# DannielSilva/MM-VQA

Measured on AMD Instinct MI355X. Metric: samples/sec ROCO-MLM pretrain (resnet152+transformer, bs16/GPU, 224^2, seq32), higher is better.
Workload: dtype f32; 1 GPU; pretrain/roco_train.py MLM-only: resnet152 + transformer(4 layers, 12 heads), num_vis 5, hidden 768, vocab 30522, per-GPU batch 16, 224x224, T=32; fwd + log_softmax/NLL + bwd + grad all-reduce + Adam; dropout on, train-mode BN; random-init weights; global_batch=16, seq_len=32, parallelism=dp1

## Files before the change

### include/mmvqa.h

```cpp
#ifndef MMVQA_H
#define MMVQA_H
#include <stddef.h>
#include <stdint.h>

#ifdef __cplusplus
extern "C" {
#endif

typedef void* mmvqa_stream_t;

#define MMVQA_ACT_NONE 0
#define MMVQA_ACT_RELU 1
#define MMVQA_ACT_GELU 2
#define MMVQA_ACT_SERF 3
#define MMVQA_ACT_SILU 4
#define MMVQA_ACT_SIGMOID 5

#define MMVQA_KIND_FWD 0
#define MMVQA_KIND_DGRAD 1
#define MMVQA_KIND_WGRAD 2

#define MMVQA_STAT_SLOTS 16

typedef struct mmvqa_bn_fold {
// ... 75 lines not shown
  float* colsum;
  const float* gate;
  int gate_hw;
  int mk_mode;
  const int* pixmask;
  float* sk_ws;
  long long sk_ws_floats;
  mmvqa_bn_fold a_fold;
  int stat_slots;
  int reserved1;
  unsigned int* sk_cnt;
  int sk_cnt_n;
  int reserved0;
} mmvqa_gemm_desc;

#define MMVQA_PREC_F32 0
#define MMVQA_PREC_F16 1

typedef struct mmvqa_attn_desc {
  const float* q;
  const float* k;
  const float* v;
  int row_stride, head_stride;
  float* out;
  int out_row_stride, out_head_stride;
  const long long* mask;
  int mask_on_query;
  const float* prev_in;
  float* prev_out;
  float* probs;
  int B, T, heads;
  float sqrt_d;
  float drop_p;
  uint32_t seed;
  const float* dout;
  float* dq;
  float* dk;
  float* dv;
  const float* dprev_in;
  float* dprev_out;
} mmvqa_attn_desc;

typedef struct mmvqa_fb_attn_desc {
  const float* q;
  int q_ld;
  const float* mem_k;
  const float* mem_v;
  long long mem_win;
  int mem_ld;
  const float* self_k;
  const float* self_v;
  int self_ld;
  const float* bias;
  float* probs;
  int p_ld;
  float* out;
  int out_ld;
  int B, n, n_mem, T;
  float scale, drop_p;
  uint32_t seed;
  const float* dout;
  int dout_ld;
  float* dq;
  int dq_ld;
  float* dself_k;
  float* dself_v;
  int dself_ld;
  float* dmem_k;
  float* dmem_v;
  float* dbias;
} mmvqa_fb_attn_desc;

#define MMVQA_FB_MAX_HIDDENS 16
#define MMVQA_FB_MAX_T 256

typedef struct mmvqa_model_desc {
  int cnn;
  int resnet_layers[4];
  int resnet_width;
  int effnet_depth_div;
  int encoder;
  int hidden, heads, n_layers;
  int emb_vocab, max_pos, type_vocab;
  int num_vis;
  int head_kind;
  int n_classes;
  int supcon, feat_dim;
  int use_relu;
  float p_drop;
  float p_emb_drop;
  float p_rf_drop;
  float p_fb_drop;
  int fb_tokens;
} mmvqa_model_desc;

typedef struct mmvqa_bert_desc {
  int layers, hidden, heads, inter, vocab, max_pos, type_vocab;
  float eps;
} mmvqa_bert_desc;

typedef struct mmvqa_bert mmvqa_bert;

typedef void (*mmvqa_grad_cb)(void* user, long long lo, long long hi);

typedef struct mmvqa_engine mmvqa_engine;

int mmvqa_version(void);
const char* mmvqa_last_error(void);
size_t mmvqa_sizeof_gemm_desc(void);
size_t mmvqa_sizeof_attn_desc(void);
size_t mmvqa_sizeof_model_desc(void);
size_t mmvqa_sizeof_fb_attn_desc(void);
size_t mmvqa_sizeof_bert_desc(void);

int mmvqa_igemm(const mmvqa_gemm_desc* d, int kind, int nchw, int tile, mmvqa_stream_t s);
int mmvqa_attention(const mmvqa_attn_desc* d, int head_dim, int backward, mmvqa_stream_t s);
int mmvqa_attention_len_fwd(mmvqa_stream_t s, const float* q, const float* k, const float* v, int row_stride,
                            int head_stride, float* out, int out_row_stride, int out_head_stride, const int* len, int B,
                            int T, int heads, float scale);
int mmvqa_qkv_attention_fwd(mmvqa_stream_t s, const float* xn, const float* W, const float* bias, const long long* mask,
                            float* qkv, float* probs, float* ctx, int B, int T, int hidden, int heads, float drop_p,
                            uint32_t seed);

int mmvqa_fb_attention(const mmvqa_fb_attn_desc* d, int backward, mmvqa_stream_t s);
int mmvqa_fb_aggregate_fwd(mmvqa_stream_t s, const float* hid, long long hid_stride, int n_hid, const float* layer_weight,
                           float* agg, long rows, int H);
int mmvqa_fb_aggregate_bwd(mmvqa_stream_t s, const float* dagg, const float* hid, long long hid_stride, int n_hid,
                           const float* layer_weight, float* dh, long long dh_stride, float* dtop, float* d_layer_weight,
                           long rows, int H);
int mmvqa_geglu_fwd(mmvqa_stream_t s, const float* pre, float* y, long M, int F, float drop_p, uint32_t seed, uint32_t idx0);
int mmvqa_geglu_bwd(mmvqa_stream_t s, const float* dy, const float* pre, float* dpre, long M, int F, float drop_p,
                    uint32_t seed, uint32_t idx0);

int mmvqa_bn_coef_fwd(mmvqa_stream_t s, const double* stat, int C, double count, float eps, const float* gamma,
                      const float* beta, float* run_mean, float* run_var, long long* nbt, float momentum, int reps,
                      int training, float* scale, float* shift, float* mean, float* invstd);
int mmvqa_bn_coef_bwd(mmvqa_stream_t s, const double* stat, int C, double count, const float* gamma,
                      const float* mean, const float* invstd, int training, float* P, float* Q, float* R,
                      float* dgamma, float* dbeta);
int mmvqa_bn_add_relu(mmvqa_stream_t s, const float* z, const float* sc, const float* sh, const float* idn,
                      const float* id_sc, const float* id_sh, float* out, long rows, int C);
int mmvqa_bn_add_relu_fold(mmvqa_stream_t s, const float* z, const mmvqa_bn_fold* f3, const float* idn,
                           const mmvqa_bn_fold* fd, float* out, long rows, int C);
int mmvqa_maxpool_fwd(mmvqa_stream_t s, const float* z, const float* sc, const float* sh, float* out,
                      unsigned char* idx, int N, int H, int W, int C, int OH, int OW);
int mmvqa_maxpool_bwd(mmvqa_stream_t s, const float* gp, const unsigned char* idx, const float* extra,
                      const float* z, const float* sc, const float* sh, const float* mean, const float* invstd,
                      float* g0, double* stat, int N, int H, int W, int C, int OH, int OW);
int mmvqa_layernorm_fwd(mmvqa_stream_t s, const float* x, const float* res, const float* gamma, const float* beta,
                        float* y, float* sum_out, float* mean, float* rstd, int rows, int H, float eps);
int mmvqa_layernorm_bwd(mmvqa_stream_t s, const float* dy, const float* x, const float* gamma, const float* mean,
                        const float* rstd, const float* dres, float* dx, float* dgamma, float* dbeta, int rows,
                        int H);
int mmvqa_embed_fwd(mmvqa_stream_t s, const long long* ids, const long long* seg, const float* word,
                    const float* pos, const float* type, const float* gamma, const float* beta, const float* vis,
                    float* out, float* xhat, float* rstd, int B, int T, int H, int num_vis, float eps,
                    float drop_p, uint32_t seed);
int mmvqa_embed_bwd(mmvqa_stream_t s, const float* dout, const long long* ids, const long long* seg,
                    const float* xhat, const float* rstd, const float* gamma, float* dword, float* dpos,
                    float* dtype, float* dgamma, float* dbeta, float* dvis, int B, int T, int H, int num_vis,
                    float drop_p, uint32_t seed, int pad_idx);
int mmvqa_meanpool_fwd(mmvqa_stream_t s, const float* h, const long long* mask, float* out, int B, int T, int H);
int mmvqa_meanpool_bwd(mmvqa_stream_t s, const float* dout, const long long* mask, float* dh, int B, int T, int H,
                       int accumulate);
int mmvqa_mlm_loss(mmvqa_stream_t s, const float* logits, int ld, const long long* target, float* row_loss,
                   float* row_lse, long long* pred, float* dlogits, int dld, const float* gscale_ptr, float gscale_mul,
                   int rows, int V, float* out3);
int mmvqa_mlm_grad(mmvqa_stream_t s, const float* logits, int ld, const long long* target, const float* row_lse,
                   float* dlogits, int dld, const float* gscale_ptr, float gscale_mul, int rows, int V);
int mmvqa_asl_loss(mmvqa_stream_t s, const float* logits, int ld, const long long* target, float* row_loss,
                   float* dlogits, int dld, int rows, int C, float gamma_pos, float gamma_neg, float eps,
                   float gscale);
int mmvqa_l2norm_fwd(mmvqa_stream_t s, const float* x, float* y, float* nrm, int rows, int D);
int mmvqa_l2norm_bwd(mmvqa_stream_t s, const float* dy, const float* y, const float* nrm, float* dx, int rows,
                     int D);
int mmvqa_supcon_loss(mmvqa_stream_t s, const float* f, float* loss, float* df, float* ws, int N, int D, float temp,
                      float base_temp, float gscale);
int mmvqa_supcon_loss_masked(mmvqa_stream_t s, const float* f, const float* mask, float* loss, float* df, float* ws,
                             int N, int D, float temp, float base_temp, float gscale);
int mmvqa_jaccard_mask(mmvqa_stream_t s, const int* offsets, const int* ids, const int* rowsA, const int* colsA,
                       const int* rowsB, const int* colsB, float* mask, int n, int table_rows);
int mmvqa_normalize_rows(mmvqa_stream_t s, float* x, long long rows, int D, float eps);
int mmvqa_cosine_mask(mmvqa_stream_t s, const float* table, const int* rowsA, const int* colsA, const int* rowsB,
                      const int* colsB, float* mask, int n, int D, int table_rows);
int mmvqa_bertscore_mask(mmvqa_stream_t s, const float* xa, const int* lenA, const float* xb, const int* lenB, float* mask,
                         float* prec, float* rec, int n, int T, int D, float baseline);
#define MMVQA_SOFT_CE_HARD 0
#define MMVQA_SOFT_CE_UNIFORM 1
#define MMVQA_SOFT_CE_CATEGORY 2
int mmvqa_soft_ce_loss(mmvqa_stream_t s, const float* logits, int ld, const long long* target, const long long* category,
                       const float* table, int table_ld, int n_cat, int mode, double smoothing, float* row_loss,
                       float* loss, float* dlogits, int dld, int rows, int C, float gscale);
int mmvqa_distill_mse(mmvqa_stream_t s, const float* h, int ld, const void* table, int table_f16, long long table_rows,
                      const long long* start, const int* count, int first, int B, int T, int H, float* row_sq, float* loss,
                      float* dh, int dld, float gscale);
int mmvqa_dwconv_fwd(mmvqa_stream_t s, const float* z1, const float* s1, const float* b1, const float* w, float* z2,
                     double* stat, int N, int H, int W, int C, int OH, int OW, int stride, int pad);
int mmvqa_dwconv_bwd_data(mmvqa_stream_t s, const float* g2, const float* z2, const float* P, const float* Q,
                          const float* R, const float* w, const float* z1, const float* s1, const float* b1,
                          const float* mean1, const float* invstd1, float* g1, double* stat, int N, int H, int W, int C,
                          int OH, int OW, int stride, int pad);
int mmvqa_dwconv_bwd_weight(mmvqa_stream_t s, const float* g2, const float* z2, const float* P, const float* Q,
                            const float* R, const float* z1, const float* s1, const float* b1, float* dw, int N, int H,
                            int W, int C, int OH, int OW, int stride, int pad);
int mmvqa_se_pool(mmvqa_stream_t s, const float* z, const float* sc, const float* sh, float* pool, int N, int HW, int C);
int mmvqa_se_dgate(mmvqa_stream_t s, const float* t, const float* z, const float* sc, const float* sh, float* dgate,
                   int N, int HW, int C);
int mmvqa_dwconv_fwd_fold(mmvqa_stream_t s, const float* z1, const float* s1, const float* b1, const float* w, float* z2,
                          double* stat, int N, int H, int W, int C, int OH, int OW, int stride, int pad,
                          const mmvqa_bn_fold* fold);
int mmvqa_dwconv_bwd_data_fold(mmvqa_stream_t s, const float* g2, const float* z2, const float* P, const float* Q,
                               const float* R, const float* w, const float* z1, const float* s1, const float* b1,
                               const float* mean1, const float* invstd1, float* g1, double* stat, int N, int H, int W,
                               int C, int OH, int OW, int stride, int pad, const mmvqa_bn_fold* fold);
int mmvqa_dwconv_bwd_weight_fold(mmvqa_stream_t s, const float* g2, const float* z2, const float* P, const float* Q,
                                 const float* R, const float* z1, const float* s1, const float* b1, float* dw, int N,
                                 int H, int W, int C, int OH, int OW, int stride, int pad, const mmvqa_bn_fold* fold);
int mmvqa_se_pool_fold(mmvqa_stream_t s, const float* z, const float* sc, const float* sh, float* pool, int N, int HW,
                       int C, const mmvqa_bn_fold* fold);
int mmvqa_tap_thin_ok(long M, int N, int C, int HW);
int mmvqa_tap_thin_fwd(mmvqa_stream_t s, const float* x, const float* sc, const float* sh, const float* W, float* out,
                       long M, int N, int C, int HW, int act);
int mmvqa_tap_thin_bwd(mmvqa_stream_t s, const float* x, const float* sc, const float* sh, const float* W,
                       const float* dv, float* du, long M, int N, int C, int HW, int act);
int mmvqa_se_fc_fwd(mmvqa_stream_t s, const float* pool, const float* Wr, const float* br, const float* We,
                    const float* be, float* rpre, float* r, float* gpre, float* gate, int B, int mid, int rd);
size_t mmvqa_se_fc_bwd_scratch_floats(int B, int mid, int rd);
int mmvqa_se_fc_bwd(mmvqa_stream_t s, const float* dgate, const float* gpre, const float* r, const float* rpre,
                    const float* pool, const float* We, const float* Wr, float* dWe, float* dbe, float* dWr, float* dbr,
                    float* dpool, float* scratch, int B, int mid, int rd);
int mmvqa_act_bwd_stats(mmvqa_stream_t s, const float* t, const float* gate, const float* add, const float* z,
                        const float* sc, const float* sh, const float* mean, const float* invstd, int act, float* out,
                        double* stat, long npix, int HW, int C);
int mmvqa_bn_act_add(mmvqa_stream_t s, const float* z, const float* sc, const float* sh, int pre_act, const float* idn,
                     const float* ids, const float* idb, int idn_act, int post_act, float* out, long rows, int C);
int mmvqa_bn_act_add_fold(mmvqa_stream_t s, const float* z, const mmvqa_bn_fold* f3, int pre_act, const float* idn,
                          const mmvqa_bn_fold* fd, int post_act, float* out, long rows, int C);
int mmvqa_adam(mmvqa_stream_t s, float* p, float* g, float* m, float* v, long n, double lr, double b1, double b2,
               double eps, int step, float gscale, int zero_grad);
int mmvqa_amp_unscale(mmvqa_stream_t s, float* g, long n, const float* inv_scale, float* found_inf, int multiply);
int mmvqa_amp_update_scale(mmvqa_stream_t s, float* scale, int* growth_tracker, const float* found_inf,
                           double growth_factor, double backoff_factor, int growth_interval);
int mmvqa_axpy(mmvqa_stream_t s, float* y, const float* x, float a, long n);
int mmvqa_colsum(mmvqa_stream_t s, const float* x, int ld, int rows, int cols, float* out);
int mmvqa_dropout(mmvqa_stream_t s, float* x, long n, float p, uint32_t seed);
int mmvqa_dropout_copy(mmvqa_stream_t s, const float* x, float* y, long n, float p, uint32_t seed);
int mmvqa_pixmask(mmvqa_stream_t s, int* out, int N, int OH, int OW, int SH, int SW, int KH, int KW, int stride,
                  int pad);

int mmvqa_engine_create(const mmvqa_model_desc* desc, mmvqa_engine** out);
void mmvqa_engine_destroy(mmvqa_engine* e);
int mmvqa_engine_num_tensors(const mmvqa_engine* e);
int mmvqa_engine_tensor_info(const mmvqa_engine* e, int i, char* name, int name_cap, int* kind, int* ndim,
                             long long shape[4], long long* offset, int* channels_last);
long long mmvqa_engine_param_floats(const mmvqa_engine* e);
long long mmvqa_engine_buf_floats(const mmvqa_engine* e);
long long mmvqa_engine_nbt_count(const mmvqa_engine* e);
size_t mmvqa_engine_plan(mmvqa_engine* e, int B, int T, int img_h, int img_w);
int mmvqa_engine_bind(mmvqa_engine* e, float* params, float* grads, float* bufs, long long* nbt, void* workspace,
                      size_t workspace_bytes);
int mmvqa_engine_forward(mmvqa_engine* e, mmvqa_stream_t s, const float* img, const long long* ids,
                         const long long* seg, const long long* mask, float* logits, int logits_ld, float* feat,
                         int training, uint32_t seed);
int mmvqa_engine_backward(mmvqa_engine* e, mmvqa_stream_t s, const float* dlogits, int dlogits_ld,
                          const float* dfeat);
int mmvqa_engine_backward_feature(mmvqa_engine* e, mmvqa_stream_t s, const float* dlogits, int dlogits_ld, float* dA);
int mmvqa_engine_feature_map(mmvqa_engine* e, const float** A, int* H, int* W, int* C);
int mmvqa_gradcam(mmvqa_stream_t s, const float* A, const float* dA, int B, int H, int W, int C, float* cam, int* valid,
                  float* up, int IH, int IW, const unsigned char* image_u8, const unsigned char* jet, float alpha,
                  unsigned char* overlay);
int mmvqa_engine_set_grad_callback(mmvqa_engine* e, mmvqa_grad_cb cb, void* user);
int mmvqa_engine_tune(mmvqa_engine* e, int enable);
int mmvqa_engine_set_precision(mmvqa_engine* e, int mode);
int mmvqa_engine_profile(mmvqa_engine* e, int enable);
int mmvqa_engine_profile_read(mmvqa_engine* e, int cls, long long* launches, double* ms, double* flops);
int mmvqa_engine_profile_read_region(mmvqa_engine* e, int region, int cls, long long* launches, double* ms,
                                     double* flops);
int mmvqa_engine_profile_read_hbm(mmvqa_engine* e, int kernel, long long* launches, double* ms, double* bytes);

int mmvqa_bert_create(const mmvqa_bert_desc* desc, mmvqa_bert** out);
void mmvqa_bert_destroy(mmvqa_bert* e);
int mmvqa_bert_num_tensors(const mmvqa_bert* e);
long long mmvqa_bert_param_floats(const mmvqa_bert* e);
int mmvqa_bert_tensor_info(const mmvqa_bert* e, int i, char* name, int name_cap, int* ndim, long long shape[2],
                           long long* offset);
size_t mmvqa_bert_plan(mmvqa_bert* e, int B, int T);
int mmvqa_bert_bind(mmvqa_bert* e, const float* params, void* workspace, size_t workspace_bytes);
int mmvqa_bert_forward(mmvqa_bert* e, mmvqa_stream_t s, const long long* ids, const int* len, int B, int T, float* out);
int mmvqa_bert_forward_layers(mmvqa_bert* e, mmvqa_stream_t s, const long long* ids, const int* len, int B, int T,
                              int n_layers, float* out);

typedef struct mmvqa_resample_job {
  const unsigned char* src; int sh, sw, spitch;
  int bx, by, bw, bh;
  int rw, rh;
  int ox, oy;
  int ty0, tyn;
  unsigned char* tmp;
  unsigned char* dst; int dpitch;
  const int* hb; const int* hk; int hks;
  const int* vb; const int* vk; int vks;
} mmvqa_resample_job;
size_t mmvqa_sizeof_resample_job(void);
int mmvqa_resample_coeffs(int in_size, double in0, double in1, int out_size, int* bounds, int* kk, int ksize_cap);
int mmvqa_aug_resample(mmvqa_stream_t s, const mmvqa_resample_job* jobs_dev, int njobs, int max_tmp_rows, int out_h,
                       int out_w);
// ... 30 lines not shown
```

### mm-vqa_amd/_lib.py

```python
from __future__ import annotations

import ctypes as C
import os

_HERE = os.path.dirname(os.path.abspath(__file__))
LIB_PATH = os.path.join(_HERE, "libmmvqa_hip.so")

c_f32p = C.c_void_p
c_ptr = C.c_void_p

ACT_NONE, ACT_RELU, ACT_GELU, ACT_SERF, ACT_SILU, ACT_SIGMOID = 0, 1, 2, 3, 4, 5
KIND_FWD, KIND_DGRAD, KIND_WGRAD = 0, 1, 2
PRO_NONE, PRO_AFFINE_RELU, PRO_DZ, PRO_AFFINE, PRO_AFFINE_SILU, PRO_SILU_GATE = 0, 1, 2, 3, 4, 5
EPI_PLAIN, EPI_TAP_FWD, EPI_TAP_BWD = 0, 1, 2
PREC_F32, PREC_F16 = 0, 1
SOFT_CE_HARD, SOFT_CE_UNIFORM, SOFT_CE_CATEGORY = 0, 1, 2
HEAD_MLM, HEAD_VQA, HEAD_NONE = 0, 1, 2
STAT_SLOTS = 16


class BnFold(C.Structure):
    _fields_ = [
        ("stat", c_ptr), ("slots", C.c_int), ("bwd", C.c_int), ("publish", C.c_int), ("reps", C.c_int),
        ("count", C.c_double), ("keep", C.c_double), ("eps", C.c_float), ("reserved", C.c_int),
        ("gamma", c_ptr), ("beta", c_ptr), ("mean", c_ptr), ("invstd", c_ptr),
        ("out0", c_ptr), ("out1", c_ptr), ("out2", c_ptr), ("out3", c_ptr),
        ("run_mean", c_ptr), ("run_var", c_ptr), ("nbt", c_ptr), ("dgamma", c_ptr), ("dbeta", c_ptr),
    ]


class GemmDesc(C.Structure):
    _fields_ = [
        ("M", C.c_int), ("N", C.c_int), ("K", C.c_int), ("splitk", C.c_int), ("ktiles_per_split", C.c_int),
        ("A", c_ptr), ("A2", c_ptr), ("a_c0", c_ptr), ("a_c1", c_ptr), ("a_c2", c_ptr),
        ("a_pro", C.c_int), ("a_ld", C.c_int),
        ("B", c_ptr), ("b_c0", c_ptr), ("b_c1", c_ptr), ("b_pro", C.c_int), ("b_ld", C.c_int),
        ("b_tapstride", C.c_int),
        ("g_SH", C.c_int), ("g_SW", C.c_int), ("g_Cs", C.c_int), ("g_OH", C.c_int), ("g_OW", C.c_int),
        ("g_KH", C.c_int), ("g_KW", C.c_int), ("g_stride", C.c_int), ("g_pad", C.c_int), ("g_nchw", C.c_int),
        ("C", c_ptr), ("c_ld", C.c_int), ("c_atomic", C.c_int), ("Cpre", c_ptr), ("bias", c_ptr),
        ("act", C.c_int), ("dact", C.c_int), ("Pre", c_ptr), ("pre_ld", C.c_int),
        ("drop_p", C.c_float), ("drop_seed", C.c_uint32), ("R", c_ptr), ("r_ld", C.c_int),
        ("epi_mode", C.c_int), ("tap_HW", C.c_int), ("tap_out", c_ptr), ("tap_dv", c_ptr),
        ("Mk", c_ptr), ("mk_ld", C.c_int), ("mk_s", c_ptr), ("mk_b", c_ptr),
        ("stat1", c_ptr), ("stat_bwd", C.c_int), ("Z1", c_ptr), ("z1_ld", C.c_int), ("mean1", c_ptr),
        ("invstd1", c_ptr),
        ("stat2", c_ptr), ("Z2", c_ptr), ("z2_ld", C.c_int), ("mean2", c_ptr), ("invstd2", c_ptr),
        ("colsum", c_ptr), ("gate", c_ptr), ("gate_hw", C.c_int), ("mk_mode", C.c_int), ("pixmask", c_ptr),
        ("sk_ws", c_ptr), ("sk_ws_floats", C.c_longlong),
        ("a_fold", BnFold), ("stat_slots", C.c_int), ("reserved1", C.c_int), ("sk_cnt", c_ptr), ("sk_cnt_n", C.c_int),
        ("reserved0", C.c_int),
    ]


class AttnDesc(C.Structure):
    _fields_ = [
        ("q", c_ptr), ("k", c_ptr), ("v", c_ptr), ("row_stride", C.c_int), ("head_stride", C.c_int),
        ("out", c_ptr), ("out_row_stride", C.c_int), ("out_head_stride", C.c_int),
        ("mask", c_ptr), ("mask_on_query", C.c_int), ("prev_in", c_ptr), ("prev_out", c_ptr), ("probs", c_ptr),
        ("B", C.c_int), ("T", C.c_int), ("heads", C.c_int), ("sqrt_d", C.c_float), ("drop_p", C.c_float),
        ("seed", C.c_uint32),
        ("dout", c_ptr), ("dq", c_ptr), ("dk", c_ptr), ("dv", c_ptr), ("dprev_in", c_ptr), ("dprev_out", c_ptr),
    ]


class FbAttnDesc(C.Structure):
    _fields_ = [
        ("q", c_ptr), ("q_ld", C.c_int), ("mem_k", c_ptr), ("mem_v", c_ptr), ("mem_win", C.c_longlong), ("mem_ld", C.c_int),
        ("self_k", c_ptr), ("self_v", c_ptr), ("self_ld", C.c_int), ("bias", c_ptr), ("probs", c_ptr), ("p_ld", C.c_int),
        ("out", c_ptr), ("out_ld", C.c_int), ("B", C.c_int), ("n", C.c_int), ("n_mem", C.c_int), ("T", C.c_int),
        ("scale", C.c_float), ("drop_p", C.c_float), ("seed", C.c_uint32),
        ("dout", c_ptr), ("dout_ld", C.c_int), ("dq", c_ptr), ("dq_ld", C.c_int),
        ("dself_k", c_ptr), ("dself_v", c_ptr), ("dself_ld", C.c_int), ("dmem_k", c_ptr), ("dmem_v", c_ptr), ("dbias", c_ptr),
    ]


FB_MAX_HIDDENS, FB_MAX_T = 16, 256
ENC_TRANSFORMER, ENC_REALFORMER, ENC_FEEDBACK = 0, 1, 2


class ResampleJob(C.Structure):
    _fields_ = [
        ("src", c_ptr), ("sh", C.c_int), ("sw", C.c_int), ("spitch", C.c_int),
        ("bx", C.c_int), ("by", C.c_int), ("bw", C.c_int), ("bh", C.c_int),
        ("rw", C.c_int), ("rh", C.c_int), ("ox", C.c_int), ("oy", C.c_int), ("ty0", C.c_int), ("tyn", C.c_int),
        ("tmp", c_ptr), ("dst", c_ptr), ("dpitch", C.c_int),
        ("hb", c_ptr), ("hk", c_ptr), ("hks", C.c_int), ("vb", c_ptr), ("vk", c_ptr), ("vks", C.c_int),
    ]


class AugRecord(C.Structure):
    _fields_ = [
        ("bx", C.c_int), ("by", C.c_int), ("bw", C.c_int), ("bh", C.c_int), ("ty0", C.c_int), ("tyn", C.c_int),
        ("hb", C.c_int), ("hk", C.c_int), ("hks", C.c_int), ("vb", C.c_int), ("vk", C.c_int), ("vks", C.c_int),
        ("fix", C.c_int * 6), ("op", C.c_int * 4), ("factor", C.c_float * 4),
    ]


class ModelDesc(C.Structure):
    _fields_ = [
        ("cnn", C.c_int), ("resnet_layers", C.c_int * 4), ("resnet_width", C.c_int), ("effnet_depth_div", C.c_int),
        ("encoder", C.c_int), ("hidden", C.c_int), ("heads", C.c_int), ("n_layers", C.c_int),
        ("emb_vocab", C.c_int), ("max_pos", C.c_int), ("type_vocab", C.c_int), ("num_vis", C.c_int),
        ("head_kind", C.c_int), ("n_classes", C.c_int), ("supcon", C.c_int), ("feat_dim", C.c_int),
        ("use_relu", C.c_int), ("p_drop", C.c_float), ("p_emb_drop", C.c_float), ("p_rf_drop", C.c_float),
        ("p_fb_drop", C.c_float), ("fb_tokens", C.c_int),
    ]


class BertDesc(C.Structure):
    _fields_ = [
        ("layers", C.c_int), ("hidden", C.c_int), ("heads", C.c_int), ("inter", C.c_int), ("vocab", C.c_int),
        ("max_pos", C.c_int), ("type_vocab", C.c_int), ("eps", C.c_float),
    ]


_i, _f, _d, _l, _ll, _u32, _sz = C.c_int, C.c_float, C.c_double, C.c_long, C.c_longlong, C.c_uint32, C.c_size_t
_P = c_ptr
SIGNATURES = {
    "mmvqa_version": (_i, []),
    "mmvqa_last_error": (C.c_char_p, []),
    "mmvqa_sizeof_gemm_desc": (_sz, []),
    "mmvqa_sizeof_attn_desc": (_sz, []),
    "mmvqa_sizeof_model_desc": (_sz, []),
    "mmvqa_sizeof_fb_attn_desc": (_sz, []),
    "mmvqa_sizeof_bert_desc": (_sz, []),
    "mmvqa_igemm": (_i, [C.POINTER(GemmDesc), _i, _i, _i, _P]),
    "mmvqa_attention": (_i, [C.POINTER(AttnDesc), _i, _i, _P]),
    "mmvqa_attention_len_fwd": (_i, [_P, _P, _P, _P, _i, _i, _P, _i, _i, _P, _i, _i, _i, _f]),
    "mmvqa_qkv_attention_fwd": (_i, [_P, _P, _P, _P, _P, _P, _P, _P, _i, _i, _i, _i, _f, _u32]),
    "mmvqa_fb_attention": (_i, [C.POINTER(FbAttnDesc), _i, _P]),
    "mmvqa_fb_aggregate_fwd": (_i, [_P, _P, _ll, _i, _P, _P, _l, _i]),
    "mmvqa_fb_aggregate_bwd": (_i, [_P, _P, _P, _ll, _i, _P, _P, _ll, _P, _P, _l, _i]),
    "mmvqa_geglu_fwd": (_i, [_P, _P, _P, _l, _i, _f, _u32, _u32]),
    "mmvqa_geglu_bwd": (_i, [_P, _P, _P, _P, _l, _i, _f, _u32, _u32]),
    "mmvqa_bn_coef_fwd": (_i, [_P, _P, _i, _d, _f, _P, _P, _P, _P, _P, _f, _i, _i, _P, _P, _P, _P]),
    "mmvqa_bn_coef_bwd": (_i, [_P, _P, _i, _d, _P, _P, _P, _i, _P, _P, _P, _P, _P]),
    "mmvqa_bn_add_relu": (_i, [_P, _P, _P, _P, _P, _P, _P, _P, _l, _i]),
    "mmvqa_bn_add_relu_fold": (_i, [_P, _P, C.POINTER(BnFold), _P, C.POINTER(BnFold), _P, _l, _i]),
    "mmvqa_maxpool_fwd": (_i, [_P, _P, _P, _P, _P, _P, _i, _i, _i, _i, _i, _i]),
    "mmvqa_maxpool_bwd": (_i, [_P, _P, _P, _P, _P, _P, _P, _P, _P, _P, _P, _i, _i, _i, _i, _i, _i]),
    "mmvqa_layernorm_fwd": (_i, [_P, _P, _P, _P, _P, _P, _P, _P, _P, _i, _i, _f]),
    "mmvqa_layernorm_bwd": (_i, [_P, _P, _P, _P, _P, _P, _P, _P, _P, _P, _i, _i]),
    "mmvqa_embed_fwd": (_i, [_P, _P, _P, _P, _P, _P, _P, _P, _P, _P, _P, _P, _i, _i, _i, _i, _f, _f, _u32]),
    "mmvqa_embed_bwd": (_i, [_P, _P, _P, _P, _P, _P, _P, _P, _P, _P, _P, _P, _P, _i, _i, _i, _i, _f, _u32, _i]),
    "mmvqa_meanpool_fwd": (_i, [_P, _P, _P, _P, _i, _i, _i]),
    "mmvqa_meanpool_bwd": (_i, [_P, _P, _P, _P, _i, _i, _i, _i]),
    "mmvqa_mlm_loss": (_i, [_P, _P, _i, _P, _P, _P, _P, _P, _i, _P, _f, _i, _i, _P]),
    "mmvqa_mlm_grad": (_i, [_P, _P, _i, _P, _P, _P, _i, _P, _f, _i, _i]),
    "mmvqa_asl_loss": (_i, [_P, _P, _i, _P, _P, _P, _i, _i, _i, _f, _f, _f, _f]),
    "mmvqa_l2norm_fwd": (_i, [_P, _P, _P, _P, _i, _i]),
    "mmvqa_l2norm_bwd": (_i, [_P, _P, _P, _P, _P, _i, _i]),
    "mmvqa_supcon_loss": (_i, [_P, _P, _P, _P, _P, _i, _i, _f, _f, _f]),
    "mmvqa_supcon_loss_masked": (_i, [_P, _P, _P, _P, _P, _P, _i, _i, _f, _f, _f]),
    "mmvqa_jaccard_mask": (_i, [_P] * 8 + [_i, _i]),
    "mmvqa_normalize_rows": (_i, [_P, _P, _ll, _i, _f]),
    "mmvqa_cosine_mask": (_i, [_P] * 7 + [_i, _i, _i]),
    "mmvqa_bertscore_mask": (_i, [_P] * 8 + [_i, _i, _i, _f]),
    "mmvqa_soft_ce_loss": (_i, [_P, _P, _i, _P, _P, _P, _i, _i, _i, _d, _P, _P, _P, _i, _i, _i, _f]),
    "mmvqa_distill_mse": (_i, [_P, _P, _i, _P, _i, _ll, _P, _P, _i, _i, _i, _i, _P, _P, _P, _i, _f]),
    "mmvqa_dwconv_fwd": (_i, [_P, _P, _P, _P, _P, _P, _P] + [_i] * 8),
    "mmvqa_dwconv_bwd_data": (_i, [_P] * 14 + [_i] * 8),
    "mmvqa_dwconv_bwd_weight": (_i, [_P] * 10 + [_i] * 8),
    "mmvqa_se_pool": (_i, [_P, _P, _P, _P, _P, _i, _i, _i]),
    "mmvqa_dwconv_fwd_fold": (_i, [_P, _P, _P, _P, _P, _P, _P] + [_i] * 8 + [C.POINTER(BnFold)]),
    "mmvqa_dwconv_bwd_data_fold": (_i, [_P] * 14 + [_i] * 8 + [C.POINTER(BnFold)]),
    "mmvqa_dwconv_bwd_weight_fold": (_i, [_P] * 10 + [_i] * 8 + [C.POINTER(BnFold)]),
    "mmvqa_se_pool_fold": (_i, [_P, _P, _P, _P, _P, _i, _i, _i, C.POINTER(BnFold)]),
    "mmvqa_bn_act_add_fold": (_i, [_P, _P, C.POINTER(BnFold), _i, _P, C.POINTER(BnFold), _i, _P, _l, _i]),
    "mmvqa_se_dgate": (_i, [_P, _P, _P, _P, _P, _P, _i, _i, _i]),
    "mmvqa_tap_thin_ok": (_i, [_l, _i, _i, _i]),
    "mmvqa_tap_thin_fwd": (_i, [_P] * 6 + [_l, _i, _i, _i, _i]),
    "mmvqa_tap_thin_bwd": (_i, [_P] * 7 + [_l, _i, _i, _i, _i]),
    "mmvqa_se_fc_fwd": (_i, [_P] * 10 + [_i, _i, _i]),
    "mmvqa_se_fc_bwd_scratch_floats": (_sz, [_i, _i, _i]),
    "mmvqa_se_fc_bwd": (_i, [_P] * 14 + [_i, _i, _i]),
    "mmvqa_act_bwd_stats": (_i, [_P] * 9 + [_i, _P, _P, _l, _i, _i]),
    "mmvqa_bn_act_add": (_i, [_P, _P, _P, _P, _i, _P, _P, _P, _i, _i, _P, _l, _i]),
    "mmvqa_adam": (_i, [_P, _P, _P, _P, _P, _l, _d, _d, _d, _d, _i, _f, _i]),
    "mmvqa_axpy": (_i, [_P, _P, _P, _f, _l]),
    "mmvqa_colsum": (_i, [_P, _P, _i, _i, _i, _P]),
    "mmvqa_dropout": (_i, [_P, _P, _l, _f, _u32]),
    "mmvqa_dropout_copy": (_i, [_P, _P, _P, _l, _f, _u32]),
    "mmvqa_pixmask": (_i, [_P, _P] + [_i] * 9),
    "mmvqa_sizeof_resample_job": (_sz, []),
    "mmvqa_resample_coeffs": (_i, [_i, _d, _d, _i, _P, _P, _i]),
    "mmvqa_aug_resample": (_i, [_P, _P, _i, _i, _i, _i]),
    "mmvqa_aug_rotate": (_i, [_P, _P, _P, _P, _i, _i, _i]),
    "mmvqa_aug_jitter_round": (_i, [_P, _P, _P, _P, _P, _i, _i]),
    "mmvqa_aug_to_tensor": (_i, [_P, _P, _P, _i, _i, _P, _P]),
    "mmvqa_sizeof_aug_record": (_sz, []),
    "mmvqa_aug_train_fused": (_i, [_P, _P, _P, _P, _P, _i, _i, _P, _P]),
    "mmvqa_aug_train_fused_views": (_i, [_P, _P, _P, _P, _P, _P, _i, _i, _i, _P, _P]),
    "mmvqa_aug_train_fused_fits": (_i, [_i]),
    "mmvqa_low_priority_stream": (_i, [C.POINTER(_P), C.POINTER(_i)]),
    "mmvqa_stream_priority": (_i, [_P, C.POINTER(_i)]),
    "mmvqa_bert_create": (_i, [C.POINTER(BertDesc), C.POINTER(_P)]),
    "mmvqa_bert_destroy": (None, [_P]),
    "mmvqa_bert_num_tensors": (_i, [_P]),
    "mmvqa_bert_param_floats": (_ll, [_P]),
    "mmvqa_bert_tensor_info": (_i, [_P, _i, C.c_char_p, _i, C.POINTER(_i), C.POINTER(_ll * 2), C.POINTER(_ll)]),
    "mmvqa_bert_plan": (_sz, [_P, _i, _i]),
    "mmvqa_bert_bind": (_i, [_P, _P, _P, _sz]),
    "mmvqa_bert_forward": (_i, [_P, _P, _P, _P, _i, _i, _P]),
    "mmvqa_bert_forward_layers": (_i, [_P, _P, _P, _P, _i, _i, _i, _P]),
    "mmvqa_engine_create": (_i, [C.POINTER(ModelDesc), C.POINTER(_P)]),
    "mmvqa_engine_destroy": (None, [_P]),
    "mmvqa_engine_num_tensors": (_i, [_P]),
    "mmvqa_engine_tensor_info": (_i, [_P, _i, C.c_char_p, _i, C.POINTER(_i), C.POINTER(_i), C.POINTER(_ll * 4),
                                      C.POINTER(_ll), C.POINTER(_i)]),
    "mmvqa_engine_param_floats": (_ll, [_P]),
    "mmvqa_engine_buf_floats": (_ll, [_P]),
    "mmvqa_engine_nbt_count": (_ll, [_P]),
    "mmvqa_engine_plan": (_sz, [_P, _i, _i, _i, _i]),
    "mmvqa_engine_bind": (_i, [_P, _P, _P, _P, _P, _P, _sz]),
    "mmvqa_engine_forward": (_i, [_P, _P, _P, _P, _P, _P, _P, _i, _P, _i, _u32]),
    "mmvqa_engine_backward": (_i, [_P, _P, _P, _i, _P]),
    "mmvqa_engine_backward_feature": (_i, [_P, _P, _P, _i, _P]),
    "mmvqa_engine_feature_map": (_i, [_P, C.POINTER(_P), C.POINTER(_i), C.POINTER(_i), C.POINTER(_i)]),
    "mmvqa_gradcam": (_i, [_P, _P, _P, _i, _i, _i, _i, _P, _P, _P, _i, _i, _P, _P, _f, _P]),
    "mmvqa_engine_set_grad_callback": (_i, [_P, _P, _P]),
    "mmvqa_engine_tune": (_i, [_P, _i]),
    "mmvqa_amp_unscale": (_i, [_P, _P, _l, _P, _P, _i]),
    "mmvqa_amp_update_scale": (_i, [_P, _P, _P, _P, _d, _d, _i]),
    "mmvqa_engine_set_precision": (_i, [_P, _i]),
    "mmvqa_engine_profile": (_i, [_P, _i]),
    "mmvqa_engine_profile_read": (_i, [_P, _i, C.POINTER(_ll), C.POINTER(_d), C.POINTER(_d)]),
    "mmvqa_engine_profile_read_region": (_i, [_P, _i, _i, C.POINTER(_ll), C.POINTER(_d), C.POINTER(_d)]),
    "mmvqa_engine_profile_read_hbm": (_i, [_P, _i, C.POINTER(_ll), C.POINTER(_d), C.POINTER(_d)]),
}

_lib = None


class MMVQAError(RuntimeError):
    pass


def lib():
    global _lib
    if _lib is not None:
        return _lib
    if not os.path.exists(LIB_PATH):
        raise MMVQAError(
            f"{LIB_PATH} not found: the HIP extension is not built. There is no CPU fallback -- run "
            "`python -c 'import __graft_entry__ as g; g.build()'` (needs hipcc, no GPU required).")
    L = C.CDLL(LIB_PATH)
    for name, (res, args) in SIGNATURES.items():
        fn = getattr(L, name)
        fn.restype = res
        fn.argtypes = args
    for nm, st in (("gemm", GemmDesc), ("attn", AttnDesc), ("model", ModelDesc), ("fb_attn", FbAttnDesc), ("bert", BertDesc), ("resample_job", ResampleJob),
                   ("aug_record", AugRecord)):
        if nm in ("resample_job", "aug_record"):
            got = getattr(L, f"mmvqa_sizeof_{nm}")()
            if got != C.sizeof(st):
                raise MMVQAError(f"ABI mismatch: sizeof(mmvqa_{nm}) = {got} in the library, {C.sizeof(st)} in Python")
            continue
        got = getattr(L, f"mmvqa_sizeof_{nm}_desc")()
        if got != C.sizeof(st):
            raise MMVQAError(f"ABI mismatch: sizeof(mmvqa_{nm}_desc) = {got} in the library, {C.sizeof(st)} in Python")
    _lib = L
    return L


def check(rc: int):
    if rc != 0:
        msg = lib().mmvqa_last_error()
        raise MMVQAError(f"mmvqa error {rc}: {msg.decode() if msg else '?'}")


def ptr(t):
    return None if t is None else C.c_void_p(t.data_ptr())


def stream_ptr():
    import torch
    return C.c_void_p(torch.cuda.current_stream().cuda_stream)
```

### mm-vqa_amd/csrc/abi.cpp

```cpp
#include <cstring>

#include "engine.h"

const char* mmvqa_get_error();
size_t engine_plan(mmvqa_engine* e, int B, int T, int IH, int IW);
int engine_forward(mmvqa_engine* e, hipStream_t st, const float* img, const long long* ids, const long long* seg,
                   const long long* mask, float* logits, int logits_ld, float* feat, int training, uint32_t seed);
int engine_backward(mmvqa_engine* e, hipStream_t st, const float* dlogits, int dl_ld, const float* dfeat);
int engine_backward_feature(mmvqa_engine* e, hipStream_t st, const float* dlogits, int dl_ld, float* dA);
int engine_feature_map(mmvqa_engine* e, const float** A, int* H, int* W, int* C);
int engine_create(const mmvqa_model_desc* desc, mmvqa_engine** out);
int engine_profile_collect(mmvqa_engine* e);

#define ST(s) reinterpret_cast<hipStream_t>(s)

extern "C" {

int mmvqa_version(void) { return 100; }
const char* mmvqa_last_error(void) { return mmvqa_get_error(); }
size_t mmvqa_sizeof_gemm_desc(void) { return sizeof(mmvqa_gemm_desc); }
size_t mmvqa_sizeof_attn_desc(void) { return sizeof(mmvqa_attn_desc); }
size_t mmvqa_sizeof_model_desc(void) { return sizeof(mmvqa_model_desc); }
size_t mmvqa_sizeof_fb_attn_desc(void) { return sizeof(mmvqa_fb_attn_desc); }

static int check_gemm(const mmvqa_gemm_desc* d, int kind, int nchw) {
  if (!d) return mmvqa_set_error(MMVQA_ERR_ARG, "igemm: null descriptor");
  if (kind < 0 || kind > 2) return mmvqa_set_error(MMVQA_ERR_ARG, "igemm: kind=%d", kind);
  if (!d->A || !d->B || (!d->C && d->epi_mode != EPI_TAP_FWD))
    return mmvqa_set_error(MMVQA_ERR_ARG, "igemm: null operand");
  if (!nchw) {
    const int taps = d->g_KH * d->g_KW;
    if ((d->a_ld & 3) || (d->b_ld & 3) || (taps > 1 && (d->g_Cs & 3)))
      return mmvqa_set_error(MMVQA_ERR_ARG, "igemm: a_ld=%d b_ld=%d g_Cs=%d must be multiples of 4", d->a_ld,
                             d->b_ld, d->g_Cs);
    if (kind != KIND_FWD && (d->N & 3) && kind == KIND_DGRAD)
      return mmvqa_set_error(MMVQA_ERR_ARG, "igemm dgrad: N=%d must be a multiple of 4", d->N);
  }
  if (d->a_pro == PRO_DZ && (!d->A2 || (!d->a_fold.stat && (!d->a_c0 || !d->a_c1 || !d->a_c2))))
    return mmvqa_set_error(MMVQA_ERR_ARG, "igemm: PRO_DZ needs A2 and three coefficient arrays (or a_fold)");
  if (d->g_SH <= 0 || d->g_SW <= 0 || d->g_OH <= 0 || d->g_OW <= 0 || d->g_Cs <= 0)
    return mmvqa_set_error(MMVQA_ERR_ARG, "igemm: gather geometry not set");
  return MMVQA_OK;
}

int mmvqa_igemm(const mmvqa_gemm_desc* d, int kind, int nchw, int tile, mmvqa_stream_t s) {
  int r = check_gemm(d, kind, nchw);
  if (r != MMVQA_OK) return r;
  return mmvqa_launch_igemm(*d, kind, nchw, tile, ST(s));
}

int mmvqa_attention(const mmvqa_attn_desc* d, int head_dim, int backward, mmvqa_stream_t s) {
  if (!d || !d->q || !d->k || !d->v || !d->mask || !d->probs)
    return mmvqa_set_error(MMVQA_ERR_ARG, "attention: null operand");
  if ((d->row_stride & 3) || (d->head_stride & 3) || (d->out_row_stride & 3) || (d->out_head_stride & 3))
    return mmvqa_set_error(MMVQA_ERR_ARG, "attention: strides must be multiples of 4");
  if (backward && (!d->dout || !d->dq || !d->dk || !d->dv))
    return mmvqa_set_error(MMVQA_ERR_ARG, "attention backward: null gradient pointer");
  if (!backward && !d->out) return mmvqa_set_error(MMVQA_ERR_ARG, "attention: null output");
  return mmvqa_launch_attention(*d, head_dim, backward, ST(s));
}

int mmvqa_qkv_attention_fwd(mmvqa_stream_t s, const float* xn, const float* W, const float* bias, const long long* mask,
                            float* qkv, float* probs, float* ctx, int B, int T, int hidden, int heads, float drop_p,
                            uint32_t seed) {
  if (B <= 0 || drop_p < 0.f || drop_p >= 1.f) return mmvqa_set_error(MMVQA_ERR_ARG, "qkv_attention_fwd: B=%d drop_p=%g", B, (double)drop_p);
  return k_qkv_attn_fwd(ST(s), xn, W, bias, mask, qkv, probs, ctx, B, T, hidden, heads, drop_p, seed);
}
int mmvqa_attention_len_fwd(mmvqa_stream_t s, const float* q, const float* k, const float* v, int row_stride,
                            int head_stride, float* out, int out_row_stride, int out_head_stride, const int* len, int B,
                            int T, int heads, float scale) {
  return k_attention_len_fwd(ST(s), q, k, v, row_stride, head_stride, out, out_row_stride, out_head_stride, len, B, T, heads,
                             scale);
}
int mmvqa_fb_attention(const mmvqa_fb_attn_desc* d, int backward, mmvqa_stream_t s) {
  if (!d) return mmvqa_set_error(MMVQA_ERR_ARG, "fb_attention: null descriptor");
  return k_fb_attention(ST(s), *d, backward ? 1 : 0);
}
int mmvqa_fb_aggregate_fwd(mmvqa_stream_t s, const float* hid, long long hid_stride, int n_hid, const float* layer_weight,
                           float* agg, long rows, int H) {
  return k_fb_aggregate_fwd(ST(s), hid, hid_stride, n_hid, layer_weight, agg, rows, H);
}
int mmvqa_fb_aggregate_bwd(mmvqa_stream_t s, const float* dagg, const float* hid, long long hid_stride, int n_hid,
                           const float* layer_weight, float* dh, long long dh_stride, float* dtop, float* d_layer_weight,
                           long rows, int H) {
  return k_fb_aggregate_bwd(ST(s), dagg, hid, hid_stride, n_hid, layer_weight, dh, dh_stride, dtop, d_layer_weight, rows, H);
}
int mmvqa_geglu_fwd(mmvqa_stream_t s, const float* pre, float* y, long M, int F, float drop_p, uint32_t seed, uint32_t idx0) {
  return k_geglu_fwd(ST(s), pre, y, M, F, drop_p, seed, idx0);
}
int mmvqa_geglu_bwd(mmvqa_stream_t s, const float* dy, const float* pre, float* dpre, long M, int F, float drop_p,
                    uint32_t seed, uint32_t idx0) {
  return k_geglu_bwd(ST(s), dy, pre, dpre, M, F, drop_p, seed, idx0);
}
int mmvqa_bn_coef_fwd(mmvqa_stream_t s, const double* stat, int C, double count, float eps, const float* gamma,
                      const float* beta, float* run_mean, float* run_var, long long* nbt, float momentum, int reps,
                      int training, float* scale, float* shift, float* mean, float* invstd) {
  return k_bn_coef_fwd(ST(s), stat, C, count, eps, gamma, beta, run_mean, run_var, nbt, momentum, reps, training,
                       scale, shift, mean, invstd);
}
int mmvqa_bn_coef_bwd(mmvqa_stream_t s, const double* stat, int C, double count, const float* gamma,
                      const float* mean, const float* invstd, int training, float* P, float* Q, float* R,
                      float* dgamma, float* dbeta) {
  return k_bn_coef_bwd(ST(s), stat, C, count, gamma, mean, invstd, training, P, Q, R, dgamma, dbeta);
}
int mmvqa_bn_add_relu_fold(mmvqa_stream_t s, const float* z, const mmvqa_bn_fold* f3, const float* idn,
                           const mmvqa_bn_fold* fd, float* out, long rows, int C) {
  if (!z || !idn || !out || !f3) return mmvqa_set_error(MMVQA_ERR_ARG, "bn_add_relu_fold: null operand");
  return k_bn_add_relu_fold(ST(s), z, f3, idn, fd, out, rows, C);
}
int mmvqa_bn_add_relu(mmvqa_stream_t s, const float* z, const float* sc, const float* sh, const float* idn,
                      const float* id_sc, const float* id_sh, float* out, long rows, int C) {
  if (C & 3) return mmvqa_set_error(MMVQA_ERR_ARG, "bn_add_relu: C %% 4 != 0");
  return k_bn_add_relu(ST(s), z, sc, sh, idn, id_sc, id_sh, out, rows, C);
}
int mmvqa_maxpool_fwd(mmvqa_stream_t s, const float* z, const float* sc, const float* sh, float* out,
                      unsigned char* idx, int N, int H, int W, int C, int OH, int OW) {
  if (C & 3) return mmvqa_set_error(MMVQA_ERR_ARG, "maxpool: C %% 4 != 0");
  return k_maxpool_fwd(ST(s), z, sc, sh, out, idx, N, H, W, C, OH, OW);
}
int mmvqa_maxpool_bwd(mmvqa_stream_t s, const float* gp, const unsigned char* idx, const float* extra,
                      const float* z, const float* sc, const float* sh, const float* mean, const float* invstd,
                      float* g0, double* stat, int N, int H, int W, int C, int OH, int OW) {
  return k_maxpool_bwd(ST(s), gp, idx, extra, z, sc, sh, mean, invstd, g0, stat, N, H, W, C, OH, OW);
}
int mmvqa_layernorm_fwd(mmvqa_stream_t s, const float* x, const float* res, const float* gamma, const float* beta,
                        float* y, float* sum_out, float* mean, float* rstd, int rows, int H, float eps) {
  return k_layernorm_fwd(ST(s), x, res, gamma, beta, y, sum_out, mean, rstd, rows, H, eps);
}
int mmvqa_layernorm_bwd(mmvqa_stream_t s, const float* dy, const float* x, const float* gamma, const float* mean,
                        const float* rstd, const float* dres, float* dx, float* dgamma, float* dbeta, int rows,
                        int H) {
  return k_layernorm_bwd(ST(s), dy, x, gamma, mean, rstd, dres, dx, dgamma, dbeta, rows, H);
}
int mmvqa_embed_fwd(mmvqa_stream_t s, const long long* ids, const long long* seg, const float* word,
                    const float* pos, const float* type, const float* gamma, const float* beta, const float* vis,
                    float* out, float* xhat, float* rstd, int B, int T, int H, int num_vis, float eps,
                    float drop_p, uint32_t seed) {
  return k_embed_fwd(ST(s), ids, seg, word, pos, type, gamma, beta, vis, out, xhat, rstd, B, T, H, num_vis, eps,
                     drop_p, seed);
}
int mmvqa_embed_bwd(mmvqa_stream_t s, const float* dout, const long long* ids, const long long* seg,
                    const float* xhat, const float* rstd, const float* gamma, float* dword, float* dpos,
                    float* dtype, float* dgamma, float* dbeta, float* dvis, int B, int T, int H, int num_vis,
                    float drop_p, uint32_t seed, int pad_idx) {
  return k_embed_bwd(ST(s), dout, ids, seg, xhat, rstd, gamma, dword, dpos, dtype, dgamma, dbeta, dvis, B, T, H,
                     num_vis, drop_p, seed, pad_idx);
}
int mmvqa_meanpool_fwd(mmvqa_stream_t s, const float* h, const long long* mask, float* out, int B, int T, int H) {
  return k_meanpool_fwd(ST(s), h, mask, out, B, T, H);
}
int mmvqa_meanpool_bwd(mmvqa_stream_t s, const float* dout, const long long* mask, float* dh, int B, int T, int H,
                       int accumulate) {
  return k_meanpool_bwd(ST(s), dout, mask, dh, B, T, H, accumulate);
}
int mmvqa_mlm_loss(mmvqa_stream_t s, const float* logits, int ld, const long long* target, float* row_loss,
                   float* row_lse, long long* pred, float* dlogits, int dld, const float* gscale_ptr, float gscale_mul,
                   int rows, int V, float* out3) {
  return k_lsm_nll(ST(s), logits, ld, target, row_loss, row_lse, pred, dlogits, dld, gscale_ptr, gscale_mul, rows, V, out3);
}
int mmvqa_mlm_grad(mmvqa_stream_t s, const float* logits, int ld, const long long* target, const float* row_lse,
                   float* dlogits, int dld, const float* gscale_ptr, float gscale_mul, int rows, int V) {
  return k_lsm_grad(ST(s), logits, ld, target, row_lse, dlogits, dld, gscale_ptr, gscale_mul, rows, V);
}
int mmvqa_asl_loss(mmvqa_stream_t s, const float* logits, int ld, const long long* target, float* row_loss,
                   float* dlogits, int dld, int rows, int C, float gamma_pos, float gamma_neg, float eps,
                   float gscale) {
  return k_asl(ST(s), logits, ld, target, row_loss, dlogits, dld, rows, C, gamma_pos, gamma_neg, eps, gscale);
}
int mmvqa_l2norm_fwd(mmvqa_stream_t s, const float* x, float* y, float* nrm, int rows, int D) {
  return k_l2norm_fwd(ST(s), x, y, nrm, rows, D);
}
int mmvqa_l2norm_bwd(mmvqa_stream_t s, const float* dy, const float* y, const float* nrm, float* dx, int rows,
                     int D) {
  return k_l2norm_bwd(ST(s), dy, y, nrm, dx, rows, D);
}
int mmvqa_supcon_loss(mmvqa_stream_t s, const float* f, float* loss, float* df, float* ws, int N, int D, float temp,
                      float base_temp, float gscale) {
  return k_supcon(ST(s), f, nullptr, loss, df, ws, N, D, temp, base_temp, gscale);
}
int mmvqa_supcon_loss_masked(mmvqa_stream_t s, const float* f, const float* mask, float* loss, float* df, float* ws,
                             int N, int D, float temp, float base_temp, float gscale) {
  if (!mask) return mmvqa_set_error(MMVQA_ERR_ARG, "supcon_masked: mask is null (mmvqa_supcon_loss is the loss without one)");
  return k_supcon(ST(s), f, mask, loss, df, ws, N, D, temp, base_temp, gscale);
}
int mmvqa_jaccard_mask(mmvqa_stream_t s, const int* offsets, const int* ids, const int* rowsA, const int* colsA,
                       const int* rowsB, const int* colsB, float* mask, int n, int table_rows) {
  return k_jaccard_mask(ST(s), offsets, ids, rowsA, colsA, rowsB, colsB, mask, n, table_rows);
}
int mmvqa_normalize_rows(mmvqa_stream_t s, float* x, long long rows, int D, float eps) {
  return k_normalize_rows(ST(s), x, rows, D, eps);
}
int mmvqa_cosine_mask(mmvqa_stream_t s, const float* table, const int* rowsA, const int* colsA, const int* rowsB,
                      const int* colsB, float* mask, int n, int D, int table_rows) {
  return k_cosine_mask(ST(s), table, rowsA, colsA, rowsB, colsB, mask, n, D, table_rows);
}
int mmvqa_bertscore_mask(mmvqa_stream_t s, const float* xa, const int* lenA, const float* xb, const int* lenB, float* mask,
                         float* prec, float* rec, int n, int T, int D, float baseline) {
  return k_bertscore_mask(ST(s), xa, lenA, xb, lenB, mask, prec, rec, n, T, D, baseline);
}
int mmvqa_soft_ce_loss(mmvqa_stream_t s, const float* logits, int ld, const long long* target, const long long* category,
                       const float* table, int table_ld, int n_cat, int mode, double smoothing, float* row_loss,
                       float* loss, float* dlogits, int dld, int rows, int C, float gscale) {
  return k_soft_ce(ST(s), logits, ld, target, category, table, table_ld, n_cat, mode, smoothing, row_loss, loss, dlogits,
                   dld, rows, C, gscale);
}
int mmvqa_distill_mse(mmvqa_stream_t s, const float* h, int ld, const void* table, int table_f16, long long table_rows,
                      const long long* start, const int* count, int first, int B, int T, int H, float* row_sq, float* loss,
                      float* dh, int dld, float gscale) {
  return k_distill_mse(ST(s), h, ld, table, table_f16, table_rows, start, count, first, B, T, H, row_sq, loss, dh, dld,
                       gscale);
}
int mmvqa_dwconv_fwd(mmvqa_stream_t s, const float* z1, const float* s1, const float* b1, const float* w, float* z2,
                     double* stat, int N, int H, int W, int C, int OH, int OW, int stride, int pad) {
  return k_dwconv_fwd(ST(s), z1, s1, b1, w, z2, stat, N, H, W, C, OH, OW, stride, pad);
}
int mmvqa_dwconv_bwd_data(mmvqa_stream_t s, const float* g2, const float* z2, const float* P, const float* Q,
                          const float* R, const float* w, const float* z1, const float* s1, const float* b1,
                          const float* mean1, const float* invstd1, float* g1, double* stat, int N, int H, int W, int C,
                          int OH, int OW, int stride, int pad) {
  return k_dwconv_bwd_data(ST(s), g2, z2, P, Q, R, w, z1, s1, b1, mean1, invstd1, g1, stat, N, H, W, C, OH, OW, stride, pad);
}
int mmvqa_dwconv_bwd_weight(mmvqa_stream_t s, const float* g2, const float* z2, const float* P, const float* Q,
                            const float* R, const float* z1, const float* s1, const float* b1, float* dw, int N, int H,
                            int W, int C, int OH, int OW, int stride, int pad) {
  return k_dwconv_bwd_weight(ST(s), g2, z2, P, Q, R, z1, s1, b1, dw, N, H, W, C, OH, OW, stride, pad);
}
int mmvqa_se_pool(mmvqa_stream_t s, const float* z, const float* sc, const float* sh, float* pool, int N, int HW, int C) {
  return k_se_pool(ST(s), z, sc, sh, pool, N, HW, C);
}
int mmvqa_dwconv_fwd_fold(mmvqa_stream_t s, const float* z1, const float* s1, const float* b1, const float* w, float* z2,
                          double* stat, int N, int H, int W, int C, int OH, int OW, int stride, int pad,
                          const mmvqa_bn_fold* fold) {
  return k_dwconv_fwd(ST(s), z1, s1, b1, w, z2, stat, N, H, W, C, OH, OW, stride, pad, fold);
}
int mmvqa_dwconv_bwd_data_fold(mmvqa_stream_t s, const float* g2, const float* z2, const float* P, const float* Q,
                               const float* R, const float* w, const float* z1, const float* s1, const float* b1,
                               const float* mean1, const float* invstd1, float* g1, double* stat, int N, int H, int W,
                               int C, int OH, int OW, int stride, int pad, const mmvqa_bn_fold* fold) {
  return k_dwconv_bwd_data(ST(s), g2, z2, P, Q, R, w, z1, s1, b1, mean1, invstd1, g1, stat, N, H, W, C, OH, OW, stride, pad, fold);
}
int mmvqa_dwconv_bwd_weight_fold(mmvqa_stream_t s, const float* g2, const float* z2, const float* P, const float* Q,
                                 const float* R, const float* z1, const float* s1, const float* b1, float* dw, int N,
                                 int H, int W, int C, int OH, int OW, int stride, int pad, const mmvqa_bn_fold* fold) {
  return k_dwconv_bwd_weight(ST(s), g2, z2, P, Q, R, z1, s1, b1, dw, N, H, W, C, OH, OW, stride, pad, fold);
}
int mmvqa_se_pool_fold(mmvqa_stream_t s, const float* z, const float* sc, const float* sh, float* pool, int N, int HW,
                       int C, const mmvqa_bn_fold* fold) {
  return k_se_pool(ST(s), z, sc, sh, pool, N, HW, C, fold);
}
int mmvqa_bn_act_add_fold(mmvqa_stream_t s, const float* z, const mmvqa_bn_fold* f3, int pre_act, const float* idn,
                          const mmvqa_bn_fold* fd, int post_act, float* out, long rows, int C) {
  return k_bn_act_add_fold(ST(s), z, f3, pre_act, idn, fd, post_act, out, rows, C);
}
int mmvqa_se_dgate(mmvqa_stream_t s, const float* t, const float* z, const float* sc, const float* sh, float* dgate,
                   int N, int HW, int C) {
  return k_se_dgate(ST(s), t, z, sc, sh, dgate, N, HW, C);
}
int mmvqa_tap_thin_ok(long M, int N, int C, int HW) { return k_tap_thin_ok(M, N, C, HW) ? 1 : 0; }
int mmvqa_tap_thin_fwd(mmvqa_stream_t s, const float* x, const float* sc, const float* sh, const float* W, float* out,
                       long M, int N, int C, int HW, int act) {
  return k_tap_thin_fwd(ST(s), x, sc, sh, W, out, M, N, C, HW, act);
}
int mmvqa_tap_thin_bwd(mmvqa_stream_t s, const float* x, const float* sc, const float* sh, const float* W,
                       const float* dv, float* du, long M, int N, int C, int HW, int act) {
  return k_tap_thin_bwd(ST(s), x, sc, sh, W, dv, du, M, N, C, HW, act);
}
int mmvqa_se_fc_fwd(mmvqa_stream_t s, const float* pool, const float* Wr, const float* br, const float* We,
                    const float* be, float* rpre, float* r, float* gpre, float* gate, int B, int mid, int rd) {
  int rc = k_skinny_fwd(ST(s), pool, mid, Wr, br, ACT_SILU, rpre, r, B, rd, mid);
  if (rc != MMVQA_OK) return rc;
  return k_skinny_fwd(ST(s), r, rd, We, be, ACT_SIGMOID, gpre, gate, B, mid, rd);
}
size_t mmvqa_se_fc_bwd_scratch_floats(int B, int mid, int rd) { return k_se_fc_bwd_scratch_floats(B, mid, rd); }
int mmvqa_se_fc_bwd(mmvqa_stream_t s, const float* dgate, const float* gpre, const float* r, const float* rpre,
                    const float* pool, const float* We, const float* Wr, float* dWe, float* dbe, float* dWr, float* dbr,
                    float* dpool, float* scratch, int B, int mid, int rd) {
  return k_se_fc_bwd(ST(s), dgate, gpre, r, rpre, pool, We, Wr, dWe, dbe, dWr, dbr, dpool, scratch, 0, B, mid, rd);
}
int mmvqa_act_bwd_stats(mmvqa_stream_t s, const float* t, const float* gate, const float* add, const float* z,
                        const float* sc, const float* sh, const float* mean, const float* invstd, int act, float* out,
                        double* stat, long npix, int HW, int C) {
  return k_act_bwd_stats(ST(s), t, gate, add, z, sc, sh, mean, invstd, act, out, stat, npix, HW, C);
}
int mmvqa_bn_act_add(mmvqa_stream_t s, const float* z, const float* sc, const float* sh, int pre_act, const float* idn,
                     const float* ids, const float* idb, int idn_act, int post_act, float* out, long rows, int C) {
  return k_bn_act_add(ST(s), z, sc, sh, pre_act, idn, ids, idb, idn_act, post_act, out, rows, C);
// ... 169 lines not shown
```

### mm-vqa_amd/csrc/elementwise.hip

```cpp
#include <cstring>

#include "common.h"

static inline int cdiv_i(long a, long b) { return (int)((a + b - 1) / b); }

static_assert(MMVQA_STAT_SLOTS == 16, "one lane per statistics replica");
__device__ __forceinline__ void stat_fold16(const double* __restrict__ stat, int C, int c, bool live, double& s0,
                                            double& s1) {
  typedef double f64x2 __attribute__((ext_vector_type(2)));
  const int sl = threadIdx.x & 15;
  f64x2 v = {0.0, 0.0};
  if (live) v = *reinterpret_cast<const f64x2*>(stat + ((size_t)sl * C + c) * 2);
  s0 = v[0]; s1 = v[1];
#pragma unroll
  for (int o = 8; o > 0; o >>= 1) { s0 += __shfl_xor(s0, o, 64); s1 += __shfl_xor(s1, o, 64); }
}
__global__ __launch_bounds__(256) void bn_coef_fwd_kernel(const double* __restrict__ stat, int C, double count, float eps,
                                   const float* __restrict__ gamma, const float* __restrict__ beta,
                                   float* __restrict__ run_mean, float* __restrict__ run_var,
                                   long long* __restrict__ nbt, double keep, int reps, int training,
                                   float* __restrict__ scale, float* __restrict__ shift,
                                   float* __restrict__ mean_out, float* __restrict__ invstd_out) {
  const int c = blockIdx.x * 16 + (threadIdx.x >> 4);
  if (blockIdx.x == 0 && threadIdx.x == 0 && training && nbt) *nbt += reps;
// ... 73 lines not shown
                                   unsigned char* __restrict__ idx, int N, int H, int W, int C, int OH, int OW) {
  const int C4 = C / 4;
  long total = (long)N * OH * OW * C4;
  long i = (long)blockIdx.x * blockDim.x + threadIdx.x;
  long stride = (long)gridDim.x * blockDim.x;
  for (; i < total; i += stride) {
    int c = (int)(i % C4) * 4;
    long pix = i / C4;
    int ox = (int)(pix % OW); long t = pix / OW;
    int oy = (int)(t % OH); int n = (int)(t / OH);
    f32x4 sv = *reinterpret_cast<const f32x4*>(s + c), bv = *reinterpret_cast<const f32x4*>(b + c);
    f32x4 best = {-INFINITY, -INFINITY, -INFINITY, -INFINITY};
    int bi[4] = {0, 0, 0, 0};
#pragma unroll
    for (int kh = 0; kh < 3; ++kh) {
      int y = oy * 2 - 1 + kh;
      if (y < 0 || y >= H) continue;
#pragma unroll
      for (int kw = 0; kw < 3; ++kw) {
        int x = ox * 2 - 1 + kw;
        if (x < 0 || x >= W) continue;
        f32x4 v = *reinterpret_cast<const f32x4*>(z + ((size_t)(n * H + y) * W + x) * C + c);
#pragma unroll
        for (int j = 0; j < 4; ++j) {
          float a = v[j] * sv[j] + bv[j];
          a = a > 0.f ? a : 0.f;
          if (a > best[j]) { best[j] = a; bi[j] = kh * 3 + kw; }
        }
      }
    }
    reinterpret_cast<f32x4*>(out)[i] = best;
    uchar4 u; u.x = bi[0]; u.y = bi[1]; u.z = bi[2]; u.w = bi[3];
    reinterpret_cast<uchar4*>(idx)[i] = u;
  }
}

__global__ void maxpool_bwd_kernel(const float* __restrict__ gp, const unsigned char* __restrict__ idx,
                                   const float* __restrict__ extra, const float* __restrict__ z,
                                   const float* __restrict__ s, const float* __restrict__ b,
                                   const float* __restrict__ mean, const float* __restrict__ invstd,
                                   float* __restrict__ g0, double* __restrict__ stat,
                                   int N, int H, int W, int C, int OH, int OW) {
  const int C4 = C / 4;
  long total = (long)N * H * W * C4;
  long i = (long)blockIdx.x * blockDim.x + threadIdx.x;
  long stride = (long)gridDim.x * blockDim.x;
  const int c = (int)(i % C4) * 4;
  f32x4 sv = *reinterpret_cast<const f32x4*>(s + c), bv = *reinterpret_cast<const f32x4*>(b + c);
  f32x4 mu = *reinterpret_cast<const f32x4*>(mean + c), is = *reinterpret_cast<const f32x4*>(invstd + c);
  double sg[4] = {0, 0, 0, 0}, sgx[4] = {0, 0, 0, 0};
  for (; i < total; i += stride) {
    long pix = i / C4;
    int x = (int)(pix % W); long t = pix / W;
    int y = (int)(t % H); int n = (int)(t / H);
    f32x4 g = extra ? reinterpret_cast<const f32x4*>(extra)[i] : f32x4{0, 0, 0, 0};
    int oy0 = y >> 1, ox0 = x >> 1;
    for (int oy = oy0; oy <= oy0 + 1; ++oy) {
      int kh = y - (oy * 2 - 1);
      if (kh < 0 || kh > 2 || oy >= OH) continue;
      for (int ox = ox0; ox <= ox0 + 1; ++ox) {
        int kw = x - (ox * 2 - 1);
        if (kw < 0 || kw > 2 || ox >= OW) continue;
        size_t o = ((size_t)(n * OH + oy) * OW + ox) * C + c;
        uchar4 u = *reinterpret_cast<const uchar4*>(idx + o);
        f32x4 gv = *reinterpret_cast<const f32x4*>(gp + o);
        int code = kh * 3 + kw;
        if (u.x == code) g[0] += gv[0];
        if (u.y == code) g[1] += gv[1];
        if (u.z == code) g[2] += gv[2];
        if (u.w == code) g[3] += gv[3];
      }
    }
    f32x4 zv = reinterpret_cast<const f32x4*>(z)[i];
#pragma unroll
    for (int j = 0; j < 4; ++j) {
      float a = zv[j] * sv[j] + bv[j];
      if (!(a > 0.f)) g[j] = 0.f;
      sg[j] += (double)g[j];
      sgx[j] += (double)(g[j] * ((zv[j] - mu[j]) * is[j]));
    }
    reinterpret_cast<f32x4*>(g0)[i] = g;
  }
  __shared__ double red[256 * 8];
  const int tid = threadIdx.x;
#pragma unroll
  for (int j = 0; j < 4; ++j) { red[tid * 8 + j] = sg[j]; red[tid * 8 + 4 + j] = sgx[j]; }
  __syncthreads();
  if (tid < C4) {
    double a[8] = {0, 0, 0, 0, 0, 0, 0, 0};
    for (int t = tid; t < 256; t += C4)
#pragma unroll
      for (int j = 0; j < 8; ++j) a[j] += red[t * 8 + j];
    int slot = blockIdx.x & (MMVQA_STAT_SLOTS - 1);
#pragma unroll
    for (int j = 0; j < 4; ++j) {
      double* d = stat + ((size_t)slot * C + tid * 4 + j) * 2;
      atomicAdd(d, a[j]);
      atomicAdd(d + 1, a[4 + j]);
    }
  }
}

#define LN_MAXV 4
__global__ void layernorm_fwd_kernel(const float* __restrict__ x, const float* __restrict__ res,
                                     const float* __restrict__ gamma, const float* __restrict__ beta,
                                     float* __restrict__ y, float* __restrict__ sum_out,
                                     float* __restrict__ mean_out, float* __restrict__ rstd_out,
                                     int rows, int H, float eps) {
  const int lane = threadIdx.x & 63;
  const int row = blockIdx.x * (blockDim.x >> 6) + (threadIdx.x >> 6);
  if (row >= rows) return;
  const int H4 = H / 4;
  f32x4 v[LN_MAXV];
  float s = 0.f;
#pragma unroll
  for (int j = 0; j < LN_MAXV; ++j) {
    int q = lane + 64 * j;
    v[j] = f32x4{0, 0, 0, 0};
    if (q < H4) {
      v[j] = reinterpret_cast<const f32x4*>(x + (size_t)row * H)[q];
      if (res) {
        f32x4 r = reinterpret_cast<const f32x4*>(res + (size_t)row * H)[q];
        v[j] += r;
        if (sum_out) reinterpret_cast<f32x4*>(sum_out + (size_t)row * H)[q] = v[j];
      }
      s += v[j][0] + v[j][1] + v[j][2] + v[j][3];
    }
  }
  float mean = wave_sum(s) / (float)H;
  float ss = 0.f;
#pragma unroll
  for (int j = 0; j < LN_MAXV; ++j) {
    int q = lane + 64 * j;
    if (q < H4) {
#pragma unroll
      for (int e = 0; e < 4; ++e) { float d = v[j][e] - mean; ss += d * d; }
    }
  }
  float var = wave_sum(ss) / (float)H;
  float rstd = 1.0f / sqrtf(var + eps);
#pragma unroll
  for (int j = 0; j < LN_MAXV; ++j) {
    int q = lane + 64 * j;
    if (q < H4) {
      f32x4 g = reinterpret_cast<const f32x4*>(gamma)[q], b = reinterpret_cast<const f32x4*>(beta)[q], o;
#pragma unroll
      for (int e = 0; e < 4; ++e) o[e] = (v[j][e] - mean) * rstd * g[e] + b[e];
      reinterpret_cast<f32x4*>(y + (size_t)row * H)[q] = o;
    }
  }
  if (lane == 0) { mean_out[row] = mean; rstd_out[row] = rstd; }
}

__global__ void layernorm_bwd_kernel(const float* __restrict__ dy, const float* __restrict__ x,
                                     const float* __restrict__ gamma, const float* __restrict__ mean,
                                     const float* __restrict__ rstd, const float* __restrict__ dres,
                                     float* __restrict__ dx, float* __restrict__ dgamma,
                                     float* __restrict__ dbeta, int rows, int H, int rows_per_wave) {
  extern __shared__ float lds[];
  const int lane = threadIdx.x & 63, wave = threadIdx.x >> 6, nw = blockDim.x >> 6;
  const int H4 = H / 4;
  for (int i = threadIdx.x; i < 2 * H; i += blockDim.x) lds[i] = 0.f;
  __syncthreads();
  f32x4 ag[LN_MAXV], ab[LN_MAXV];
#pragma unroll
  for (int j = 0; j < LN_MAXV; ++j) { ag[j] = f32x4{0, 0, 0, 0}; ab[j] = f32x4{0, 0, 0, 0}; }
  const int row0 = (blockIdx.x * nw + wave) * rows_per_wave;
  for (int rr = 0; rr < rows_per_wave; ++rr) {
    const int row = row0 + rr;
    if (row >= rows) break;
    const float mu = mean[row], rs = rstd[row];
    f32x4 xh[LN_MAXV], dg[LN_MAXV];
    float s1 = 0.f, s2 = 0.f;
#pragma unroll
    for (int j = 0; j < LN_MAXV; ++j) {
      int q = lane + 64 * j;
      xh[j] = f32x4{0, 0, 0, 0}; dg[j] = f32x4{0, 0, 0, 0};
      if (q < H4) {
        f32x4 xv = reinterpret_cast<const f32x4*>(x + (size_t)row * H)[q];
        f32x4 d = reinterpret_cast<const f32x4*>(dy + (size_t)row * H)[q];
        f32x4 g = reinterpret_cast<const f32x4*>(gamma)[q];
#pragma unroll
        for (int e = 0; e < 4; ++e) {
          xh[j][e] = (xv[e] - mu) * rs;
          dg[j][e] = d[e] * g[e];
          s1 += dg[j][e];
          s2 += dg[j][e] * xh[j][e];
          ag[j][e] += d[e] * xh[j][e];
          ab[j][e] += d[e];
        }
      }
    }
    s1 = wave_sum(s1) / (float)H;
    s2 = wave_sum(s2) / (float)H;
#pragma unroll
    for (int j = 0; j < LN_MAXV; ++j) {
      int q = lane + 64 * j;
      if (q < H4) {
        f32x4 o;
#pragma unroll
        for (int e = 0; e < 4; ++e) o[e] = rs * (dg[j][e] - s1 - xh[j][e] * s2);
        if (dres) o += reinterpret_cast<const f32x4*>(dres + (size_t)row * H)[q];
        reinterpret_cast<f32x4*>(dx + (size_t)row * H)[q] = o;
      }
    }
  }
#pragma unroll
  for (int j = 0; j < LN_MAXV; ++j) {
    int q = lane + 64 * j;
    if (q < H4) {
#pragma unroll
      for (int e = 0; e < 4; ++e) {
        atomicAdd(&lds[q * 4 + e], ag[j][e]);
        atomicAdd(&lds[H + q * 4 + e], ab[j][e]);
      }
    }
  }
  __syncthreads();
  if (!dgamma) return;
  for (int i = threadIdx.x; i < H; i += blockDim.x) {
    atomicAdd(&dgamma[i], lds[i]);
    atomicAdd(&dbeta[i], lds[H + i]);
  }
}

__global__ void embed_fwd_kernel(const long long* __restrict__ ids, const long long* __restrict__ seg,
                                 const float* __restrict__ word, const float* __restrict__ pos,
                                 const float* __restrict__ type, const float* __restrict__ gamma,
                                 const float* __restrict__ beta, const float* __restrict__ vis,
                                 float* __restrict__ out, float* __restrict__ xhat_out,
                                 float* __restrict__ rstd_out, int B, int T, int H, int num_vis,
                                 float eps, float drop_p, uint32_t seed) {
  const int lane = threadIdx.x & 63;
  const int row = blockIdx.x * (blockDim.x >> 6) + (threadIdx.x >> 6);
  if (row >= B * T) return;
  const int b = row / T, t = row - b * T;
  const int H4 = H / 4;
  if (t < num_vis) {
    for (int q = lane; q < H4; q += 64)
      reinterpret_cast<f32x4*>(out + (size_t)row * H)[q] =
          reinterpret_cast<const f32x4*>(vis + ((size_t)t * B + b) * H)[q];
    return;
  }
  const long long id = ids[row], sg = seg[row];
  f32x4 v[LN_MAXV];
  float s = 0.f;
#pragma unroll
  for (int j = 0; j < LN_MAXV; ++j) {
    int q = lane + 64 * j;
    v[j] = f32x4{0, 0, 0, 0};
    if (q < H4) {
      f32x4 w = reinterpret_cast<const f32x4*>(word + (size_t)id * H)[q];
      f32x4 ty = reinterpret_cast<const f32x4*>(type + (size_t)sg * H)[q];
      f32x4 p = reinterpret_cast<const f32x4*>(pos + (size_t)t * H)[q];
#pragma unroll
      for (int e = 0; e < 4; ++e) v[j][e] = (w[e] + ty[e]) + p[e];
      s += v[j][0] + v[j][1] + v[j][2] + v[j][3];
    }
  }
  float mean = wave_sum(s) / (float)H;
  float ss = 0.f;
#pragma unroll
  for (int j = 0; j < LN_MAXV; ++j) {
    int q = lane + 64 * j;
    if (q < H4) {
#pragma unroll
      for (int e = 0; e < 4; ++e) { float d = v[j][e] - mean; ss += d * d; }
    }
  }
  float rstd = 1.0f / sqrtf(wave_sum(ss) / (float)H + eps);
  const float ks = drop_p > 0.f ? 1.0f / (1.0f - drop_p) : 1.f;
#pragma unroll
  for (int j = 0; j < LN_MAXV; ++j) {
    int q = lane + 64 * j;
    if (q < H4) {
      f32x4 g = reinterpret_cast<const f32x4*>(gamma)[q], be = reinterpret_cast<const f32x4*>(beta)[q], o, xh;
#pragma unroll
      for (int e = 0; e < 4; ++e) {
        xh[e] = (v[j][e] - mean) * rstd;
        o[e] = xh[e] * g[e] + be[e];
        if (drop_p > 0.f) {
          float u = rng_uniform(seed, (uint32_t)row * (uint32_t)H + q * 4 + e);
          o[e] = (u >= drop_p) ? o[e] * ks : 0.f;
        }
      }
      reinterpret_cast<f32x4*>(out + (size_t)row * H)[q] = o;
      if (xhat_out) reinterpret_cast<f32x4*>(xhat_out + (size_t)row * H)[q] = xh;
    }
  }
  if (lane == 0 && rstd_out) rstd_out[row] = rstd;
}

__global__ void embed_bwd_kernel(const float* __restrict__ dout, const long long* __restrict__ ids,
                                 const long long* __restrict__ seg, const float* __restrict__ xhat,
                                 const float* __restrict__ rstd, const float* __restrict__ gamma,
                                 float* __restrict__ dword, float* __restrict__ dpos, float* __restrict__ dtype,
                                 float* __restrict__ dgamma, float* __restrict__ dbeta, float* __restrict__ dvis,
                                 int B, int T, int H, int num_vis, float drop_p, uint32_t seed, int pad_idx) {
  const int lane = threadIdx.x & 63;
  const int row = blockIdx.x * (blockDim.x >> 6) + (threadIdx.x >> 6);
  if (row >= B * T) return;
  const int b = row / T, t = row - b * T;
  const int H4 = H / 4;
  if (t < num_vis) {
    for (int q = lane; q < H4; q += 64)
      reinterpret_cast<f32x4*>(dvis + ((size_t)t * B + b) * H)[q] =
          reinterpret_cast<const f32x4*>(dout + (size_t)row * H)[q];
    return;
  }
  const long long id = ids[row], sg = seg[row];
  const float rs = rstd[row];
  const float ks = drop_p > 0.f ? 1.0f / (1.0f - drop_p) : 1.f;
  f32x4 xh[LN_MAXV], dg[LN_MAXV];
  float s1 = 0.f, s2 = 0.f;
#pragma unroll
  for (int j = 0; j < LN_MAXV; ++j) {
    int q = lane + 64 * j;
    xh[j] = f32x4{0, 0, 0, 0}; dg[j] = f32x4{0, 0, 0, 0};
    if (q < H4) {
      f32x4 d = reinterpret_cast<const f32x4*>(dout + (size_t)row * H)[q];
      xh[j] = reinterpret_cast<const f32x4*>(xhat + (size_t)row * H)[q];
      f32x4 g = reinterpret_cast<const f32x4*>(gamma)[q];
#pragma unroll
      for (int e = 0; e < 4; ++e) {
        if (drop_p > 0.f) {
          float u = rng_uniform(seed, (uint32_t)row * (uint32_t)H + q * 4 + e);
          d[e] = (u >= drop_p) ? d[e] * ks : 0.f;
        }
        atomicAdd(&dgamma[q * 4 + e], d[e] * xh[j][e]);
        atomicAdd(&dbeta[q * 4 + e], d[e]);
        dg[j][e] = d[e] * g[e];
        s1 += dg[j][e];
        s2 += dg[j][e] * xh[j][e];
      }
    }
  }
  s1 = wave_sum(s1) / (float)H;
  s2 = wave_sum(s2) / (float)H;
#pragma unroll
  for (int j = 0; j < LN_MAXV; ++j) {
    int q = lane + 64 * j;
    if (q < H4) {
#pragma unroll
      for (int e = 0; e < 4; ++e) {
        float de = rs * (dg[j][e] - s1 - xh[j][e] * s2);
        if (id != pad_idx) atomicAdd(&dword[(size_t)id * H + q * 4 + e], de);
        atomicAdd(&dtype[(size_t)sg * H + q * 4 + e], de);
        atomicAdd(&dpos[(size_t)t * H + q * 4 + e], de);
      }
    }
  }
}

__global__ void meanpool_fwd_kernel(const float* __restrict__ h, const long long* __restrict__ mask,
                                    float* __restrict__ out, int B, int T, int H) {
  int b = blockIdx.x;
  float cnt = 0.f;
  for (int t = 0; t < T; ++t) cnt += (float)mask[b * T + t];
  float denom = fmaxf(cnt, 1e-9f);
  for (int c = threadIdx.x; c < H; c += blockDim.x) {
    float s = 0.f;
    for (int t = 0; t < T; ++t) s += h[((size_t)b * T + t) * H + c] * (float)mask[b * T + t];
    out[(size_t)b * H + c] = s / denom;
  }
}
__global__ void meanpool_bwd_kernel(const float* __restrict__ dout, const long long* __restrict__ mask,
                                    float* __restrict__ dh, int B, int T, int H, int accumulate) {
  int b = blockIdx.x;
  float cnt = 0.f;
  for (int t = 0; t < T; ++t) cnt += (float)mask[b * T + t];
  float denom = fmaxf(cnt, 1e-9f);
  for (int i = threadIdx.x; i < T * H; i += blockDim.x) {
    int t = i / H, c = i - t * H;
    float v = dout[(size_t)b * H + c] * (float)mask[b * T + t] / denom;
    size_t o = ((size_t)b * T + t) * H + c;
    dh[o] = accumulate ? dh[o] + v : v;
  }
}

__global__ void lsm_nll_kernel(const float* __restrict__ logits, int ld, const long long* __restrict__ target,
                               float* __restrict__ row_loss, float* __restrict__ row_lse,
                               long long* __restrict__ pred,
                               float* __restrict__ dlogits, int dld, const float* __restrict__ gscale_ptr,
                               float gscale_mul, int V) {
  __shared__ float red_m[4], red_s[4];
  __shared__ int red_i[4];
  const int row = blockIdx.x;
  const float* x = logits + (size_t)row * ld;
  const int lane = threadIdx.x & 63, wave = threadIdx.x >> 6;
  float m = -INFINITY; int mi = 0x7fffffff;
  for (int i = threadIdx.x; i < V; i += blockDim.x) {
    float v = x[i];
    if (v > m) { m = v; mi = i; }
  }
#pragma unroll
  for (int o = 32; o > 0; o >>= 1) {
    float om = __shfl_xor(m, o, 64); int oi = __shfl_xor(mi, o, 64);
    if (om > m || (om == m && oi < mi)) { m = om; mi = oi; }
  }
  if (lane == 0) { red_m[wave] = m; red_i[wave] = mi; }
  __syncthreads();
  m = red_m[0]; mi = red_i[0];
  for (int w = 1; w < 4; ++w) if (red_m[w] > m || (red_m[w] == m && red_i[w] < mi)) { m = red_m[w]; mi = red_i[w]; }
  float s = 0.f;
  for (int i = threadIdx.x; i < V; i += blockDim.x) s += expf(x[i] - m);
  s = wave_sum(s);
  if (lane == 0) red_s[wave] = s;
  __syncthreads();
  s = red_s[0] + red_s[1] + red_s[2] + red_s[3];
  const float lse = m + logf(s);
  const long long tg = target[row];
  if (threadIdx.x == 0) {
    row_loss[row] = lse - x[tg];
    if (row_lse) row_lse[row] = lse;
    pred[row] = mi;
  }
  if (dlogits) {
    const float gs = (gscale_ptr ? *gscale_ptr : 1.0f) * gscale_mul;
    float* d = dlogits + (size_t)row * dld;
    for (int i = threadIdx.x; i < V; i += blockDim.x) {
      float pr = expf(x[i] - lse);
      d[i] = (pr - (i == tg ? 1.f : 0.f)) * gs;
    }
  }
}

#define LSM_U 4
__device__ __forceinline__ void lsm_combine(float& m, int& mi, float& s, float om, int oi, float os) {
  const float M = fmaxf(m, om);
  const float sa = (m == -INFINITY) ? 0.f : s * expf(m - M);
  const float sb = (om == -INFINITY) ? 0.f : os * expf(om - M);
  if (om > m || (om == m && oi < mi)) mi = oi;
  m = M; s = sa + sb;
}
__global__ void __launch_bounds__(1024) lsm_stats_kernel(const float* __restrict__ logits, int ld,
                                                         const long long* __restrict__ target,
                                                         float* __restrict__ row_loss, float* __restrict__ row_lse,
                                                         long long* __restrict__ pred, int V) {
  __shared__ float red_m[16], red_s[16];
  __shared__ int red_i[16];
  const int row = blockIdx.x;
  const float* x = logits + (size_t)row * ld;
  const f32x4* x4 = reinterpret_cast<const f32x4*>(x);
  const int nvec = (V + 3) >> 2, lane = threadIdx.x & 63, wave = threadIdx.x >> 6;
  float m = -INFINITY, s = 0.f; int mi = 0x7fffffff;
  for (int j0 = threadIdx.x; j0 < nvec; j0 += 1024 * LSM_U) {
    f32x4 v[LSM_U];
#pragma unroll
    for (int u = 0; u < LSM_U; ++u) {
      const int j = j0 + u * 1024;
      v[u] = (j < nvec) ? x4[j] : f32x4{-INFINITY, -INFINITY, -INFINITY, -INFINITY};
    }
    float cm = m;
#pragma unroll
    for (int u = 0; u < LSM_U; ++u) {
      const int base = (j0 + u * 1024) * 4;
#pragma unroll
      for (int e = 0; e < 4; ++e) {
        if (base + e >= V) v[u][e] = -INFINITY;
        if (v[u][e] > cm) { cm = v[u][e]; mi = base + e; }
      }
    }
    if (cm > -INFINITY) {
      float acc = 0.f;
#pragma unroll
      for (int u = 0; u < LSM_U; ++u)
#pragma unroll
        for (int e = 0; e < 4; ++e) acc += __expf(v[u][e] - cm);
      s = (m == -INFINITY ? 0.f : s * expf(m - cm)) + acc;
      m = cm;
    }
  }
#pragma unroll
  for (int o = 32; o > 0; o >>= 1) {
    const float om = __shfl_xor(m, o, 64), os = __shfl_xor(s, o, 64);
    const int oi = __shfl_xor(mi, o, 64);
    lsm_combine(m, mi, s, om, oi, os);
  }
  if (lane == 0) { red_m[wave] = m; red_i[wave] = mi; red_s[wave] = s; }
  __syncthreads();
  if (threadIdx.x == 0) {
    for (int w = 1; w < 16; ++w) lsm_combine(m, mi, s, red_m[w], red_i[w], red_s[w]);
    const float lse = m + logf(s);
    row_lse[row] = lse;
    row_loss[row] = lse - x[target[row]];
    pred[row] = mi;
  }
}
__global__ void __launch_bounds__(256) lsm_grad_kernel(const float* __restrict__ logits, int ld,
                                                       const long long* __restrict__ target,
                                                       const float* __restrict__ row_lse, float* __restrict__ dlogits,
                                                       int dld, const float* __restrict__ gscale_ptr, float gscale_mul,
                                                       int V) {
  const int row = blockIdx.x;
  const f32x4* x4 = reinterpret_cast<const f32x4*>(logits + (size_t)row * ld);
  f32x4* d4 = reinterpret_cast<f32x4*>(dlogits + (size_t)row * dld);
  const int nvec = (V + 3) >> 2;
  const float lse = row_lse[row];
  const int tg = (int)target[row];
  const float gs = (gscale_ptr ? *gscale_ptr : 1.0f) * gscale_mul;
  const int j0 = blockIdx.y * 256 * LSM_U + threadIdx.x;
  f32x4 v[LSM_U];
// ... 16 lines not shown
  }
}

__global__ void mlm_reduce_kernel(const float* __restrict__ row_loss, const long long* __restrict__ pred,
                                  const long long* __restrict__ target, int rows, float* __restrict__ out3) {
  float s = 0.f, nm = 0.f, nc = 0.f;
  for (int i = threadIdx.x; i < rows; i += blockDim.x) {
    s += row_loss[i];
    if (target[i] > 0) { nm += 1.f; if (pred[i] == target[i]) nc += 1.f; }
  }
  __shared__ float red[3][4];
  s = wave_sum(s); nm = wave_sum(nm); nc = wave_sum(nc);
  int lane = threadIdx.x & 63, wave = threadIdx.x >> 6;
  if (lane == 0) { red[0][wave] = s; red[1][wave] = nm; red[2][wave] = nc; }
  __syncthreads();
  if (threadIdx.x == 0) {
    out3[0] = (red[0][0] + red[0][1] + red[0][2] + red[0][3]) / (float)rows;
    out3[1] = red[1][0] + red[1][1] + red[1][2] + red[1][3];
    out3[2] = red[2][0] + red[2][1] + red[2][2] + red[2][3];
  }
}

__global__ void asl_kernel(const float* __restrict__ logits, int ld, const long long* __restrict__ target,
                           float* __restrict__ row_loss, float* __restrict__ dlogits, int dld, int C,
                           float gpos, float gneg, float eps, float gscale) {
  __shared__ float red[4];
  __shared__ float bc;
  const int row = blockIdx.x;
  const float* x = logits + (size_t)row * ld;
  const int lane = threadIdx.x & 63, wave = threadIdx.x >> 6;
  const int tg = (int)target[row];
  float m = -INFINITY;
  for (int i = threadIdx.x; i < C; i += blockDim.x) m = fmaxf(m, x[i]);
  m = wave_max(m);
  if (lane == 0) red[wave] = m;
  __syncthreads();
  m = fmaxf(fmaxf(red[0], red[1]), fmaxf(red[2], red[3]));
  __syncthreads();
  float s = 0.f;
  for (int i = threadIdx.x; i < C; i += blockDim.x) s += expf(x[i] - m);
  s = wave_sum(s);
  if (lane == 0) red[wave] = s;
  __syncthreads();
  const float lse = m + logf(red[0] + red[1] + red[2] + red[3]);
  __syncthreads();
  float loss = 0.f, gsum = 0.f;
  const float tsm_o = eps / (float)C;
  for (int i = threadIdx.x; i < C; i += blockDim.x) {
    float lp = x[i] - lse, p = expf(lp);
    bool is_t = (i == tg);
    float ts = (is_t ? (1.f - eps) : 0.f) + tsm_o;
    float base = is_t ? (1.f - p) : p;
    float gam = is_t ? gpos : gneg;
    float w = (gam == 0.f) ? 1.f : powf(base, gam);
    loss += -ts * w * lp;
    float dw = (gam == 0.f) ? 0.f : gam * powf(base, gam - 1.f) * (is_t ? -p : p);
    float G = -ts * (w + lp * dw);
    gsum += G;
    if (dlogits) dlogits[(size_t)row * dld + i] = G;
  }
  loss = wave_sum(loss); gsum = wave_sum(gsum);
  if (lane == 0) red[wave] = loss;
  __syncthreads();
  if (threadIdx.x == 0) row_loss[row] = red[0] + red[1] + red[2] + red[3];
  __syncthreads();
  if (lane == 0) red[wave] = gsum;
  __syncthreads();
  if (threadIdx.x == 0) bc = red[0] + red[1] + red[2] + red[3];
  __syncthreads();
  if (dlogits) {
    const float gs = bc;
    for (int i = threadIdx.x; i < C; i += blockDim.x) {
      float p = expf(x[i] - lse);
      size_t o = (size_t)row * dld + i;
      dlogits[o] = (dlogits[o] - p * gs) * gscale;
    }
  }
}

__global__ void l2norm_fwd_kernel(const float* __restrict__ x, float* __restrict__ y, float* __restrict__ nrm,
                                  int rows, int D) {
  int row = blockIdx.x * (blockDim.x >> 6) + (threadIdx.x >> 6), lane = threadIdx.x & 63;
  if (row >= rows) return;
  float s = 0.f;
  for (int i = lane; i < D; i += 64) { float v = x[(size_t)row * D + i]; s += v * v; }
  float n = fmaxf(sqrtf(wave_sum(s)), 1e-12f);
  for (int i = lane; i < D; i += 64) y[(size_t)row * D + i] = x[(size_t)row * D + i] / n;
  if (lane == 0) nrm[row] = n;
}
__global__ void l2norm_bwd_kernel(const float* __restrict__ dy, const float* __restrict__ y,
                                  const float* __restrict__ nrm, float* __restrict__ dx, int rows, int D) {
  int row = blockIdx.x * (blockDim.x >> 6) + (threadIdx.x >> 6), lane = threadIdx.x & 63;
  if (row >= rows) return;
  float s = 0.f;
  for (int i = lane; i < D; i += 64) s += dy[(size_t)row * D + i] * y[(size_t)row * D + i];
  s = wave_sum(s);
  float n = nrm[row];
  for (int i = lane; i < D; i += 64)
    dx[(size_t)row * D + i] = (dy[(size_t)row * D + i] - y[(size_t)row * D + i] * s) / n;
}

template <int U>
__global__ void adam_kernel(float* __restrict__ p, float* __restrict__ g, float* __restrict__ m,
                            float* __restrict__ v, long n4, float step_size, float b1, float omb1, float b2,
                            float omb2, float eps, float bc2_sqrt, float gscale, int zero_grad) {
  const long stride = (long)gridDim.x * blockDim.x;
  const float inv_bc2 = 1.0f / bc2_sqrt;
  auto upd = [&](f32x4& pv, const f32x4& gv, f32x4& mv, f32x4& vv) __attribute__((always_inline)) {
#pragma clang fp contract(off)
#pragma unroll
    for (int e = 0; e < 4; ++e) {
      const float gg = gv[e] * gscale;
      mv[e] = fmaf(gg - mv[e], omb1, mv[e]);
      vv[e] = fmaf(gg * gg, omb2, vv[e] * b2);
      const float denom = sqrtf(vv[e]) / bc2_sqrt + eps;
      pv[e] = fmaf(-step_size, mv[e] / denom, pv[e]);
    }
  };
  (void)inv_bc2;
  f32x4* P4 = reinterpret_cast<f32x4*>(p); f32x4* G4 = reinterpret_cast<f32x4*>(g);
  f32x4* M4 = reinterpret_cast<f32x4*>(m); f32x4* V4 = reinterpret_cast<f32x4*>(v);
  const f32x4 zero = {0, 0, 0, 0};
  long i = (long)blockIdx.x * blockDim.x + threadIdx.x;
  for (; i + (U - 1) * stride < n4; i += U * stride) {
    f32x4 pv[U], gv[U], mv[U], vv[U];
#pragma unroll
    for (int u = 0; u < U; ++u) {
      const long j = i + u * stride;
      pv[u] = P4[j]; gv[u] = G4[j]; mv[u] = __builtin_nontemporal_load(M4 + j); vv[u] = __builtin_nontemporal_load(V4 + j);
    }
#pragma unroll
    for (int u = 0; u < U; ++u) upd(pv[u], gv[u], mv[u], vv[u]);
#pragma unroll
    for (int u = 0; u < U; ++u) {
      const long j = i + u * stride;
      P4[j] = pv[u]; __builtin_nontemporal_store(mv[u], M4 + j); __builtin_nontemporal_store(vv[u], V4 + j);
      if (zero_grad) G4[j] = zero;
    }
  }
  for (; i < n4; i += stride) {
    f32x4 p0 = P4[i], g0 = G4[i], m0 = M4[i], v0 = V4[i];
    upd(p0, g0, m0, v0);
    P4[i] = p0; M4[i] = m0; V4[i] = v0;
    if (zero_grad) G4[i] = zero;
  }
}

__global__ void axpy_kernel(float* __restrict__ y, const float* __restrict__ x, float a, long n) {
  long i = (long)blockIdx.x * blockDim.x + threadIdx.x;
  long stride = (long)gridDim.x * blockDim.x;
  for (; i < n; i += stride) y[i] += a * x[i];
}

__global__ void colsum_kernel(const float* __restrict__ x, int ld, int rows, int cols, float* __restrict__ out) {
  int c = blockIdx.x * blockDim.x + threadIdx.x;
  if (c >= cols) return;
  int r0 = blockIdx.y * 64, r1 = min(rows, r0 + 64);
  float s = 0.f;
  for (int r = r0; r < r1; ++r) s += x[(size_t)r * ld + c];
  atomicAdd(&out[c], s);
}

__global__ void dropout_kernel(float* __restrict__ x, long n, float p, uint32_t seed) {
  long i = (long)blockIdx.x * blockDim.x + threadIdx.x;
  long stride = (long)gridDim.x * blockDim.x;
  const float ks = 1.0f / (1.0f - p);
  for (; i < n; i += stride) x[i] = (rng_uniform(seed, (uint32_t)i) >= p) ? x[i] * ks : 0.f;
}

__global__ void dropout_copy_kernel(const float* __restrict__ x, float* __restrict__ y, long n, float p,
                                    uint32_t seed) {
  long i = (long)blockIdx.x * blockDim.x + threadIdx.x;
  long stride = (long)gridDim.x * blockDim.x;
  const float ks = 1.0f / (1.0f - p);
  for (; i < n; i += stride) y[i] = (rng_uniform(seed, (uint32_t)i) >= p) ? x[i] * ks : 0.f;
}

static inline int grid_for(long n, int block = 256, int cap = 2048) {
  long g = (n + block - 1) / block;
  if (g > cap) g = cap;
  if (g < 1) g = 1;
  return (int)g;
}

int k_bn_coef_fwd(hipStream_t st, const double* stat, int C, double count, float eps, const float* gamma,
                  const float* beta, float* run_mean, float* run_var, long long* nbt, float momentum, int reps,
                  int training, float* scale, float* shift, float* mean, float* invstd) {
  hipLaunchKernelGGL(bn_coef_fwd_kernel, dim3(cdiv_i(C, 16)), dim3(256), 0, st, stat, C, count, eps, gamma, beta,
                     run_mean, run_var, nbt, pow(1.0 - (double)momentum, (double)reps), reps, training, scale, shift,
                     mean, invstd);
  KERNEL_CHECK_RET();
  return MMVQA_OK;
}

template <int PRE, int POST>
__global__ __launch_bounds__(256) void bn_add_relu_fold_kernel(const float* __restrict__ z, const BnFold f3,
                                                               const float* __restrict__ idn, const BnFold fd, int has_d,
                                                               float* __restrict__ out, long rows, int C, int rpw) {
  __shared__ float cs[4][64];
  const int tid = threadIdx.x, c0 = blockIdx.y * 64;
  const bool pub = blockIdx.x == 0;
  if (tid < 64) {
    float a = 0.f, b = 0.f;
    if (c0 + tid < C) bn_fold_fwd(f3, C, c0 + tid, pub && f3.publish, a, b);
    cs[0][tid] = a; cs[1][tid] = b;
  } else if (tid < 128) {
    float a = 1.f, b = 0.f;
    if (has_d && c0 + tid - 64 < C) bn_fold_fwd(fd, C, c0 + tid - 64, pub && fd.publish, a, b);
    cs[2][tid - 64] = a; cs[3][tid - 64] = b;
  }
  if (pub && blockIdx.y == 0) {
    if (tid == 0 && f3.publish && f3.nbt) *f3.nbt += f3.reps;
    if (tid == 64 && has_d && fd.publish && fd.nbt) *fd.nbt += fd.reps;
  }
  __syncthreads();
  const int q = tid & 15, rl = tid >> 4;
  const int c = c0 + q * 4;
  if (c >= C) return;
  const f32x4 s3 = *reinterpret_cast<const f32x4*>(&cs[0][q * 4]), b3 = *reinterpret_cast<const f32x4*>(&cs[1][q * 4]);
  const f32x4 sd = *reinterpret_cast<const f32x4*>(&cs[2][q * 4]), bd = *reinterpret_cast<const f32x4*>(&cs[3][q * 4]);
  const long r0 = (long)blockIdx.x * rpw, r1 = r0 + rpw < rows ? r0 + rpw : rows;
  const f32x4 zero = {0, 0, 0, 0};
  for (long r = r0 + rl; r < r1; r += 32) {
    const long i0 = r * C + c, i1 = (r + 16) * C + c;
    const bool two = r + 16 < r1;
    const f32x4 z0 = *reinterpret_cast<const f32x4*>(z + i0), d0 = idn ? *reinterpret_cast<const f32x4*>(idn + i0) : zero;
    f32x4 z1 = z0, d1 = d0;
    if (two) { z1 = *reinterpret_cast<const f32x4*>(z + i1); if (idn) d1 = *reinterpret_cast<const f32x4*>(idn + i1); }
    f32x4 o0, o1;
#pragma unroll
    for (int j = 0; j < 4; ++j) {
      const float t0 = act_fwd(PRE, z0[j] * s3[j] + b3[j]) + (d0[j] * sd[j] + bd[j]);
      const float t1 = act_fwd(PRE, z1[j] * s3[j] + b3[j]) + (d1[j] * sd[j] + bd[j]);
      o0[j] = act_fwd(POST, t0);
      o1[j] = act_fwd(POST, t1);
    }
    *reinterpret_cast<f32x4*>(out + i0) = o0;
    if (two) *reinterpret_cast<f32x4*>(out + i1) = o1;
  }
}

int k_bn_act_add_fold(hipStream_t st, const float* z, const mmvqa_bn_fold* f3, int pre_act, const float* idn,
                      const mmvqa_bn_fold* fd, int post_act, float* out, long rows, int C) {
  if (C % 4 != 0 || !f3 || !f3->stat || f3->bwd || (fd && (!fd->stat || fd->bwd || !idn)))
    return mmvqa_set_error(MMVQA_ERR_ARG, "bn_act_add_fold: C=%d must be a multiple of 4 and the folds forward ones", C);
  const int cb = cdiv_i(C, 64);
  static const long target = getenv("MMVQA_BAR_WGS") ? atol(getenv("MMVQA_BAR_WGS")) : 4096;
  int rpw = 32;
  while ((long)cdiv_i(rows, rpw) * cb > target && rpw < 1024) rpw *= 2;
  mmvqa_bn_fold none;
  memset(&none, 0, sizeof(none));
  const dim3 grid(cdiv_i(rows, rpw), cb);
#define BAR_GO(PRE_, POST_)                                                                                            \
  hipLaunchKernelGGL((bn_add_relu_fold_kernel<PRE_, POST_>), grid, dim3(256), 0, st, z, *f3, idn, fd ? *fd : none, fd ? 1 : 0, \
                     out, rows, C, rpw)
  if (pre_act == ACT_NONE && post_act == ACT_RELU) BAR_GO(ACT_NONE, ACT_RELU);
  else if (pre_act == ACT_SILU && post_act == ACT_NONE) BAR_GO(ACT_SILU, ACT_NONE);
  else if (pre_act == ACT_NONE && post_act == ACT_NONE) BAR_GO(ACT_NONE, ACT_NONE);
  else return mmvqa_set_error(MMVQA_ERR_ARG, "bn_act_add_fold: activation pair (%d, %d) not built", pre_act, post_act);
#undef BAR_GO
  KERNEL_CHECK_RET();
  return MMVQA_OK;
}

int k_bn_add_relu_fold(hipStream_t st, const float* z, const mmvqa_bn_fold* f3, const float* idn, const mmvqa_bn_fold* fd,
                       float* out, long rows, int C) {
  if (!idn) return mmvqa_set_error(MMVQA_ERR_ARG, "bn_add_relu_fold: no identity tensor");
  return k_bn_act_add_fold(st, z, f3, ACT_NONE, idn, fd, ACT_RELU, out, rows, C);
}

int k_bn_coef_fwd_keep(hipStream_t st, const double* stat, int C, double count, float eps, const float* gamma,
                       const float* beta, float* run_mean, float* run_var, long long* nbt, double keep, int reps,
                       int training, float* scale, float* shift, float* mean, float* invstd) {
  hipLaunchKernelGGL(bn_coef_fwd_kernel, dim3(cdiv_i(C, 16)), dim3(256), 0, st, stat, C, count, eps, gamma, beta,
                     run_mean, run_var, nbt, keep, reps, training, scale, shift, mean, invstd);
  KERNEL_CHECK_RET();
  return MMVQA_OK;
}

int k_bn_coef_bwd(hipStream_t st, const double* stat, int C, double count, const float* gamma, const float* mean,
                  const float* invstd, int training, float* P, float* Q, float* R, float* dgamma, float* dbeta) {
  hipLaunchKernelGGL(bn_coef_bwd_kernel, dim3(cdiv_i(C, 16)), dim3(256), 0, st, stat, C, count, gamma, mean,
                     invstd, training, P, Q, R, dgamma, dbeta);
  KERNEL_CHECK_RET();
  return MMVQA_OK;
}

int k_bn_add_relu(hipStream_t st, const float* z, const float* s, const float* b, const float* idn,
                  const float* ids, const float* idb, float* out, long rows, int C) {
  long n4 = rows * C / 4;
  hipLaunchKernelGGL(bn_add_relu_kernel, dim3(grid_for(n4)), dim3(256), 0, st, z, s, b, idn, ids, idb, out, n4,
                     C / 4);
  KERNEL_CHECK_RET();
  return MMVQA_OK;
}

int k_maxpool_fwd(hipStream_t st, const float* z, const float* s, const float* b, float* out, unsigned char* idx,
                  int N, int H, int W, int C, int OH, int OW) {
  long total = (long)N * OH * OW * C / 4;
  hipLaunchKernelGGL(maxpool_fwd_kernel, dim3(grid_for(total)), dim3(256), 0, st, z, s, b, out, idx, N, H, W, C,
                     OH, OW);
  KERNEL_CHECK_RET();
  return MMVQA_OK;
}

int k_maxpool_bwd(hipStream_t st, const float* gp, const unsigned char* idx, const float* extra, const float* z,
                  const float* s, const float* b, const float* mean, const float* invstd, float* g0, double* stat,
                  int N, int H, int W, int C, int OH, int OW) {
  if (C % 4 != 0 || 256 % (C / 4) != 0)
    return mmvqa_set_error(MMVQA_ERR_ARG, "maxpool_bwd: C/4 must divide 256 (C=%d)", C);
  long total = (long)N * H * W * C / 4;
  hipLaunchKernelGGL(maxpool_bwd_kernel, dim3(grid_for(total, 256, 1024)), dim3(256), 0, st, gp, idx, extra, z, s,
                     b, mean, invstd, g0, stat, N, H, W, C, OH, OW);
  KERNEL_CHECK_RET();
  return MMVQA_OK;
}

int k_layernorm_fwd(hipStream_t st, const float* x, const float* res, const float* gamma, const float* beta,
                    float* y, float* sum_out, float* mean, float* rstd, int rows, int H, float eps) {
  if (H % 4 != 0 || H > 256 * LN_MAXV) return mmvqa_set_error(MMVQA_ERR_ARG, "layernorm: H=%d unsupported", H);
  hipLaunchKernelGGL(layernorm_fwd_kernel, dim3(cdiv_i(rows, 4)), dim3(256), 0, st, x, res, gamma, beta, y,
                     sum_out, mean, rstd, rows, H, eps);
  KERNEL_CHECK_RET();
  return MMVQA_OK;
}

int k_layernorm_bwd(hipStream_t st, const float* dy, const float* x, const float* gamma, const float* mean,
                    const float* rstd, const float* dres, float* dx, float* dgamma, float* dbeta, int rows, int H) {
  if (H % 4 != 0 || H > 256 * LN_MAXV) return mmvqa_set_error(MMVQA_ERR_ARG, "layernorm: H=%d unsupported", H);
  int rpw = rows >= 2048 ? 4 : (rows >= 512 ? 2 : 1);
  int grid = cdiv_i(rows, 4 * rpw);
  hipLaunchKernelGGL(layernorm_bwd_kernel, dim3(grid), dim3(256), 2 * H * sizeof(float), st, dy, x, gamma, mean,
                     rstd, dres, dx, dgamma, dbeta, rows, H, rpw);
  KERNEL_CHECK_RET();
  return MMVQA_OK;
}

int k_embed_fwd(hipStream_t st, const long long* ids, const long long* seg, const float* word, const float* pos,
                const float* type, const float* gamma, const float* beta, const float* vis, float* out,
                float* xhat, float* rstd, int B, int T, int H, int num_vis, float eps, float drop_p,
                uint32_t seed) {
  if (H % 4 != 0 || H > 256 * LN_MAXV) return mmvqa_set_error(MMVQA_ERR_ARG, "embed: H=%d unsupported", H);
  hipLaunchKernelGGL(embed_fwd_kernel, dim3(cdiv_i((long)B * T, 4)), dim3(256), 0, st, ids, seg, word, pos, type,
                     gamma, beta, vis, out, xhat, rstd, B, T, H, num_vis, eps, drop_p, seed);
  KERNEL_CHECK_RET();
  return MMVQA_OK;
}

int k_embed_bwd(hipStream_t st, const float* dout, const long long* ids, const long long* seg, const float* xhat,
                const float* rstd, const float* gamma, float* dword, float* dpos, float* dtype, float* dgamma,
                float* dbeta, float* dvis, int B, int T, int H, int num_vis, float drop_p, uint32_t seed,
                int pad_idx) {
  if (H % 4 != 0 || H > 256 * LN_MAXV) return mmvqa_set_error(MMVQA_ERR_ARG, "embed: H=%d unsupported", H);
  hipLaunchKernelGGL(embed_bwd_kernel, dim3(cdiv_i((long)B * T, 4)), dim3(256), 0, st, dout, ids, seg, xhat, rstd,
                     gamma, dword, dpos, dtype, dgamma, dbeta, dvis, B, T, H, num_vis, drop_p, seed, pad_idx);
  KERNEL_CHECK_RET();
  return MMVQA_OK;
}

int k_meanpool_fwd(hipStream_t st, const float* h, const long long* mask, float* out, int B, int T, int H) {
  hipLaunchKernelGGL(meanpool_fwd_kernel, dim3(B), dim3(256), 0, st, h, mask, out, B, T, H);
  KERNEL_CHECK_RET();
  return MMVQA_OK;
}
int k_meanpool_bwd(hipStream_t st, const float* dout, const long long* mask, float* dh, int B, int T, int H,
                   int accumulate) {
  hipLaunchKernelGGL(meanpool_bwd_kernel, dim3(B), dim3(256), 0, st, dout, mask, dh, B, T, H, accumulate);
  KERNEL_CHECK_RET();
  return MMVQA_OK;
}

static bool lsm_fast_ok(const float* logits, int ld, int V) {
  return ((uintptr_t)logits & 15) == 0 && (ld & 3) == 0 && ld >= ((V + 3) & ~3);
}
int k_lsm_grad(hipStream_t st, const float* logits, int ld, const long long* target, const float* row_lse,
               float* dlogits, int dld, const float* gscale_ptr, float gscale_mul, int rows, int V) {
  if (!lsm_fast_ok(logits, ld, V) || !lsm_fast_ok(dlogits, dld, V))
    return mmvqa_set_error(MMVQA_ERR_ARG, "mlm_grad: logits/dlogits rows must be 16-byte aligned with ld >= round_up(V,4)");
  hipLaunchKernelGGL(lsm_grad_kernel, dim3(rows, cdiv_i((V + 3) >> 2, 256 * LSM_U)), dim3(256), 0, st, logits, ld, target,
                     row_lse, dlogits, dld, gscale_ptr, gscale_mul, V);
  KERNEL_CHECK_RET();
  return MMVQA_OK;
}
int k_lsm_nll(hipStream_t st, const float* logits, int ld, const long long* target, float* row_loss, float* row_lse,
              long long* pred, float* dlogits, int dld, const float* gscale_ptr, float gscale_mul, int rows, int V,
              float* out3) {
  if (row_lse && lsm_fast_ok(logits, ld, V) && (!dlogits || lsm_fast_ok(dlogits, dld, V))) {
    hipLaunchKernelGGL(lsm_stats_kernel, dim3(rows), dim3(1024), 0, st, logits, ld, target, row_loss, row_lse, pred, V);
    KERNEL_CHECK_RET();
    if (dlogits) {
      int r = k_lsm_grad(st, logits, ld, target, row_lse, dlogits, dld, gscale_ptr, gscale_mul, rows, V);
      if (r != MMVQA_OK) return r;
    }
  } else {
    hipLaunchKernelGGL(lsm_nll_kernel, dim3(rows), dim3(256), 0, st, logits, ld, target, row_loss, row_lse, pred,
                       dlogits, dld, gscale_ptr, gscale_mul, V);
    KERNEL_CHECK_RET();
  }
  if (out3) {
    hipLaunchKernelGGL(mlm_reduce_kernel, dim3(1), dim3(256), 0, st, row_loss, pred, target, rows, out3);
    KERNEL_CHECK_RET();
  }
  return MMVQA_OK;
}

int k_asl(hipStream_t st, const float* logits, int ld, const long long* target, float* row_loss, float* dlogits,
          int dld, int rows, int C, float gpos, float gneg, float eps, float gscale) {
  hipLaunchKernelGGL(asl_kernel, dim3(rows), dim3(256), 0, st, logits, ld, target, row_loss, dlogits, dld, C, gpos,
                     gneg, eps, gscale);
  KERNEL_CHECK_RET();
  return MMVQA_OK;
}

int k_l2norm_fwd(hipStream_t st, const float* x, float* y, float* nrm, int rows, int D) {
  hipLaunchKernelGGL(l2norm_fwd_kernel, dim3(cdiv_i(rows, 4)), dim3(256), 0, st, x, y, nrm, rows, D);
  KERNEL_CHECK_RET();
  return MMVQA_OK;
}
int k_l2norm_bwd(hipStream_t st, const float* dy, const float* y, const float* nrm, float* dx, int rows, int D) {
  hipLaunchKernelGGL(l2norm_bwd_kernel, dim3(cdiv_i(rows, 4)), dim3(256), 0, st, dy, y, nrm, dx, rows, D);
  KERNEL_CHECK_RET();
  return MMVQA_OK;
}

int k_adam(hipStream_t st, float* p, float* g, float* m, float* v, long n, double lr, double b1, double b2, double eps,
           int step, float gscale, int zero_grad) {
  if (n % 4 != 0) return mmvqa_set_error(MMVQA_ERR_ARG, "adam: n must be a multiple of 4");
  const double bc1 = 1.0 - pow(b1, (double)step), bc2 = 1.0 - pow(b2, (double)step);
  const char* cap_s = getenv("MMVQA_ADAM_WGS");
  const int cap = cap_s ? atoi(cap_s) : 16384;
  static const int unroll = getenv("MMVQA_ADAM_UNROLL") ? atoi(getenv("MMVQA_ADAM_UNROLL")) : 2;
#define ADAM_GO(U_)                                                                                                       \
  hipLaunchKernelGGL(adam_kernel<U_>, dim3(grid_for(n / 4, 256, cap > 0 ? cap : 16384)), dim3(256), 0, st, p, g, m, v, n / 4, \
                     (float)(lr / bc1), (float)b1, (float)(1.0 - b1), (float)b2, (float)(1.0 - b2), (float)eps,            \
                     (float)sqrt(bc2), gscale, zero_grad)
  if (unroll >= 4) ADAM_GO(4); else if (unroll == 3) ADAM_GO(3); else if (unroll == 1) ADAM_GO(1); else ADAM_GO(2);
#undef ADAM_GO
  KERNEL_CHECK_RET();
  return MMVQA_OK;
}

int k_axpy(hipStream_t st, float* y, const float* x, float a, long n) {
  hipLaunchKernelGGL(axpy_kernel, dim3(grid_for(n)), dim3(256), 0, st, y, x, a, n);
  KERNEL_CHECK_RET();
  return MMVQA_OK;
}

int k_colsum(hipStream_t st, const float* x, int ld, int rows, int cols, float* out) {
  hipLaunchKernelGGL(colsum_kernel, dim3(cdiv_i(cols, 256), cdiv_i(rows, 64)), dim3(256), 0, st, x, ld, rows, cols,
                     out);
  KERNEL_CHECK_RET();
  return MMVQA_OK;
}

int k_dropout(hipStream_t st, float* x, long n, float p, uint32_t seed) {
  hipLaunchKernelGGL(dropout_kernel, dim3(grid_for(n)), dim3(256), 0, st, x, n, p, seed);
  KERNEL_CHECK_RET();
  return MMVQA_OK;
}

__global__ void pixmask_kernel(int* out, int total, int OH, int OW, int SH, int SW, int KH, int KW, int stride, int pad) {
  const int m = blockIdx.x * blockDim.x + threadIdx.x;
  if (m >= total) return;
  const int rem = m % (OH * OW), oy = rem / OW, ox = rem - oy * OW;
  const int y0 = oy * stride - pad, x0 = ox * stride - pad;
  unsigned mk = 0;
  for (int kh = 0; kh < KH; ++kh)
    for (int kw = 0; kw < KW; ++kw)
      if ((unsigned)(y0 + kh) < (unsigned)SH && (unsigned)(x0 + kw) < (unsigned)SW) mk |= 1u << (kh * KW + kw);
  out[m] = (int)mk;
}

int k_pixmask(hipStream_t st, int* out, int N, int OH, int OW, int SH, int SW, int KH, int KW, int stride, int pad) {
  if (KH * KW > 32) return mmvqa_set_error(MMVQA_ERR_ARG, "pixmask: at most 32 taps");
  const int total = N * OH * OW;
  if (total <= 0) return MMVQA_OK;
  hipLaunchKernelGGL(pixmask_kernel, dim3((total + 255) / 256), dim3(256), 0, st, out, total, OH, OW, SH, SW, KH, KW, stride, pad);
  KERNEL_CHECK_RET();
  return MMVQA_OK;
}

int k_dropout_copy(hipStream_t st, const float* x, float* y, long n, float p, uint32_t seed) {
  hipLaunchKernelGGL(dropout_copy_kernel, dim3(grid_for(n)), dim3(256), 0, st, x, y, n, p, seed);
  KERNEL_CHECK_RET();
  return MMVQA_OK;
}


__global__ void bn_act_add_kernel(const float* __restrict__ z, const float* __restrict__ s,
                                  const float* __restrict__ b, int pre_act, const float* __restrict__ idn,
                                  const float* __restrict__ ids, const float* __restrict__ idb, int idn_act,
                                  int post_act, float* __restrict__ out, long n4, int C4) {
  long i = (long)blockIdx.x * blockDim.x + threadIdx.x;
  long stride = (long)gridDim.x * blockDim.x;
  for (; i < n4; i += stride) {
    int c = (int)(i % C4) * 4;
    f32x4 zv = reinterpret_cast<const f32x4*>(z)[i];
    f32x4 sv = *reinterpret_cast<const f32x4*>(s + c), bv = *reinterpret_cast<const f32x4*>(b + c);
    f32x4 o;
#pragma unroll
    for (int j = 0; j < 4; ++j) o[j] = act_fwd(pre_act, zv[j] * sv[j] + bv[j]);
    if (idn) {
      f32x4 iv = reinterpret_cast<const f32x4*>(idn)[i];
      if (ids) {
        f32x4 s2 = *reinterpret_cast<const f32x4*>(ids + c), b2 = *reinterpret_cast<const f32x4*>(idb + c);
#pragma unroll
        for (int j = 0; j < 4; ++j) iv[j] = act_fwd(idn_act, iv[j] * s2[j] + b2[j]);
      }
      o += iv;
    }
#pragma unroll
    for (int j = 0; j < 4; ++j) o[j] = act_fwd(post_act, o[j]);
    reinterpret_cast<f32x4*>(out)[i] = o;
  }
}

__global__ __launch_bounds__(256) void dwconv_fwd_kernel(const float* __restrict__ z1, const float* __restrict__ s1,
                                                        const float* __restrict__ b1, const BnFold f1, const float* __restrict__ w,
                                                        float* __restrict__ z2, double* __restrict__ stat, int N,
                                                        int H, int W, int C, int OH, int OW, int stride, int pad) {
  __shared__ double red[256 * 8];
  const int q = threadIdx.x & 7, pl = threadIdx.x >> 3;
  const int c = blockIdx.y * 32 + q * 4;
  const long npix = (long)N * OH * OW;
  __shared__ __attribute__((aligned(16))) float cf[2][32];
  bn_coef_block_fwd<32>(s1, b1, f1, C, blockIdx.y * 32, f1.publish && blockIdx.x == 0, cf);
  const f32x4 sv = *reinterpret_cast<const f32x4*>(&cf[0][q * 4]), bv = *reinterpret_cast<const f32x4*>(&cf[1][q * 4]);
  if (f1.stat && f1.publish && f1.nbt && blockIdx.x == 0 && blockIdx.y == 0 && threadIdx.x == 0) *f1.nbt += f1.reps;
  f32x4 wv[9];
#pragma unroll
  for (int t = 0; t < 9; ++t)
#pragma unroll
    for (int j = 0; j < 4; ++j) wv[t][j] = w[(size_t)(c + j) * 9 + t];
  double sa[4] = {0, 0, 0, 0}, sb[4] = {0, 0, 0, 0};
  for (long pix = (long)blockIdx.x * 32 + pl; pix < npix; pix += (long)gridDim.x * 32) {
    int ox = (int)(pix % OW); long t = pix / OW;
    int oy = (int)(t % OH), n = (int)(t / OH);
    f32x4 acc = {0, 0, 0, 0};
#pragma unroll
    for (int kh = 0; kh < 3; ++kh) {
      int y = oy * stride - pad + kh;
      if (y < 0 || y >= H) continue;
#pragma unroll
      for (int kw = 0; kw < 3; ++kw) {
        int x = ox * stride - pad + kw;
        if (x < 0 || x >= W) continue;
        f32x4 v = *reinterpret_cast<const f32x4*>(z1 + ((size_t)(n * H + y) * W + x) * C + c);
#pragma unroll
        for (int j = 0; j < 4; ++j) acc[j] += silu_f(v[j] * sv[j] + bv[j]) * wv[kh * 3 + kw][j];
      }
    }
    *reinterpret_cast<f32x4*>(z2 + (size_t)pix * C + c) = acc;
#pragma unroll
    for (int j = 0; j < 4; ++j) { sa[j] += (double)acc[j]; sb[j] += (double)acc[j] * (double)acc[j]; }
  }
  if (stat) {
#pragma unroll
    for (int j = 0; j < 4; ++j) { red[threadIdx.x * 8 + j] = sa[j]; red[threadIdx.x * 8 + 4 + j] = sb[j]; }
    __syncthreads();
    if (threadIdx.x < 32) {
      const int qq = threadIdx.x >> 2, j = threadIdx.x & 3;
      double a0 = 0, a1 = 0;
      for (int r = 0; r < 32; ++r) { a0 += red[(r * 8 + qq) * 8 + j]; a1 += red[(r * 8 + qq) * 8 + 4 + j]; }
      const int slot = blockIdx.x & (MMVQA_STAT_SLOTS - 1);
      double* d = stat + ((size_t)slot * C + blockIdx.y * 32 + qq * 4 + j) * 2;
      atomicAdd(d, a0);
      atomicAdd(d + 1, a1);
    }
  }
}

__global__ __launch_bounds__(256) void dwconv_bwd_data_kernel(
    const float* __restrict__ g2, const float* __restrict__ z2, const float* __restrict__ P, const float* __restrict__ Q,
    const float* __restrict__ R, const float* __restrict__ w, const float* __restrict__ z1, const float* __restrict__ s1,
    const float* __restrict__ b1, const float* __restrict__ mean1, const float* __restrict__ invstd1,
    float* __restrict__ g1, double* __restrict__ stat, int N, int H, int W, int C, int OH, int OW, int stride, int pad,
    const BnFold f2) {
  __shared__ double red[256 * 8];
  __shared__ __attribute__((aligned(16))) float cf[3][32];
  const int q = threadIdx.x & 7, pl = threadIdx.x >> 3;
  const int c = blockIdx.y * 32 + q * 4;
  const long npix = (long)N * H * W;
  bn_coef_block_bwd<32>(P, Q, R, f2, C, blockIdx.y * 32, f2.publish && blockIdx.x == 0, cf);
  f32x4 sv = *reinterpret_cast<const f32x4*>(s1 + c), bv = *reinterpret_cast<const f32x4*>(b1 + c);
  f32x4 mu = *reinterpret_cast<const f32x4*>(mean1 + c), is = *reinterpret_cast<const f32x4*>(invstd1 + c);
  f32x4 Pv = *reinterpret_cast<const f32x4*>(&cf[0][q * 4]), Qv = *reinterpret_cast<const f32x4*>(&cf[1][q * 4]),
        Rv = *reinterpret_cast<const f32x4*>(&cf[2][q * 4]);
  f32x4 wv[9];
#pragma unroll
  for (int t = 0; t < 9; ++t)
#pragma unroll
    for (int j = 0; j < 4; ++j) wv[t][j] = w[(size_t)(c + j) * 9 + t];
  double sa[4] = {0, 0, 0, 0}, sb[4] = {0, 0, 0, 0};
  for (long pix = (long)blockIdx.x * 32 + pl; pix < npix; pix += (long)gridDim.x * 32) {
    int x = (int)(pix % W); long t = pix / W;
    int y = (int)(t % H), n = (int)(t / H);
    f32x4 acc = {0, 0, 0, 0};
#pragma unroll
    for (int kh = 0; kh < 3; ++kh) {
      int ty = y + pad - kh;
      if (ty < 0 || ty % stride) continue;
      int oy = ty / stride;
      if (oy >= OH) continue;
// ... 531 lines not shown
```

### mm-vqa_amd/csrc/engine.cpp

```cpp
#include "engine.h"

#include <cmath>
#include <cstdarg>
#include <cstdio>
#include <cstring>

static thread_local char g_err[1024] = "";
int mmvqa_set_error(int code, const char* fmt, ...) {
  va_list ap;
  va_start(ap, fmt);
  vsnprintf(g_err, sizeof(g_err), fmt, ap);
  va_end(ap);
  return code;
}
const char* mmvqa_get_error() { return g_err; }

#define TRY(x)                    \
  do {                            \
    int _r = (x);                 \
    if (_r != MMVQA_OK) return _r; \
  } while (0)

namespace {

// ... 423 lines not shown
  for (int pass = 0; pass < 2; ++pass) {
    const bool bw = pass == 1;
    take(e->stem_bn, bw);
    for (auto& blk : e->blocks) { take(blk.b1, bw); take(blk.b2, bw); take(blk.b3, bw); if (blk.has_ds) take(blk.bd, bw); }
    for (auto& blk : e->eff) { take(blk.b_a, bw); if (blk.type == 2) take(blk.b_dw, bw); if (blk.type != 0) take(blk.b_p, bw); }
  }
  const size_t half = sd / 2;
  if (sd != 2 * half) { mmvqa_set_error(MMVQA_ERR_STATE, "plan: stat zone mismatch"); return 0; }
  e->statzone_floats = sd * 2;
  a.f(e->statzone_floats);
  e->ws_floats = (a.cur + 63) & ~(size_t)63;
  e->planned = true;
  e->bound = false;
  return e->ws_floats * sizeof(float);
}

#define WS(off) (e->ws + (off))
#define PRM(off) (e->params + (off))
#define GRD(off) (e->grads + (off))
static inline double* stat_ptr(mmvqa_engine* e, size_t doff) {
  return reinterpret_cast<double*>(e->ws + e->statzone) + doff;
}

static int prof_begin(mmvqa_engine* e, hipStream_t st, int cls, double flops, int tag = HB_NONE, double bytes = 0.0) {
  if (!e->prof_on) return MMVQA_OK;
  mmvqa_engine::ProfRec r;
  HIP_CHECK_RET(hipEventCreate(&r.a));
  HIP_CHECK_RET(hipEventCreate(&r.b));
  r.cls = cls; r.reg = e->prof_reg; r.flops = flops; r.tag = tag != HB_NONE ? tag : e->prof_tag; r.bytes = bytes;
  HIP_CHECK_RET(hipEventRecord(r.a, st));
  e->prof.push_back(r);
  return MMVQA_OK;
}
static int prof_end(mmvqa_engine* e, hipStream_t st) {
  if (!e->prof_on) return MMVQA_OK;
  HIP_CHECK_RET(hipEventRecord(e->prof.back().b, st));
  return MMVQA_OK;
}
struct RegScope {
  mmvqa_engine* e; int old;
  RegScope(mmvqa_engine* e_, int r) : e(e_), old(e_->prof_reg) { e->prof_reg = r; }
  ~RegScope() { e->prof_reg = old; }
};
#define REG(r) RegScope _reg_scope(e, r)
#define RUNB_ON(s, tag, bytes, call)                             \
  do {                                                           \
    TRY(prof_begin(e, s, PROF_OTHER, 0, tag, (double)(bytes)));  \
    TRY(call);                                                   \
    TRY(prof_end(e, s));                                         \
  } while (0)
#define RUN_ON(s, cls, flops, call)    \
  do {                                 \
    TRY(prof_begin(e, s, cls, flops)); \
    TRY(call);                         \
    TRY(prof_end(e, s));               \
  } while (0)
#define RUNB(tag, bytes, call) RUNB_ON(st, tag, bytes, call)
#define RUN(cls, flops, call) RUN_ON(st, cls, flops, call)

static GemmParams gp_linear_geom() {
  GemmParams g;
  memset(&g, 0, sizeof(g));
  g.g_SH = g.g_SW = g.g_OH = g.g_OW = 1;
  g.g_KH = g.g_KW = 1; g.g_stride = 1; g.g_pad = 0;
  return g;
}

static void set_sk(mmvqa_engine* e, hipStream_t st, GemmParams& g) {
  static const bool off = getenv("MMVQA_NO_SK_WS") != nullptr;
  if (off) return;
  const int which = (e->side && st == e->side) ? 1 : ((e->side2 && st == e->side2) ? 2 : 0);
  g.sk_ws = WS(e->sk_ws[which]);
  g.sk_ws_floats = (long long)SK_WS_FLOATS;
  g.sk_cnt = reinterpret_cast<unsigned int*>(WS(e->sk_cnt[which]));
  g.sk_cnt_n = SK_CNT_N;
}

struct EpiOpt {
  const float* R = nullptr; int r_ld = 0;
  const float* Mk = nullptr; int mk_ld = 0; const float* mk_s = nullptr; const float* mk_b = nullptr; int mk_mode = 0;
  BNRef* st1 = nullptr; const float* Z1 = nullptr;
  BNRef* st2 = nullptr; const float* Z2 = nullptr;
};

static void apply_epi(mmvqa_engine* e, GemmParams& g, const EpiOpt& o) {
  g.R = o.R; g.r_ld = o.r_ld;
  g.Mk = o.Mk; g.mk_ld = o.mk_ld; g.mk_s = o.mk_s; g.mk_b = o.mk_b; g.mk_mode = o.mk_mode;
  if (o.st1) {
    g.stat1 = stat_ptr(e, o.st1->stat_b); g.stat_bwd = 1; g.stat_slots = o.st1->slots;
    g.Z1 = o.Z1; g.z1_ld = o.st1->C; g.mean1 = WS(o.st1->mean); g.invstd1 = WS(o.st1->invstd);
  }
  if (o.st2) {
    g.stat2 = stat_ptr(e, o.st2->stat_b);
    g.Z2 = o.Z2; g.z2_ld = o.st2->C; g.mean2 = WS(o.st2->mean); g.invstd2 = WS(o.st2->invstd);
  }
}

static int lin_fwd(mmvqa_engine* e, hipStream_t st, const float* x, int x_ld, long M, const LinRef& L, float* y,
                   int y_ld, int act, float* pre, float drop_p, uint32_t seed, const float* R, int r_ld) {
  GemmParams g = gp_linear_geom();
  g.M = (int)M; g.N = L.out; g.K = L.in;
  g.A = x; g.a_ld = x_ld; g.g_Cs = L.in;
  g.B = PRM(L.w); g.b_ld = L.in;
  g.C = y; g.c_ld = y_ld; g.Cpre = pre;
  g.bias = L.b >= 0 ? PRM(L.b) : nullptr;
  g.act = act; g.drop_p = drop_p; g.drop_seed = seed; g.R = R; g.r_ld = r_ld;
  set_sk(e, st, g);
  RUN(PROF_IGEMM, 2.0 * M * L.out * L.in, mmvqa_launch_igemm(g, KIND_FWD, 0, 0, st));
  return MMVQA_OK;
}

static int lin_dgrad(mmvqa_engine* e, hipStream_t st, const float* dy, int dy_ld, long M, const LinRef& L, float* dx,
                     int dx_ld, int dact, const float* Pre, int pre_ld, float* colsum, const float* R, int r_ld) {
  GemmParams g = gp_linear_geom();
  g.M = (int)M; g.N = L.in; g.K = L.out;
  g.A = dy; g.a_ld = dy_ld; g.g_Cs = L.out;
  g.B = PRM(L.w); g.b_ld = L.in; g.b_tapstride = 0;
  g.C = dx; g.c_ld = dx_ld;
  g.dact = dact; g.Pre = Pre; g.pre_ld = pre_ld; g.colsum = colsum; g.R = R; g.r_ld = r_ld;
  const long tiles = ((M + 63) / 64) * ((L.in + 63) / 64);
  if (!dact && !colsum && !R && tiles < 256 && L.out >= 1536 && L.out <= 8192 && dx_ld == L.in) {
    int sk = (int)((512 + tiles - 1) / tiles);
    const int maxs = (L.out / 64) / 8;
    if (sk > maxs) sk = maxs;
    if (sk > 1) {
      HIP_CHECK_RET(hipMemsetAsync(dx, 0, sizeof(float) * (size_t)M * dx_ld, st));
      g.c_atomic = 1; g.splitk = sk;
    }
  }
  set_sk(e, st, g);
  RUN(PROF_IGEMM, 2.0 * M * L.out * L.in, mmvqa_launch_igemm(g, KIND_DGRAD, 0, 0, st));
  return MMVQA_OK;
}

static int lin_wgrad(mmvqa_engine* e, hipStream_t st, const float* dy, int dy_ld, const float* x, int x_ld, long M,
                     const LinRef& L, bool bias_from_colsum) {
  GemmParams g = gp_linear_geom();
  g.M = L.out; g.N = L.in; g.K = (int)M;
  g.A = dy; g.a_ld = dy_ld;
  g.B = x; g.b_ld = x_ld; g.g_Cs = L.in;
  g.C = GRD(L.w); g.c_ld = L.in; g.c_atomic = 1;
  RUN(PROF_IGEMM, 2.0 * M * L.out * L.in, mmvqa_launch_igemm(g, KIND_WGRAD, 0, 0, st));
  if (bias_from_colsum && L.b >= 0) RUN(PROF_OTHER, 0, k_colsum(st, dy, dy_ld, (int)M, L.out, GRD(L.b)));
  return MMVQA_OK;
}

static int ln_fwd(mmvqa_engine* e, hipStream_t st, const float* x, const LNRef& ln, float* y, float* mean,
                  float* rstd, long rows, float eps) {
  RUNB(HB_LAYERNORM_FWD, 8.0 * rows * e->d.hidden, k_layernorm_fwd(st, x, nullptr, PRM(ln.g), PRM(ln.b), y, nullptr, mean, rstd, (int)rows,
                                     e->d.hidden, eps));
  return MMVQA_OK;
}
static int ln_bwd(mmvqa_engine* e, hipStream_t st, const float* dy, const float* x, const LNRef& ln,
                  const float* mean, const float* rstd, const float* dres, float* dx, long rows, bool data_only = false) {
  RUNB(HB_LAYERNORM_BWD, (dres ? 16.0 : 12.0) * rows * e->d.hidden, k_layernorm_bwd(st, dy, x, PRM(ln.g), mean, rstd, dres, dx,
                                     data_only ? nullptr : GRD(ln.g), data_only ? nullptr : GRD(ln.b), (int)rows,
                                     e->d.hidden));
  return MMVQA_OK;
}

static void conv_geom(GemmParams& g, const ConvRef& c, int SH, int SW, int Cs, int OH, int OW) {
  g.g_SH = SH; g.g_SW = SW; g.g_Cs = Cs; g.g_OH = OH; g.g_OW = OW;
  g.g_KH = g.g_KW = c.KH; g.g_stride = c.stride; g.g_pad = c.pad;
}

static int bn_coef_fwd(mmvqa_engine* e, hipStream_t st, BNRef& bn) {
  REG(REG_BNCOEF);
  RUN(PROF_OTHER, 0,
      k_bn_coef_fwd(st, stat_ptr(e, bn.stat_f), bn.C, bn.count, bn.eps, PRM(bn.gamma), PRM(bn.beta),
                    e->bufs + bn.rmean, e->bufs + bn.rvar, e->nbt + bn.nbt, 0.1f, bn.reps, e->training,
                    WS(bn.scale), WS(bn.shift), WS(bn.mean), WS(bn.invstd)));
  return MMVQA_OK;
}
static int bn_coef_bwd(mmvqa_engine* e, hipStream_t st, BNRef& bn) {
  REG(REG_BNCOEF);
  RUN(PROF_OTHER, 0,
      k_bn_coef_bwd(st, stat_ptr(e, bn.stat_b), bn.C, bn.count, PRM(bn.gamma), WS(bn.mean), WS(bn.invstd),
                    e->training, WS(bn.P), WS(bn.Q), WS(bn.R), GRD(bn.gamma), GRD(bn.beta)));
  return MMVQA_OK;
}

static inline bool folding(const mmvqa_engine* e) { return e->bn_fold && e->training && e->d.cnn == 0; }
static inline bool eff_folding(const mmvqa_engine* e) { return e->bn_fold && e->training && e->d.cnn != 0; }

static void set_fold_fwd(mmvqa_engine* e, mmvqa_bn_fold& f, BNRef& bn) {
  memset(&f, 0, sizeof(f));
  f.stat = stat_ptr(e, bn.stat_f); f.slots = bn.slots; f.bwd = 0; f.publish = 1; f.reps = bn.reps;
  f.count = bn.count; f.keep = pow(1.0 - (double)0.1f, (double)bn.reps); f.eps = bn.eps;
  f.gamma = PRM(bn.gamma); f.beta = PRM(bn.beta);
  f.out0 = WS(bn.scale); f.out1 = WS(bn.shift); f.out2 = WS(bn.mean); f.out3 = WS(bn.invstd);
  f.run_mean = e->bufs + bn.rmean; f.run_var = e->bufs + bn.rvar; f.nbt = e->nbt + bn.nbt;
}
static void set_fold_bwd(mmvqa_engine* e, mmvqa_bn_fold& f, const BNRef& bn, bool publish) {
  memset(&f, 0, sizeof(f));
  f.stat = stat_ptr(e, bn.stat_b); f.slots = bn.slots; f.bwd = 1; f.publish = publish ? 1 : 0; f.reps = bn.reps;
  f.count = bn.count; f.keep = 1.0; f.eps = bn.eps;
  f.gamma = PRM(bn.gamma); f.mean = WS(bn.mean); f.invstd = WS(bn.invstd);
  f.out0 = WS(bn.P); f.out1 = WS(bn.Q); f.out2 = WS(bn.R);
  f.dgamma = GRD(bn.gamma); f.dbeta = GRD(bn.beta);
}

struct ConvIn {
  const BNRef* bn = nullptr;
  int pro = 0;
  const float* gate = nullptr;
  int gate_hw(int OH, int OW) const { return bn && pro != PRO_AFFINE_RELU ? OH * OW : 0; }
};

static int conv_fwd(mmvqa_engine* e, hipStream_t st, const ConvRef& c, const float* x, const ConvIn& in, int N,
                    int H, int W, int OH, int OW, float* z, BNRef& bn_out, bool coef = true) {
  GemmParams g;
  memset(&g, 0, sizeof(g));
  g.M = N * OH * OW; g.N = c.Cout; g.K = c.KH * c.KH * c.Cin;
  g.A = x; g.a_ld = c.Cin;
  if (in.bn) {
    g.a_pro = in.pro; g.a_c0 = WS(in.bn->scale); g.a_c1 = WS(in.bn->shift);
    g.gate = in.gate; g.gate_hw = in.gate_hw(OH, OW);
    if (folding(e)) set_fold_fwd(e, g.a_fold, *const_cast<BNRef*>(in.bn));
  }
  conv_geom(g, c, H, W, c.Cin, OH, OW);
  g.B = PRM(c.w); g.b_ld = g.K;
  g.C = z; g.c_ld = c.Cout;
  if (e->training) { g.stat1 = stat_ptr(e, bn_out.stat_f); g.stat_bwd = 0; g.stat_slots = bn_out.slots; }
  set_sk(e, st, g);
  RUN(PROF_IGEMM, 2.0 * g.M * g.N * g.K, mmvqa_launch_igemm(g, KIND_FWD, 0, 0, st));
  return folding(e) || !coef ? MMVQA_OK : bn_coef_fwd(e, st, bn_out);
}

static int conv_wgrad(mmvqa_engine* e, hipStream_t st, const ConvRef& c, const float* G, const float* z,
                      const BNRef& bn_out, const float* x, const ConvIn& in, int N, int H, int W, int OH, int OW) {
  GemmParams g;
  memset(&g, 0, sizeof(g));
  g.M = c.Cout; g.N = c.KH * c.KH * c.Cin; g.K = N * OH * OW;
  g.A = G; g.A2 = z; g.a_ld = c.Cout; g.a_pro = PRO_DZ;
  g.a_c0 = WS(bn_out.P); g.a_c1 = WS(bn_out.Q); g.a_c2 = WS(bn_out.R);
  if (folding(e)) set_fold_bwd(e, g.a_fold, bn_out, false);
  g.B = x; g.b_ld = c.Cin;
  if (in.bn) {
    g.b_pro = in.pro; g.b_c0 = WS(in.bn->scale); g.b_c1 = WS(in.bn->shift);
    g.gate = in.gate; g.gate_hw = in.gate_hw(OH, OW);
  }
  conv_geom(g, c, H, W, c.Cin, OH, OW);
  g.C = GRD(c.w); g.c_ld = g.N; g.c_atomic = 1;
  if (c.KH > 1 && c.stride == 1 && OH == H && OW == W) {
    char key[96];
    snprintf(key, sizeof(key), "%d,%d,%d,%d,%d", N, OH, OW, c.KH, c.pad);
    auto it = e->pixmask_off.find(key);
    if (it != e->pixmask_off.end()) g.pixmask = reinterpret_cast<int*>(WS(it->second.off));
  }
  RUN(PROF_IGEMM, 2.0 * (double)g.M * g.N * g.K, mmvqa_launch_igemm(g, KIND_WGRAD, 0, 0, st));
  return MMVQA_OK;
}

static int conv_dgrad(mmvqa_engine* e, hipStream_t st, const ConvRef& c, const float* G, const float* z,
                      const BNRef& bn_out, int N, int H, int W, int OH, int OW, float* dx, const EpiOpt& o) {
  GemmParams g;
  memset(&g, 0, sizeof(g));
  g.M = N * H * W; g.N = c.Cin; g.K = c.KH * c.KH * c.Cout;
  g.A = G; g.A2 = z; g.a_ld = c.Cout; g.a_pro = PRO_DZ;
  g.a_c0 = WS(bn_out.P); g.a_c1 = WS(bn_out.Q); g.a_c2 = WS(bn_out.R);
  if (folding(e)) set_fold_bwd(e, g.a_fold, bn_out, true);
  conv_geom(g, c, OH, OW, c.Cout, H, W);
  g.B = PRM(c.w); g.b_ld = c.KH * c.KH * c.Cin; g.b_tapstride = c.Cin;
  g.C = dx; g.c_ld = c.Cin;
  apply_epi(e, g, o);
  set_sk(e, st, g);
  RUN(PROF_IGEMM, 2.0 * (double)N * OH * OW * c.Cout * c.KH * c.KH * c.Cin,
      mmvqa_launch_igemm(g, KIND_DGRAD, 0, 0, st));
  return MMVQA_OK;
}

static GemmParams stem_desc(mmvqa_engine* e, int kind, const float* g0 = nullptr) {
  const ConvRef& c = e->stem_conv;
  const int pixels = e->B * e->SH * e->SW, taps = c.KH * c.KH * c.Cin;
  GemmParams g;
  memset(&g, 0, sizeof(g));
  g.g_nchw = 1;
  conv_geom(g, c, e->IH, e->IW, c.Cin, e->SH, e->SW);
  if (kind == KIND_FWD) {
    g.M = pixels; g.N = c.Cout; g.K = taps;
    g.A = e->img;
    g.B = PRM(c.w); g.b_ld = taps;
    g.C = WS(e->z0); g.c_ld = c.Cout;
    if (e->training) g.stat1 = stat_ptr(e, e->stem_bn.stat_f);
  } else {
    g.M = c.Cout; g.N = taps; g.K = pixels;
    g.A = g0; g.A2 = WS(e->z0); g.a_ld = c.Cout; g.a_pro = PRO_DZ;
    g.a_c0 = WS(e->stem_bn.P); g.a_c1 = WS(e->stem_bn.Q); g.a_c2 = WS(e->stem_bn.R);
    g.B = e->img;
    g.C = GRD(c.w); g.c_ld = taps; g.c_atomic = 1;
  }
  return g;
}

static int tap_act(const mmvqa_engine* e) { return e->d.use_relu ? ACT_RELU : ACT_SERF; }

static bool tap_is_thin(const mmvqa_engine* e, const TapRef& t) {
  static const bool thin_off = getenv("MMVQA_NO_TAP_THIN") != nullptr;
  return !thin_off && e->prec == MMVQA_PREC_F32 && t.C <= 32 && k_tap_thin_ok(t.M, e->d.hidden, t.C, t.HW);
}

static GemmParams tap_desc(mmvqa_engine* e, hipStream_t st, const TapRef& t, const float* fmap, const BNRef* bn_in, int epi_mode) {
  GemmParams g = gp_linear_geom();
  g.M = (int)t.M; g.N = e->d.hidden; g.K = t.C;
  g.A = fmap; g.a_ld = t.C; g.g_Cs = t.C;
  if (bn_in) { g.a_pro = PRO_AFFINE_RELU; g.a_c0 = WS(bn_in->scale); g.a_c1 = WS(bn_in->shift); }
  g.B = PRM(t.w); g.b_ld = t.C;
  g.epi_mode = epi_mode; g.act = tap_act(e); g.tap_HW = t.HW;
  g.c_ld = g.N;
  set_sk(e, st, g);
// ... 428 lines not shown
    if (i < 0) return;
    EffBlock& pb = e->eff[i];
    if (pb.type != 0) { o.st1 = &pb.b_p; o.Z1 = WS(pb.zp); }
  };
  int cur = 0;
  {
    EpiOpt o;
    producer_opts(nb - 1, o);
    TRY(tap_bwd(e, st, 4, WS(e->eff[nb - 1].out), nullptr, WS(e->gbuf[cur]), o));
  }
  TRY(scx.fork());
  for (auto& b : e->eff)
    if (b.feature >= 0 && b.feature < 4) {
      TRY(tap_bwd(e, sd, b.feature, WS(b.out), nullptr, WS(e->tapgrad[b.feature]), EpiOpt()));
      TRY(scx.mark(&ev_tap[b.feature]));
    }
  for (int i = nb - 1; i >= 0; --i) {
    EffBlock& b = e->eff[i];
    const float* G = WS(e->gbuf[cur]);
    const float* x = i == 0 ? WS(e->eff_a0) : WS(e->eff[i - 1].out);
    float* Gprev = WS(e->gbuf[cur ^ 1]);
    const float* extra = (i > 0 && e->eff[i - 1].feature >= 0) ? WS(e->tapgrad[e->eff[i - 1].feature]) : nullptr;
    if (extra && b.skip) return mmvqa_set_error(MMVQA_ERR_STATE, "effnet_backward: tap gradient into a skip block");
    const long Min = (long)B * b.H * b.W, Mout = (long)B * b.OH * b.OW;
    const int pi = i & 1;
    float* gA = WS(e->eff_gA[pi]);
    float* gB = WS(e->eff_gB[pi]);
    const float* dz_first = nullptr;
    if (b.type == 0) {
      TRY(scx.need(ev_gA[pi]));
      RUNB(HB_ACT_BWD_STATS, 12.0 * Mout * b.cout, k_act_bwd_stats(st, G, nullptr, nullptr, WS(b.za), WS(b.b_a.scale), WS(b.b_a.shift),
                                         WS(b.b_a.mean), WS(b.b_a.invstd), ACT_SILU, gA, stat_ptr(e, b.b_a.stat_b), Mout,
                                         b.OH * b.OW, b.cout));
      dz_first = gA;
    } else if (b.type == 1) {
      TRY(bn_coef_bwd(e, st, b.b_p));
      TRY(scx.fork());
      TRY(conv_wgrad(e, sd, b.c_p, G, WS(b.zp), b.b_p, WS(b.za), {&b.b_a, PRO_AFFINE_SILU}, B, b.OH, b.OW, b.OH, b.OW));
      TRY(scx.mark(&ev_G[cur]));
      TRY(scx.need(ev_gA[pi]));
      EpiOpt o;
      o.Mk = WS(b.za); o.mk_ld = b.mid; o.mk_s = WS(b.b_a.scale); o.mk_b = WS(b.b_a.shift); o.mk_mode = 1;
      o.st1 = &b.b_a; o.Z1 = WS(b.za);
      TRY(conv_dgrad(e, st, b.c_p, G, WS(b.zp), b.b_p, B, b.OH, b.OW, b.OH, b.OW, gA, o));
      dz_first = gA;
    } else {
      TRY(bn_coef_bwd(e, st, b.b_p));
      TRY(scx.fork());
      TRY(conv_wgrad(e, sd, b.c_p, G, WS(b.zp), b.b_p, WS(b.zdw), {&b.b_dw, PRO_SILU_GATE, WS(b.gate)}, B, b.OH, b.OW, b.OH, b.OW));
      TRY(scx.mark(&ev_G[cur]));
      TRY(scx.need(ev_gA[pi]));
      TRY(conv_dgrad(e, st, b.c_p, G, WS(b.zp), b.b_p, B, b.OH, b.OW, b.OH, b.OW, gA, EpiOpt()));
      float* dgate = WS(e->eff_se[0]); float* dpool = WS(e->eff_se[3]);
      RUNB(HB_SE_DGATE, 8.0 * Mout * b.mid, k_se_dgate(st, gA, WS(b.zdw), WS(b.b_dw.scale), WS(b.b_dw.shift), dgate, B, b.OH * b.OW, b.mid,
                                    WS(e->eff_separt), B * b.rd));
      RUN(PROF_MATRIX, 8.0 * B * b.mid * b.rd, k_se_fc_bwd(st, dgate, WS(b.gpre), WS(b.r), WS(b.rpre), WS(b.pool), PRM(b.se_e.w), PRM(b.se_r.w),
                                     GRD(b.se_e.w), GRD(b.se_e.b), GRD(b.se_r.w), GRD(b.se_r.b), dpool,
                                     WS(e->eff_separt), 1, B, b.mid, b.rd));
      TRY(scx.need(ev_gB[pi]));
      RUNB(HB_ACT_BWD_STATS, 12.0 * Mout * b.mid, k_act_bwd_stats(st, gA, WS(b.gate), dpool, WS(b.zdw), WS(b.b_dw.scale), WS(b.b_dw.shift),
                                         WS(b.b_dw.mean), WS(b.b_dw.invstd), ACT_SILU, gB, stat_ptr(e, b.b_dw.stat_b), Mout,
                                         b.OH * b.OW, b.mid));
      mmvqa_bn_fold fdw_w, fdw_d;
      if (fold) { set_fold_bwd(e, fdw_w, b.b_dw, false); set_fold_bwd(e, fdw_d, b.b_dw, true); }
      else TRY(bn_coef_bwd(e, st, b.b_dw));
      TRY(scx.fork());
      RUNB_ON(sd, HB_DWCONV_BWD_WEIGHT, 4.0 * (2.0 * Mout + (double)Min) * b.mid, k_dwconv_bwd_weight(sd, gB, WS(b.zdw), WS(b.b_dw.P), WS(b.b_dw.Q), WS(b.b_dw.R), WS(b.za),
                                           WS(b.b_a.scale), WS(b.b_a.shift), GRD(b.dw_w), B, b.H, b.W, b.mid, b.OH, b.OW,
                                           b.stride, b.pad, fold ? &fdw_w : nullptr));
      TRY(scx.mark(&ev_gB[pi]));
      RUNB(HB_DWCONV_BWD_DATA, 4.0 * (2.0 * Mout + 2.0 * (double)Min) * b.mid, k_dwconv_bwd_data(st, gB, WS(b.zdw), WS(b.b_dw.P), WS(b.b_dw.Q), WS(b.b_dw.R), PRM(b.dw_w),
                                           WS(b.za), WS(b.b_a.scale), WS(b.b_a.shift), WS(b.b_a.mean), WS(b.b_a.invstd), gA,
                                           stat_ptr(e, b.b_a.stat_b), B, b.H, b.W, b.mid, b.OH, b.OW, b.stride, b.pad, fold ? &fdw_d : nullptr));
      dz_first = gA;
    }
    TRY(bn_coef_bwd(e, st, b.b_a));
    const int fo_h = b.type == 2 ? b.H : b.OH, fo_w = b.type == 2 ? b.W : b.OW;
    TRY(scx.fork());
    TRY(conv_wgrad(e, sd, b.c_a, dz_first, WS(b.za), b.b_a, x, {}, B, b.H, b.W, fo_h, fo_w));
    TRY(scx.mark(&ev_gA[pi]));
    EpiOpt o;
    producer_opts(i - 1, o);
    if (b.skip) { o.R = G; o.r_ld = b.cin; }
    else if (extra) { o.R = extra; o.r_ld = b.cin; TRY(scx.need(ev_tap[e->eff[i - 1].feature])); }
    TRY(scx.need(ev_G[cur ^ 1]));
    TRY(conv_dgrad(e, st, b.c_a, dz_first, WS(b.za), b.b_a, B, b.H, b.W, fo_h, fo_w, Gprev, o));
    (void)Min;
    cur ^= 1;
    if (i > 0 && (nb - i) % 12 == 0) { TRY(notify(e, scx, b.c_a.w, hi_mark)); hi_mark = b.c_a.w; }
  }
  float* g0 = WS(e->gbuf[cur ^ 1]);
  const long M0 = (long)B * e->SH * e->SW;
  const int C0 = e->stem_conv.Cout;
  TRY(scx.need(ev_G[cur ^ 1]));
  RUNB(HB_ACT_BWD_STATS, 12.0 * M0 * C0, k_act_bwd_stats(st, WS(e->gbuf[cur]), nullptr, nullptr, WS(e->z0), WS(e->stem_bn.scale),
                                     WS(e->stem_bn.shift), WS(e->stem_bn.mean), WS(e->stem_bn.invstd), ACT_SILU, g0,
                                     stat_ptr(e, e->stem_bn.stat_b), M0, e->SH * e->SW, C0));
  TRY(bn_coef_bwd(e, st, e->stem_bn));
  const GemmParams g = stem_desc(e, KIND_WGRAD, g0);
  RUN(PROF_IGEMM, 2.0 * (double)g.M * g.N * g.K, mmvqa_launch_igemm(g, KIND_WGRAD, 1, 0, st));
  TRY(scx.join());
  TRY(notify(e, scx, e->emb_hi, hi_mark));
  return MMVQA_OK;
}

static inline uint32_t site_seed(const mmvqa_engine* e, int layer, int site) {
  return e->seed + 0x9E3779B9u * (uint32_t)(layer * 8 + site + 1);
}

static int attn_call(mmvqa_engine* e, hipStream_t st, AttnParams& a, int head_dim, int bwd) {
  REG(REG_ATTN);
  const double fl = (bwd ? 10.0 : 4.0) * (double)e->B * a.heads * e->T * e->T * head_dim;
  RUN(PROF_ATTN, fl, mmvqa_launch_attention(a, head_dim, bwd, st));
  return MMVQA_OK;
}

static AttnParams bert_attn_desc(mmvqa_engine* e, const BertLayerRef& L, int layer, float p) {
  const int H = e->d.hidden, hd = H / e->d.heads;
  AttnParams a;
  memset(&a, 0, sizeof(a));
  a.q = WS(L.qkvo); a.k = a.q + H; a.v = a.q + 2 * H;
  a.row_stride = 3 * H; a.head_stride = hd;
  a.out = WS(L.ctx); a.out_row_stride = H; a.out_head_stride = hd;
  a.mask = e->mask; a.mask_on_query = 0; a.probs = WS(L.probs);
  a.B = e->B; a.T = e->T; a.heads = e->d.heads; a.sqrt_d = sqrtf((float)hd);
  a.drop_p = p; a.seed = site_seed(e, layer, 0);
  return a;
}
static AttnParams rf_attn_desc(mmvqa_engine* e, const RFLayerRef& L, int layer) {
  const int H = e->d.hidden, es = H / 8;
  AttnParams a;
  memset(&a, 0, sizeof(a));
  a.k = WS(L.kqvo); a.q = a.k + es; a.v = a.k + 2 * es;
  a.row_stride = 8 * 3 * es; a.head_stride = 3 * es;
  a.out = WS(L.res); a.out_row_stride = H; a.out_head_stride = es;
  a.mask = e->mask; a.mask_on_query = 1;
  a.prev_in = layer > 0 ? WS(e->rf[layer - 1].prev) : nullptr;
  a.prev_out = WS(L.prev); a.probs = WS(L.probs);
  a.B = e->B; a.T = e->T; a.heads = 8; a.sqrt_d = sqrtf((float)es);
  return a;
}

static int drop_grad(mmvqa_engine* e, hipStream_t st, SideReads& sr, const float* g, float p, uint32_t seed, const float** out) {
  *out = g;
  if (p > 0.f) {
    const long n = (long)e->B * e->T * e->d.hidden;
    TRY(sr.write(WS(e->t_b)));
    RUNB(HB_DROPOUT_COPY, 8.0 * n, k_dropout_copy(st, g, WS(e->t_b), n, p, seed));
    *out = WS(e->t_b);
  }
  return MMVQA_OK;
}

static int bert_forward(mmvqa_engine* e, hipStream_t st, const float* x_in, const float** x_out) {
  REG(REG_ENC);
  const mmvqa_model_desc& d = e->d;
  const int H = d.hidden;
  const long M = (long)e->B * e->T;
  const float p = e->training ? d.p_drop : 0.f;
  const float* x = x_in;
  for (int i = 0; i < d.n_layers; ++i) {
    BertLayerRef& L = e->bert[i];
    TRY(ln_fwd(e, st, x, e->norm1, WS(L.xn1), WS(L.mean1), WS(L.rstd1), M, 1e-12f));
    static const bool fused_off = getenv("MMVQA_NO_FUSED_QKV") != nullptr;
    if (!fused_off && e->prec == MMVQA_PREC_F32 && k_qkv_attn_fwd_ok(e->T, H, d.heads)) {
      REG(REG_QKV_ATTN);
      RUN(PROF_ATTN, 2.0 * M * 3 * H * H + 4.0 * e->B * d.heads * (double)e->T * e->T * (H / d.heads),
          k_qkv_attn_fwd(st, WS(L.xn1), PRM(L.qkv.w), PRM(L.qkv.b), e->mask, WS(L.qkvo), WS(L.probs), WS(L.ctx), e->B, e->T,
                         H, d.heads, p, site_seed(e, i, 0)));
    } else {
    { REG(REG_QKV); TRY(lin_fwd(e, st, WS(L.xn1), H, M, L.qkv, WS(L.qkvo), 3 * H, ACT_NONE, nullptr, 0.f, 0, nullptr, 0)); }
    AttnParams a = bert_attn_desc(e, L, i, p);
    TRY(attn_call(e, st, a, H / d.heads, 0));
    }
    TRY(lin_fwd(e, st, WS(L.ctx), H, M, L.proj, WS(L.y), H, ACT_NONE, nullptr, p, site_seed(e, i, 1), x, H));
    TRY(ln_fwd(e, st, WS(L.y), e->norm1, WS(L.xn2), WS(L.mean2), WS(L.rstd2), M, 1e-12f));
    TRY(lin_fwd(e, st, WS(L.xn2), H, M, L.fc1, WS(L.h1), 4 * H, ACT_GELU, WS(L.pre1), 0.f, 0, nullptr, 0));
    TRY(lin_fwd(e, st, WS(L.h1), 4 * H, M, L.fc2, WS(L.z), H, ACT_NONE, nullptr, p, site_seed(e, i, 2), WS(L.y), H));
    x = WS(L.z);
  }
  *x_out = x;
  return MMVQA_OK;
}

static int bert_backward(mmvqa_engine* e, hipStream_t st, const float* x_in, SideReads& sr) {
  REG(REG_ENC);
  const mmvqa_model_desc& d = e->d;
  const int H = d.hidden;
  const long M = (long)e->B * e->T;
  const float p = e->training ? d.p_drop : 0.f;
  float* dz = WS(e->t_a);
  for (int i = d.n_layers - 1; i >= 0; --i) {
    BertLayerRef& L = e->bert[i];
    const float* x = i == 0 ? x_in : WS(e->bert[i - 1].z);
    const float* dzd;
    TRY(drop_grad(e, st, sr, dz, p, site_seed(e, i, 2), &dzd));
    TRY(lin_wgrad_side(e, sr, st, dzd, H, WS(L.h1), 4 * H, M, L.fc2, true));
    TRY(sr.write(WS(e->t_big)));
    TRY(lin_dgrad(e, st, dzd, H, M, L.fc2, WS(e->t_big), 4 * H, ACT_GELU, WS(L.pre1), 4 * H, sr.bias_grad(GRD(L.fc1.b)), nullptr, 0));
    TRY(lin_wgrad_side(e, sr, st, WS(e->t_big), 4 * H, WS(L.xn2), H, M, L.fc1, false));
    TRY(sr.write(WS(e->t_c)));
    TRY(lin_dgrad(e, st, WS(e->t_big), 4 * H, M, L.fc1, WS(e->t_c), H, 0, nullptr, 0, nullptr, nullptr, 0));
    TRY(sr.write(WS(e->t_d)));
    TRY(ln_bwd(e, st, WS(e->t_c), WS(L.y), e->norm1, WS(L.mean2), WS(L.rstd2), dz, WS(e->t_d), M, sr.data_only));
    float* dy = WS(e->t_d);
    const float* dyd;
    TRY(drop_grad(e, st, sr, dy, p, site_seed(e, i, 1), &dyd));
    TRY(lin_wgrad_side(e, sr, st, dyd, H, WS(L.ctx), H, M, L.proj, true));
    TRY(sr.write(WS(e->t_c)));
    TRY(lin_dgrad(e, st, dyd, H, M, L.proj, WS(e->t_c), H, 0, nullptr, 0, nullptr, nullptr, 0));
    AttnParams a = bert_attn_desc(e, L, i, p);
    a.dout = WS(e->t_c);
    float* dqkv = WS(e->t_big);
    a.dq = dqkv; a.dk = dqkv + H; a.dv = dqkv + 2 * H;
    TRY(sr.write(dqkv));
    TRY(attn_call(e, st, a, H / d.heads, 1));
    { REG(REG_QKV);
      TRY(lin_wgrad_side(e, sr, st, dqkv, 3 * H, WS(L.xn1), H, M, L.qkv, true));
      TRY(sr.write(WS(e->t_c)));
      TRY(lin_dgrad(e, st, dqkv, 3 * H, M, L.qkv, WS(e->t_c), H, 0, nullptr, 0, nullptr, nullptr, 0)); }
    TRY(sr.write(dz));
    TRY(ln_bwd(e, st, WS(e->t_c), x, e->norm1, WS(L.mean1), WS(L.rstd1), dy, dz, M, sr.data_only));
  }
  return MMVQA_OK;
}

static int rf_forward(mmvqa_engine* e, hipStream_t st, const float* x_in, const float** x_out) {
  REG(REG_ENC);
  const mmvqa_model_desc& d = e->d;
  const int H = d.hidden, es = H / 8;
  const long M = (long)e->B * e->T;
  const float p = e->training ? d.p_rf_drop : 0.f;
  const float* x = x_in;
  for (int i = 0; i < d.n_layers; ++i) {
    RFLayerRef& L = e->rf[i];
    { REG(REG_QKV); TRY(lin_fwd(e, st, x, es, M * 8, L.kqv, WS(L.kqvo), 3 * es, ACT_NONE, nullptr, 0.f, 0, nullptr, 0)); }
    AttnParams a = rf_attn_desc(e, L, i);
    TRY(attn_call(e, st, a, es, 0));
    TRY(lin_fwd(e, st, WS(L.res), H, M, L.proj, WS(L.s1), H, ACT_NONE, nullptr, p, site_seed(e, i, 1), x, H));
    TRY(ln_fwd(e, st, WS(L.s1), L.ln1, WS(L.x1), WS(L.mean1), WS(L.rstd1), M, 1e-5f));
    TRY(lin_fwd(e, st, WS(L.x1), H, M, L.ff0, WS(L.hact), 4 * H, ACT_SERF, WS(L.pre), 0.f, 0, nullptr, 0));
    TRY(lin_fwd(e, st, WS(L.hact), 4 * H, M, L.ff2, WS(L.s2), H, ACT_NONE, nullptr, p, site_seed(e, i, 2), WS(L.x1), H));
    TRY(ln_fwd(e, st, WS(L.s2), L.ln2, WS(L.x2), WS(L.mean2), WS(L.rstd2), M, 1e-5f));
    x = WS(L.x2);
  }
  *x_out = x;
  return MMVQA_OK;
}

static int rf_backward(mmvqa_engine* e, hipStream_t st, const float* x_in, SideReads& sr) {
  REG(REG_ENC);
  const mmvqa_model_desc& d = e->d;
  const int H = d.hidden, es = H / 8;
  const long M = (long)e->B * e->T;
  const float p = e->training ? d.p_rf_drop : 0.f;
  float* dx2 = WS(e->t_a);
  for (int i = d.n_layers - 1; i >= 0; --i) {
    RFLayerRef& L = e->rf[i];
    const float* x = i == 0 ? x_in : WS(e->rf[i - 1].x2);
    TRY(sr.write(WS(e->t_d)));
    TRY(ln_bwd(e, st, dx2, WS(L.s2), L.ln2, WS(L.mean2), WS(L.rstd2), nullptr, WS(e->t_d), M, sr.data_only));
    float* ds2 = WS(e->t_d);
    const float* dff;
    TRY(drop_grad(e, st, sr, ds2, p, site_seed(e, i, 2), &dff));
    TRY(lin_wgrad_side(e, sr, st, dff, H, WS(L.hact), 4 * H, M, L.ff2, true));
    TRY(sr.write(WS(e->t_big)));
    TRY(lin_dgrad(e, st, dff, H, M, L.ff2, WS(e->t_big), 4 * H, ACT_SERF, WS(L.pre), 4 * H, sr.bias_grad(GRD(L.ff0.b)), nullptr, 0));
    TRY(lin_wgrad_side(e, sr, st, WS(e->t_big), 4 * H, WS(L.x1), H, M, L.ff0, false));
    TRY(sr.write(WS(e->t_c)));
    TRY(lin_dgrad(e, st, WS(e->t_big), 4 * H, M, L.ff0, WS(e->t_c), H, 0, nullptr, 0, nullptr, ds2, H));
    TRY(sr.write(WS(e->t_d)));
    TRY(ln_bwd(e, st, WS(e->t_c), WS(L.s1), L.ln1, WS(L.mean1), WS(L.rstd1), nullptr, WS(e->t_d), M, sr.data_only));
    float* ds1 = WS(e->t_d);
    const float* dr;
    TRY(drop_grad(e, st, sr, ds1, p, site_seed(e, i, 1), &dr));
    TRY(lin_wgrad_side(e, sr, st, dr, H, WS(L.res), H, M, L.proj, false));
    TRY(sr.write(WS(e->t_c)));
    TRY(lin_dgrad(e, st, dr, H, M, L.proj, WS(e->t_c), H, 0, nullptr, 0, nullptr, nullptr, 0));
    AttnParams a = rf_attn_desc(e, L, i);
    a.dout = WS(e->t_c);
    float* dkqv = WS(e->t_big);
    a.dk = dkqv; a.dq = dkqv + es; a.dv = dkqv + 2 * es;
    a.dprev_in = (i < d.n_layers - 1) ? WS(e->t_dprev[(i + 1) & 1]) : nullptr;
    a.dprev_out = i > 0 ? WS(e->t_dprev[i & 1]) : nullptr;
    TRY(sr.write(dkqv));
    TRY(attn_call(e, st, a, es, 1));
    { REG(REG_QKV);
      TRY(lin_wgrad_side(e, sr, st, dkqv, 3 * es, x, es, M * 8, L.kqv, false));
      TRY(sr.write(dx2));
      TRY(lin_dgrad(e, st, dkqv, 3 * es, M * 8, L.kqv, dx2, es, 0, nullptr, 0, nullptr, ds1, es)); }
  }
  return MMVQA_OK;
}

static inline int fb_windows(int T) { return (T + 1) / 2; }
static inline int fb_tokens(int T, int w) { return 2 * w + 1 < T ? 2 : 1; }

static void fb_attn_fill(mmvqa_engine* e, const FBLayerRef& L, int layer, int w, int n, float p, mmvqa_fb_attn_desc& a) {
  const size_t r0 = (size_t)w * 2 * e->B;
  memset(&a, 0, sizeof(a));
  a.q = WS(L.q) + r0 * 512; a.q_ld = 512;
  a.mem_k = WS(e->fb_mem); a.mem_v = a.mem_k + 512; a.mem_win = (long long)2 * e->B * 1024; a.mem_ld = 1024;
  if (n == 2) { a.self_k = WS(L.kv) + r0 * 1024; a.self_v = a.self_k + 512; a.self_ld = 1024; }
  a.bias = PRM(e->fb_rel);
  a.probs = WS(L.probs) + (size_t)w * e->B * 8 * 2 * e->T; a.p_ld = e->T;
  a.out = WS(L.ctx) + r0 * 512; a.out_ld = 512;
  a.B = e->B; a.n = n; a.n_mem = 2 * w; a.T = e->T;
  a.scale = 0.125f;
  a.drop_p = p; a.seed = site_seed(e, layer, 0);
}
static int fb_attn_call(mmvqa_engine* e, hipStream_t st, const mmvqa_fb_attn_desc& a, int bwd) {
  REG(REG_ATTN);
  const double fl = (bwd ? 10.0 : 4.0) * (double)a.B * 8 * a.n * (a.n_mem + (a.n == 2 ? 2 : 0)) * 64;
  RUN(PROF_ATTN, fl, k_fb_attention(st, a, bwd));
  return MMVQA_OK;
}

static int fb_forward(mmvqa_engine* e, hipStream_t st, const float* x_in, const float** x_out) {
  REG(REG_ENC);
  const mmvqa_model_desc& d = e->d;
  const int H = d.hidden, B = e->B, T = e->T, NL = d.n_layers, nwin = fb_windows(T);
  const size_t M = (size_t)B * T;
  const float p = e->training ? d.p_fb_drop : 0.f;
  RUN(PROF_OTHER, 0, k_fb_reorder(st, x_in, WS(e->fb_hid), B, T, H, 1));
  for (int w = 0; w < nwin; ++w) {
    const int n = fb_tokens(T, w);
    const long Mw = (long)n * B;
    const size_t r0 = (size_t)w * 2 * B;
    for (int i = 0; i < NL; ++i) {
      FBLayerRef& L = e->fb[i];
      const float* x = WS(e->fb_hid) + i * M * H + r0 * H;
      TRY(ln_fwd(e, st, x, L.ln_a, WS(L.xn_a) + r0 * H, WS(L.mean_a) + r0, WS(L.rstd_a) + r0, Mw, 1e-5f));
      { REG(REG_QKV);
        TRY(lin_fwd(e, st, WS(L.xn_a) + r0 * H, H, Mw, L.to_q, WS(L.q) + r0 * 512, 512, ACT_NONE, nullptr, 0.f, 0, nullptr, 0));
        if (n == 2)
          TRY(lin_fwd(e, st, WS(L.xn_a) + r0 * H, H, Mw, e->fb_kv, WS(L.kv) + r0 * 1024, 1024, ACT_NONE, nullptr, 0.f, 0, nullptr, 0)); }
      mmvqa_fb_attn_desc a;
      fb_attn_fill(e, L, i, w, n, p, a);
      TRY(fb_attn_call(e, st, a, 0));
      TRY(lin_fwd(e, st, WS(L.ctx) + r0 * 512, 512, Mw, L.to_out, WS(L.xmid) + r0 * H, H, ACT_NONE, nullptr, 0.f, 0, x, H));
      TRY(ln_fwd(e, st, WS(L.xmid) + r0 * H, L.ln_f, WS(L.xn_f) + r0 * H, WS(L.mean_f) + r0, WS(L.rstd_f) + r0, Mw, 1e-5f));
      TRY(lin_fwd(e, st, WS(L.xn_f) + r0 * H, H, Mw, L.w1, WS(L.pre) + r0 * 8 * H, 8 * H, ACT_NONE, nullptr, 0.f, 0, nullptr, 0));
      RUN(PROF_OTHER, 0, k_geglu_fwd(st, WS(L.pre) + r0 * 8 * H, WS(L.gg) + r0 * 4 * H, Mw, 4 * H, p, site_seed(e, i, 1),
                                     (uint32_t)(r0 * 4 * H)));
      TRY(lin_fwd(e, st, WS(L.gg) + r0 * 4 * H, 4 * H, Mw, L.w2, WS(e->fb_hid) + (i + 1) * M * H + r0 * H, H, ACT_NONE, nullptr, 0.f,
                  0, WS(L.xmid) + r0 * H, H));
    }
    if (w + 1 < nwin) {
      RUN(PROF_OTHER, 0, k_fb_aggregate_fwd(st, WS(e->fb_hid) + r0 * H, (long long)(M * H), NL + 1, PRM(e->fb_lw),
                                            WS(e->fb_agg) + r0 * H, Mw, H));
      REG(REG_QKV);
      TRY(lin_fwd(e, st, WS(e->fb_agg) + r0 * H, H, Mw, e->fb_kv, WS(e->fb_mem) + r0 * 1024, 1024, ACT_NONE, nullptr, 0.f, 0, nullptr, 0));
    }
  }
  RUN(PROF_OTHER, 0, k_fb_reorder(st, WS(e->fb_hid) + NL * M * H, WS(e->fb_out), B, T, H, 0));
  *x_out = WS(e->fb_out);
  return MMVQA_OK;
}

static int fb_backward(mmvqa_engine* e, hipStream_t st, const float* x_in, SideReads& sr) {
  (void)x_in;
  REG(REG_ENC);
  const mmvqa_model_desc& d = e->d;
  const int H = d.hidden, B = e->B, T = e->T, NL = d.n_layers, nwin = fb_windows(T);
  const size_t M = (size_t)B * T;
  const float p = e->training ? d.p_fb_drop : 0.f;
  float* ghid = WS(e->fb_ghid);
  RUN(PROF_OTHER, 0, k_fb_reorder(st, WS(e->t_a), ghid + NL * M * H, B, T, H, 1));
  HIP_CHECK_RET(hipMemsetAsync(WS(e->fb_dmem), 0, M * 1024 * sizeof(float), st));
  float *s1 = WS(e->fb_s[0]), *s2 = WS(e->fb_s[1]), *s3 = WS(e->fb_s[2]), *s4 = WS(e->fb_s[3]), *s5 = WS(e->fb_s[4]);
  for (int w = nwin - 1; w >= 0; --w) {
    const int n = fb_tokens(T, w);
    const long Mw = (long)n * B;
    const size_t r0 = (size_t)w * 2 * B;
    const bool wrote_mem = w + 1 < nwin;
    if (wrote_mem) {
      { REG(REG_QKV);
        TRY(lin_dgrad(e, st, WS(e->fb_dmem) + r0 * 1024, 1024, Mw, e->fb_kv, s2, H, 0, nullptr, 0, nullptr, nullptr, 0)); }
      RUN(PROF_OTHER, 0, k_fb_aggregate_bwd(st, s2, WS(e->fb_hid) + r0 * H, (long long)(M * H), NL + 1, PRM(e->fb_lw),
                                            WS(e->fb_dhs), (long long)2 * B * H, ghid + NL * M * H + r0 * H,
                                            sr.data_only ? nullptr : GRD(e->fb_lw), Mw, H));
    }
    for (int i = NL - 1; i >= 0; --i) {
      FBLayerRef& L = e->fb[i];
      const float* gout = ghid + (i + 1) * M * H + r0 * H;
      TRY(lin_dgrad(e, st, gout, H, Mw, L.w2, s1, 4 * H, 0, nullptr, 0, nullptr, nullptr, 0));
      RUN(PROF_OTHER, 0, k_geglu_bwd(st, s1, WS(L.pre) + r0 * 8 * H, WS(L.g_pre) + r0 * 8 * H, Mw, 4 * H, p, site_seed(e, i, 1),
                                     (uint32_t)(r0 * 4 * H)));
      TRY(lin_dgrad(e, st, WS(L.g_pre) + r0 * 8 * H, 8 * H, Mw, L.w1, s2, H, 0, nullptr, 0, nullptr, nullptr, 0));
      TRY(ln_bwd(e, st, s2, WS(L.xmid) + r0 * H, L.ln_f, WS(L.mean_f) + r0, WS(L.rstd_f) + r0, gout, WS(L.g_mid) + r0 * H, Mw,
                 sr.data_only));
      TRY(lin_dgrad(e, st, WS(L.g_mid) + r0 * H, H, Mw, L.to_out, s3, 512, 0, nullptr, 0, nullptr, nullptr, 0));
      mmvqa_fb_attn_desc a;
      fb_attn_fill(e, L, i, w, n, p, a);
      a.dout = s3; a.dout_ld = 512;
      a.dq = WS(L.g_q) + r0 * 512; a.dq_ld = 512;
      if (n == 2) { a.dself_k = WS(L.g_kv) + r0 * 1024; a.dself_v = a.dself_k + 512; a.dself_ld = 1024; }
      a.dmem_k = WS(e->fb_dmem); a.dmem_v = a.dmem_k + 512;
      a.dbias = sr.data_only ? nullptr : GRD(e->fb_rel);
      TRY(fb_attn_call(e, st, a, 1));
      const float* dxn = s4;
      { REG(REG_QKV);
        TRY(lin_dgrad(e, st, WS(L.g_q) + r0 * 512, 512, Mw, L.to_q, s4, H, 0, nullptr, 0, nullptr, nullptr, 0));
        if (n == 2) {
          TRY(lin_dgrad(e, st, WS(L.g_kv) + r0 * 1024, 1024, Mw, e->fb_kv, s5, H, 0, nullptr, 0, nullptr, s4, H));
          dxn = s5;
        } }
      TRY(ln_bwd(e, st, dxn, WS(e->fb_hid) + i * M * H + r0 * H, L.ln_a, WS(L.mean_a) + r0, WS(L.rstd_a) + r0,
                 WS(L.g_mid) + r0 * H, ghid + i * M * H + r0 * H, Mw, sr.data_only));
      if (wrote_mem)
        RUN(PROF_OTHER, 0, k_axpy(st, ghid + i * M * H + r0 * H, WS(e->fb_dhs) + (size_t)i * 2 * B * H, 1.0f, Mw * H));
    }
  }
  if (!sr.data_only) {
    const long Mfull = (long)2 * B * (T / 2), Mmem = (long)2 * B * (nwin - 1);
    struct TagScope { mmvqa_engine* e; TagScope(mmvqa_engine* e_) : e(e_) { e->prof_tag = HB_FB_WGRAD; } ~TagScope() { e->prof_tag = HB_NONE; } } tag(e);
    for (int i = NL - 1; i >= 0; --i) {
      FBLayerRef& L = e->fb[i];
      TRY(lin_wgrad_side(e, sr, st, ghid + (i + 1) * M * H, H, WS(L.gg), 4 * H, (long)M, L.w2, true));
      TRY(lin_wgrad_side(e, sr, st, WS(L.g_pre), 8 * H, WS(L.xn_f), H, (long)M, L.w1, true));
      TRY(lin_wgrad_side(e, sr, st, WS(L.g_mid), H, WS(L.ctx), 512, (long)M, L.to_out, true));
      REG(REG_QKV);
      TRY(lin_wgrad_side(e, sr, st, WS(L.g_q), 512, WS(L.xn_a), H, (long)M, L.to_q, false));
      TRY(lin_wgrad_side(e, sr, st, WS(L.g_kv), 1024, WS(L.xn_a), H, Mfull, e->fb_kv, false));
    }
    if (Mmem > 0) {
      REG(REG_QKV);
      TRY(lin_wgrad_side(e, sr, st, WS(e->fb_dmem), 1024, WS(e->fb_agg), H, Mmem, e->fb_kv, false));
// ... 269 lines not shown
```

### mm-vqa_amd/csrc/kernels.h

```cpp
#pragma once
#include "common.h"

#include <string>
#include <unordered_map>
#include <utility>

struct IgemmChoice { int tile, splitk; };
struct IgemmTuner {
  bool tuning = false;
  std::unordered_map<std::string, IgemmChoice> table;
};
void mmvqa_set_tuner(IgemmTuner* t);
void mmvqa_set_igemm_precision(int prec);
int mmvqa_launch_igemm(GemmParams p, int kind, int nchw, int tile, hipStream_t stream);
int mmvqa_launch_attention(const AttnParams& p, int head_dim, int bwd, hipStream_t st);
bool k_qkv_attn_fwd_ok(int T, int H, int heads);
int k_qkv_attn_fwd(hipStream_t st, const float* xn, const float* W, const float* bias, const long long* mask, float* qkv,
                   float* probs, float* ctx, int B, int T, int H, int heads, float drop_p, uint32_t seed);

int k_bn_coef_fwd(hipStream_t st, const double* stat, int C, double count, float eps, const float* gamma,
                  const float* beta, float* run_mean, float* run_var, long long* nbt, float momentum, int reps,
                  int training, float* scale, float* shift, float* mean, float* invstd);
int k_bn_coef_fwd_keep(hipStream_t st, const double* stat, int C, double count, float eps, const float* gamma,
                       const float* beta, float* run_mean, float* run_var, long long* nbt, double keep, int reps,
                       int training, float* scale, float* shift, float* mean, float* invstd);
int k_bn_coef_bwd(hipStream_t st, const double* stat, int C, double count, const float* gamma, const float* mean,
                  const float* invstd, int training, float* P, float* Q, float* R, float* dgamma, float* dbeta);
int k_bn_add_relu(hipStream_t st, const float* z, const float* s, const float* b, const float* idn,
                  const float* ids, const float* idb, float* out, long rows, int C);
int k_bn_act_add_fold(hipStream_t st, const float* z, const mmvqa_bn_fold* f3, int pre_act, const float* idn,
                      const mmvqa_bn_fold* fd, int post_act, float* out, long rows, int C);
int k_bn_add_relu_fold(hipStream_t st, const float* z, const mmvqa_bn_fold* f3, const float* idn, const mmvqa_bn_fold* fd,
                       float* out, long rows, int C);
int k_maxpool_fwd(hipStream_t st, const float* z, const float* s, const float* b, float* out, unsigned char* idx,
                  int N, int H, int W, int C, int OH, int OW);
int k_maxpool_bwd(hipStream_t st, const float* gp, const unsigned char* idx, const float* extra, const float* z,
                  const float* s, const float* b, const float* mean, const float* invstd, float* g0, double* stat,
                  int N, int H, int W, int C, int OH, int OW);
int k_layernorm_fwd(hipStream_t st, const float* x, const float* res, const float* gamma, const float* beta,
                    float* y, float* sum_out, float* mean, float* rstd, int rows, int H, float eps);
int k_layernorm_bwd(hipStream_t st, const float* dy, const float* x, const float* gamma, const float* mean,
                    const float* rstd, const float* dres, float* dx, float* dgamma, float* dbeta, int rows, int H);
int k_embed_fwd(hipStream_t st, const long long* ids, const long long* seg, const float* word, const float* pos,
                const float* type, const float* gamma, const float* beta, const float* vis, float* out,
                float* xhat, float* rstd, int B, int T, int H, int num_vis, float eps, float drop_p, uint32_t seed);
int k_embed_bwd(hipStream_t st, const float* dout, const long long* ids, const long long* seg, const float* xhat,
                const float* rstd, const float* gamma, float* dword, float* dpos, float* dtype, float* dgamma,
                float* dbeta, float* dvis, int B, int T, int H, int num_vis, float drop_p, uint32_t seed,
                int pad_idx);
int k_meanpool_fwd(hipStream_t st, const float* h, const long long* mask, float* out, int B, int T, int H);
int k_meanpool_bwd(hipStream_t st, const float* dout, const long long* mask, float* dh, int B, int T, int H,
                   int accumulate);
int k_lsm_nll(hipStream_t st, const float* logits, int ld, const long long* target, float* row_loss, float* row_lse,
              long long* pred, float* dlogits, int dld, const float* gscale_ptr, float gscale_mul, int rows, int V,
              float* out3);
int k_lsm_grad(hipStream_t st, const float* logits, int ld, const long long* target, const float* row_lse,
               float* dlogits, int dld, const float* gscale_ptr, float gscale_mul, int rows, int V);
int k_asl(hipStream_t st, const float* logits, int ld, const long long* target, float* row_loss, float* dlogits,
          int dld, int rows, int C, float gpos, float gneg, float eps, float gscale);
int k_l2norm_fwd(hipStream_t st, const float* x, float* y, float* nrm, int rows, int D);
int k_l2norm_bwd(hipStream_t st, const float* dy, const float* y, const float* nrm, float* dx, int rows, int D);
int k_supcon(hipStream_t st, const float* f, const float* mask, float* loss, float* df, float* ws, int N, int D,
             float temp, float base_temp, float gscale);
int k_jaccard_mask(hipStream_t st, const int* offsets, const int* ids, const int* rowsA, const int* colsA,
                   const int* rowsB, const int* colsB, float* mask, int n, int table_rows);
int k_normalize_rows(hipStream_t st, float* x, long long rows, int D, float eps);
int k_cosine_mask(hipStream_t st, const float* table, const int* rowsA, const int* colsA, const int* rowsB,
                  const int* colsB, float* mask, int n, int D, int table_rows);
int k_soft_ce(hipStream_t st, const float* logits, int ld, const long long* target, const long long* category,
              const float* table, int table_ld, int n_cat, int mode, double smoothing, float* row_loss, float* loss,
              float* dlogits, int dld, int rows, int C, float gscale);
int k_distill_mse(hipStream_t st, const float* h, int ld, const void* table, int table_f16, long long table_rows,
                  const long long* start, const int* count, int first, int B, int T, int H, float* row_sq, float* loss,
                  float* dh, int dld, float gscale);
int k_attention_len_fwd(hipStream_t st, const float* q, const float* k, const float* v, int row_stride, int head_stride,
                        float* out, int out_row_stride, int out_head_stride, const int* len, int B, int T, int heads,
                        float scale);
int k_bertscore_mask(hipStream_t st, const float* xa, const int* lenA, const float* xb, const int* lenB, float* mask,
                     float* prec, float* rec, int n, int T, int D, float baseline);
int k_fb_attention(hipStream_t st, const mmvqa_fb_attn_desc& p, int bwd);
int k_fb_aggregate_fwd(hipStream_t st, const float* hid, long long hstride, int nh, const float* lw, float* agg, long rows, int H);
int k_fb_aggregate_bwd(hipStream_t st, const float* dagg, const float* hid, long long hstride, int nh, const float* lw, float* dh,
                       long long dstride, float* dtop, float* dlw, long rows, int H);
int k_geglu_fwd(hipStream_t st, const float* pre, float* y, long M, int F, float drop_p, uint32_t seed, uint32_t idx0);
int k_geglu_bwd(hipStream_t st, const float* dy, const float* pre, float* dpre, long M, int F, float drop_p, uint32_t seed,
                uint32_t idx0);
int k_fb_reorder(hipStream_t st, const float* src, float* dst, int B, int T, int H, int to_window);
int k_adam(hipStream_t st, float* p, float* g, float* m, float* v, long n, double lr, double b1, double b2, double eps,
           int step, float gscale, int zero_grad);
int k_axpy(hipStream_t st, float* y, const float* x, float a, long n);
int k_amp_unscale(hipStream_t st, float* g, long n, const float* inv_scale, float* found_inf, int mul);
int k_amp_update_scale(hipStream_t st, float* scale, int* growth_tracker, const float* found_inf, double growth_factor,
                       double backoff_factor, int growth_interval);
int k_colsum(hipStream_t st, const float* x, int ld, int rows, int cols, float* out);
int k_dropout(hipStream_t st, float* x, long n, float p, uint32_t seed);
int k_pixmask(hipStream_t st, int* out, int N, int OH, int OW, int SH, int SW, int KH, int KW, int stride, int pad);
int k_dropout_copy(hipStream_t st, const float* x, float* y, long n, float p, uint32_t seed);
int k_spin(hipStream_t st, int us);

int k_bn_act_add(hipStream_t st, const float* z, const float* s, const float* b, int pre_act, const float* idn,
                 const float* ids, const float* idb, int idn_act, int post_act, float* out, long rows, int C);
int k_dwconv_fwd(hipStream_t st, const float* z1, const float* s1, const float* b1, const float* w, float* z2,
                 double* stat, int N, int H, int W, int C, int OH, int OW, int stride, int pad, const mmvqa_bn_fold* fold = nullptr);
int k_dwconv_bwd_data(hipStream_t st, const float* g2, const float* z2, const float* P, const float* Q,
                      const float* R, const float* w, const float* z1, const float* s1, const float* b1,
                      const float* mean1, const float* invstd1, float* g1, double* stat, int N, int H, int W, int C,
                      int OH, int OW, int stride, int pad, const mmvqa_bn_fold* fold = nullptr);
int k_dwconv_bwd_weight(hipStream_t st, const float* g2, const float* z2, const float* P, const float* Q,
                        const float* R, const float* z1, const float* s1, const float* b1, float* dw, int N, int H,
                        int W, int C, int OH, int OW, int stride, int pad, const mmvqa_bn_fold* fold = nullptr);
int k_se_pool(hipStream_t st, const float* z, const float* s, const float* b, float* pool, int N, int HW, int C,
              const mmvqa_bn_fold* fold = nullptr);
int k_se_dgate(hipStream_t st, const float* t, const float* z, const float* s, const float* b, float* dgate, int N,
               int HW, int C, float* zero = nullptr, int nzero = 0);
int k_act_bwd_stats(hipStream_t st, const float* t, const float* gate, const float* add, const float* z,
                    const float* s, const float* b, const float* mean, const float* invstd, int act, float* out,
                    double* stat, long npix, int HW, int C);
int k_mul_dact(hipStream_t st, const float* x, const float* pre, int act, float* y, long n);
bool k_tap_thin_ok(long M, int N, int C, int HW);
int k_tap_thin_fwd(hipStream_t st, const float* x, const float* sc, const float* sh, const float* W, float* out, long M,
                   int N, int C, int HW, int act);
int k_tap_thin_bwd(hipStream_t st, const float* x, const float* sc, const float* sh, const float* W, const float* dv,
                   float* du, long M, int N, int C, int HW, int act);
int k_skinny_fwd(hipStream_t st, const float* x, int x_ld, const float* W, const float* b, int act, float* pre,
                 float* y, int M, int N, int K);
size_t k_se_fc_bwd_scratch_floats(int B, int mid, int rd);
bool k_se_fc_bwd_ok(int rd);
int k_se_fc_bwd(hipStream_t st, const float* dgate, const float* gpre, const float* r, const float* rpre,
                const float* pool, const float* We, const float* Wr, float* dWe, float* dbe, float* dWr, float* dbr,
                float* dpool, float* scratch, int scratch_is_zero, int B, int mid, int rd);
```

Before: 670.4 samples/s.

## Fuse dropout grad into layernorm backward; restructure LN, embed and colsum reductions

Adds a layernorm backward variant that also writes the dropout-masked gradient, removing separate dropout-grad kernels in the BERT and transformer backward passes. It also rewrites the LN backward reduction to use an LDS column sum instead of shared-memory atomics, with an optional row-prefetch variant. The embedding backward is reorganised per position so that type and position gradients are reduced within a block, and colsum is vectorised with f32x4 loads. These changes target kernel count, memory traffic and atomic contention, but they make the kernels more complex and add register pressure.

```diff
diff --git a/include/mmvqa.h b/include/mmvqa.h
--- a/include/mmvqa.h
+++ b/include/mmvqa.h
@@ -251,6 +251,9 @@
 int mmvqa_layernorm_bwd(mmvqa_stream_t s, const float* dy, const float* x, const float* gamma, const float* mean,
                         const float* rstd, const float* dres, float* dx, float* dgamma, float* dbeta, int rows,
                         int H);
+int mmvqa_layernorm_bwd_drop(mmvqa_stream_t s, const float* dy, const float* x, const float* gamma, const float* mean,
+                             const float* rstd, const float* dres, float* dx, float* dgamma, float* dbeta, int rows,
+                             int H, float* ddrop, float p, uint32_t seed);
 int mmvqa_embed_fwd(mmvqa_stream_t s, const long long* ids, const long long* seg, const float* word,
                     const float* pos, const float* type, const float* gamma, const float* beta, const float* vis,
                     float* out, float* xhat, float* rstd, int B, int T, int H, int num_vis, float eps,
diff --git a/mm-vqa_amd/_lib.py b/mm-vqa_amd/_lib.py
--- a/mm-vqa_amd/_lib.py
+++ b/mm-vqa_amd/_lib.py
@@ -142,6 +142,7 @@
     "mmvqa_maxpool_bwd": (_i, [_P, _P, _P, _P, _P, _P, _P, _P, _P, _P, _P, _i, _i, _i, _i, _i, _i]),
     "mmvqa_layernorm_fwd": (_i, [_P, _P, _P, _P, _P, _P, _P, _P, _P, _i, _i, _f]),
     "mmvqa_layernorm_bwd": (_i, [_P, _P, _P, _P, _P, _P, _P, _P, _P, _P, _i, _i]),
+    "mmvqa_layernorm_bwd_drop": (_i, [_P, _P, _P, _P, _P, _P, _P, _P, _P, _P, _i, _i, _P, _f, _u32]),
     "mmvqa_embed_fwd": (_i, [_P, _P, _P, _P, _P, _P, _P, _P, _P, _P, _P, _P, _i, _i, _i, _i, _f, _f, _u32]),
     "mmvqa_embed_bwd": (_i, [_P, _P, _P, _P, _P, _P, _P, _P, _P, _P, _P, _P, _P, _i, _i, _i, _i, _f, _u32, _i]),
     "mmvqa_meanpool_fwd": (_i, [_P, _P, _P, _P, _i, _i, _i]),
diff --git a/mm-vqa_amd/csrc/abi.cpp b/mm-vqa_amd/csrc/abi.cpp
--- a/mm-vqa_amd/csrc/abi.cpp
+++ b/mm-vqa_amd/csrc/abi.cpp
@@ -132,6 +132,11 @@
                         int H) {
   return k_layernorm_bwd(ST(s), dy, x, gamma, mean, rstd, dres, dx, dgamma, dbeta, rows, H);
 }
+int mmvqa_layernorm_bwd_drop(mmvqa_stream_t s, const float* dy, const float* x, const float* gamma, const float* mean,
+                             const float* rstd, const float* dres, float* dx, float* dgamma, float* dbeta, int rows,
+                             int H, float* ddrop, float p, uint32_t seed) {
+  return k_layernorm_bwd_drop(ST(s), dy, x, gamma, mean, rstd, dres, dx, dgamma, dbeta, rows, H, ddrop, p, seed);
+}
 int mmvqa_embed_fwd(mmvqa_stream_t s, const long long* ids, const long long* seg, const float* word,
                     const float* pos, const float* type, const float* gamma, const float* beta, const float* vis,
                     float* out, float* xhat, float* rstd, int B, int T, int H, int num_vis, float eps,
diff --git a/mm-vqa_amd/csrc/elementwise.hip b/mm-vqa_amd/csrc/elementwise.hip
--- a/mm-vqa_amd/csrc/elementwise.hip
+++ b/mm-vqa_amd/csrc/elementwise.hip
@@ -249,24 +249,80 @@
   if (lane == 0) { mean_out[row] = mean; rstd_out[row] = rstd; }
 }
 
-__global__ void layernorm_bwd_kernel(const float* __restrict__ dy, const float* __restrict__ x,
+#define LN_CPT 4
+__device__ __forceinline__ void wg_cols_sum(float* __restrict__ lds, const f32x4 (&a)[LN_MAXV], int H, float (&s)[LN_CPT]) {
+  const int lane = threadIdx.x & 63, wave = threadIdx.x >> 6, nw = blockDim.x >> 6;
+  const int H4 = H / 4;
+#pragma unroll
+  for (int j = 0; j < LN_MAXV; ++j) {
+    int q = lane + 64 * j;
+    if (q < H4) reinterpret_cast<f32x4*>(lds + (size_t)wave * H)[q] = a[j];
+  }
+  __syncthreads();
+#pragma unroll
+  for (int k = 0; k < LN_CPT; ++k) {
+    const int i = threadIdx.x + k * blockDim.x;
+    s[k] = 0.f;
+    if (i < H) {
+      s[k] = lds[i];
+      for (int w = 1; w < nw; ++w) s[k] += lds[(size_t)w * H + i];
+    }
+  }
+  __syncthreads();
+}
+
+struct LnBwdRow {
+  f32x4 x[LN_MAXV], d[LN_MAXV], r[LN_MAXV];
+  float mu, rs;
+};
+__device__ __forceinline__ void ln_bwd_load(LnBwdRow& in, const float* __restrict__ x, const float* __restrict__ dy,
+                                            const float* __restrict__ dres, const float* __restrict__ mean,
+                                            const float* __restrict__ rstd, int row, int H) {
+  const int lane = threadIdx.x & 63, H4 = H / 4;
+  in.mu = mean[row]; in.rs = rstd[row];
+#pragma unroll
+  for (int j = 0; j < LN_MAXV; ++j) {
+    int q = lane + 64 * j;
+    in.x[j] = f32x4{0, 0, 0, 0}; in.d[j] = f32x4{0, 0, 0, 0}; in.r[j] = f32x4{0, 0, 0, 0};
+    if (q < H4) {
+      in.x[j] = reinterpret_cast<const f32x4*>(x + (size_t)row * H)[q];
+      in.d[j] = reinterpret_cast<const f32x4*>(dy + (size_t)row * H)[q];
+      if (dres) in.r[j] = reinterpret_cast<const f32x4*>(dres + (size_t)row * H)[q];
+    }
+  }
+}
+
+template <bool PF>
+__global__ __launch_bounds__(PF ? 512 : 256) void layernorm_bwd_kernel(const float* __restrict__ dy, const float* __restrict__ x,
                                      const float* __restrict__ gamma, const float* __restrict__ mean,
                                      const float* __restrict__ rstd, const float* __restrict__ dres,
                                      float* __restrict__ dx, float* __restrict__ dgamma,
-                                     float* __restrict__ dbeta, int rows, int H, int rows_per_wave) {
+                                     float* __restrict__ dbeta, float* __restrict__ ddrop, float drop_p, uint32_t seed,
+                                     int rows, int H, int rows_per_wave) {
   extern __shared__ float lds[];
   const int lane = threadIdx.x & 63, wave = threadIdx.x >> 6, nw = blockDim.x >> 6;
   const int H4 = H / 4;
-  for (int i = threadIdx.x; i < 2 * H; i += blockDim.x) lds[i] = 0.f;
-  __syncthreads();
-  f32x4 ag[LN_MAXV], ab[LN_MAXV];
-#pragma unroll
-  for (int j = 0; j < LN_MAXV; ++j) { ag[j] = f32x4{0, 0, 0, 0}; ab[j] = f32x4{0, 0, 0, 0}; }
-  const int row0 = (blockIdx.x * nw + wave) * rows_per_wave;
-  for (int rr = 0; rr < rows_per_wave; ++rr) {
-    const int row = row0 + rr;
-    if (row >= rows) break;
-    const float mu = mean[row], rs = rstd[row];
+  const float ks = 1.0f / (1.0f - drop_p);
+  f32x4 g[LN_MAXV], ag[LN_MAXV], ab[LN_MAXV];
+#pragma unroll
+  for (int j = 0; j < LN_MAXV; ++j) {
+    int q = lane + 64 * j;
+    ag[j] = f32x4{0, 0, 0, 0}; ab[j] = f32x4{0, 0, 0, 0}; g[j] = f32x4{0, 0, 0, 0};
+    if (q < H4) g[j] = reinterpret_cast<const f32x4*>(gamma)[q];
+  }
+  const int rpw = PF ? rows_per_wave : 1;
+  const int row0 = min(rows, (blockIdx.x * nw + wave) * rpw), row1 = min(rows, row0 + rpw);
+  LnBwdRow nx;
+  if (PF && row0 < row1) ln_bwd_load(nx, x, dy, dres, mean, rstd, row0, H);
+  for (int row = row0; row < row1; ++row) {
+    LnBwdRow in;
+    if (PF) {
+      in = nx;
+      if (row + 1 < row1) ln_bwd_load(nx, x, dy, dres, mean, rstd, row + 1, H);
+    } else {
+      ln_bwd_load(in, x, dy, dres, mean, rstd, row, H);
+    }
+    const float mu = in.mu, rs = in.rs;
     f32x4 xh[LN_MAXV], dg[LN_MAXV];
     float s1 = 0.f, s2 = 0.f;
 #pragma unroll
@@ -274,17 +330,12 @@
       int q = lane + 64 * j;
       xh[j] = f32x4{0, 0, 0, 0}; dg[j] = f32x4{0, 0, 0, 0};
       if (q < H4) {
-        f32x4 xv = reinterpret_cast<const f32x4*>(x + (size_t)row * H)[q];
-        f32x4 d = reinterpret_cast<const f32x4*>(dy + (size_t)row * H)[q];
-        f32x4 g = reinterpret_cast<const f32x4*>(gamma)[q];
 #pragma unroll
         for (int e = 0; e < 4; ++e) {
-          xh[j][e] = (xv[e] - mu) * rs;
-          dg[j][e] = d[e] * g[e];
+          xh[j][e] = (in.x[j][e] - mu) * rs;
+          dg[j][e] = in.d[j][e] * g[j][e];
           s1 += dg[j][e];
           s2 += dg[j][e] * xh[j][e];
-          ag[j][e] += d[e] * xh[j][e];
-          ab[j][e] += d[e];
         }
       }
     }
@@ -296,28 +347,32 @@
       if (q < H4) {
         f32x4 o;
 #pragma unroll
-        for (int e = 0; e < 4; ++e) o[e] = rs * (dg[j][e] - s1 - xh[j][e] * s2);
-        if (dres) o += reinterpret_cast<const f32x4*>(dres + (size_t)row * H)[q];
+        for (int e = 0; e < 4; ++e) {
+          o[e] = rs * (dg[j][e] - s1 - xh[j][e] * s2);
+          ag[j][e] += in.d[j][e] * xh[j][e];
+          ab[j][e] += in.d[j][e];
+        }
+        if (dres) o += in.r[j];
         reinterpret_cast<f32x4*>(dx + (size_t)row * H)[q] = o;
+        if (ddrop) {
+          f32x4 od;
+#pragma unroll
+          for (int e = 0; e < 4; ++e)
+            od[e] = (rng_uniform(seed, (uint32_t)row * (uint32_t)H + q * 4 + e) >= drop_p) ? o[e] * ks : 0.f;
+          reinterpret_cast<f32x4*>(ddrop + (size_t)row * H)[q] = od;
+        }
       }
     }
-  }
-#pragma unroll
-  for (int j = 0; j < LN_MAXV; ++j) {
-    int q = lane + 64 * j;
-    if (q < H4) {
-#pragma unroll
-      for (int e = 0; e < 4; ++e) {
-        atomicAdd(&lds[q * 4 + e], ag[j][e]);
-        atomicAdd(&lds[H + q * 4 + e], ab[j][e]);
-      }
-    }
-  }
-  __syncthreads();
+    if (!PF) break;
+  }
   if (!dgamma) return;
-  for (int i = threadIdx.x; i < H; i += blockDim.x) {
-    atomicAdd(&dgamma[i], lds[i]);
-    atomicAdd(&dbeta[i], lds[H + i]);
+  float sg[LN_CPT], sb[LN_CPT];
+  wg_cols_sum(lds, ag, H, sg);
+  wg_cols_sum(lds, ab, H, sb);
+#pragma unroll
+  for (int k = 0; k < LN_CPT; ++k) {
+    const int i = threadIdx.x + k * blockDim.x;
+    if (i < H) { atomicAdd(&dgamma[i], sg[k]); atomicAdd(&dbeta[i], sb[k]); }
   }
 }
 
@@ -388,63 +443,96 @@
   if (lane == 0 && rstd_out) rstd_out[row] = rstd;
 }
 
-__global__ void embed_bwd_kernel(const float* __restrict__ dout, const long long* __restrict__ ids,
+__global__ __launch_bounds__(256) void embed_bwd_kernel(const float* __restrict__ dout, const long long* __restrict__ ids,
                                  const long long* __restrict__ seg, const float* __restrict__ xhat,
                                  const float* __restrict__ rstd, const float* __restrict__ gamma,
                                  float* __restrict__ dword, float* __restrict__ dpos, float* __restrict__ dtype,
                                  float* __restrict__ dgamma, float* __restrict__ dbeta, float* __restrict__ dvis,
                                  int B, int T, int H, int num_vis, float drop_p, uint32_t seed, int pad_idx) {
-  const int lane = threadIdx.x & 63;
-  const int row = blockIdx.x * (blockDim.x >> 6) + (threadIdx.x >> 6);
-  if (row >= B * T) return;
-  const int b = row / T, t = row - b * T;
+  extern __shared__ float lds[];
+  const int lane = threadIdx.x & 63, wave = threadIdx.x >> 6, nw = blockDim.x >> 6;
+  const int t = blockIdx.x;
   const int H4 = H / 4;
   if (t < num_vis) {
-    for (int q = lane; q < H4; q += 64)
-      reinterpret_cast<f32x4*>(dvis + ((size_t)t * B + b) * H)[q] =
-          reinterpret_cast<const f32x4*>(dout + (size_t)row * H)[q];
+    const int b = blockIdx.y * nw + wave;
+    if (b < B)
+      for (int q = lane; q < H4; q += 64)
+        reinterpret_cast<f32x4*>(dvis + ((size_t)t * B + b) * H)[q] =
+            reinterpret_cast<const f32x4*>(dout + ((size_t)b * T + t) * H)[q];
     return;
   }
-  const long long id = ids[row], sg = seg[row];
-  const float rs = rstd[row];
   const float ks = drop_p > 0.f ? 1.0f / (1.0f - drop_p) : 1.f;
-  f32x4 xh[LN_MAXV], dg[LN_MAXV];
-  float s1 = 0.f, s2 = 0.f;
+  f32x4 ag[LN_MAXV], ab[LN_MAXV], at0[LN_MAXV], at1[LN_MAXV];
 #pragma unroll
   for (int j = 0; j < LN_MAXV; ++j) {
-    int q = lane + 64 * j;
-    xh[j] = f32x4{0, 0, 0, 0}; dg[j] = f32x4{0, 0, 0, 0};
-    if (q < H4) {
-      f32x4 d = reinterpret_cast<const f32x4*>(dout + (size_t)row * H)[q];
-      xh[j] = reinterpret_cast<const f32x4*>(xhat + (size_t)row * H)[q];
-      f32x4 g = reinterpret_cast<const f32x4*>(gamma)[q];
-#pragma unroll
-      for (int e = 0; e < 4; ++e) {
-        if (drop_p > 0.f) {
-          float u = rng_uniform(seed, (uint32_t)row * (uint32_t)H + q * 4 + e);
-          d[e] = (u >= drop_p) ? d[e] * ks : 0.f;
+    ag[j] = f32x4{0, 0, 0, 0}; ab[j] = f32x4{0, 0, 0, 0}; at0[j] = f32x4{0, 0, 0, 0}; at1[j] = f32x4{0, 0, 0, 0};
+  }
+  int has0 = 0, has1 = 0;
+  const int b = blockIdx.y * nw + wave;
+  if (b < B) {
+    const int row = b * T + t;
+    const long long id = ids[row], sg = seg[row];
+    const float rs = rstd[row];
+    has0 = sg == 0; has1 = sg == 1;
+    f32x4 xh[LN_MAXV], dg[LN_MAXV];
+    float s1 = 0.f, s2 = 0.f;
+#pragma unroll
+    for (int j = 0; j < LN_MAXV; ++j) {
+      int q = lane + 64 * j;
+      xh[j] = f32x4{0, 0, 0, 0}; dg[j] = f32x4{0, 0, 0, 0};
+      if (q < H4) {
+        f32x4 d = reinterpret_cast<const f32x4*>(dout + (size_t)row * H)[q];
+        xh[j] = reinterpret_cast<const f32x4*>(xhat + (size_t)row * H)[q];
+        f32x4 g = reinterpret_cast<const f32x4*>(gamma)[q];
+#pragma unroll
+        for (int e = 0; e < 4; ++e) {
+          if (drop_p > 0.f) {
+            float u = rng_uniform(seed, (uint32_t)row * (uint32_t)H + q * 4 + e);
+            d[e] = (u >= drop_p) ? d[e] * ks : 0.f;
+          }
+          ag[j][e] = d[e] * xh[j][e];
+          ab[j][e] = d[e];
+          dg[j][e] = d[e] * g[e];
+          s1 += dg[j][e];
+          s2 += dg[j][e] * xh[j][e];
         }
-        atomicAdd(&dgamma[q * 4 + e], d[e] * xh[j][e]);
-        atomicAdd(&dbeta[q * 4 + e], d[e]);
-        dg[j][e] = d[e] * g[e];
-        s1 += dg[j][e];
-        s2 += dg[j][e] * xh[j][e];
       }
     }
-  }
-  s1 = wave_sum(s1) / (float)H;
-  s2 = wave_sum(s2) / (float)H;
-#pragma unroll
-  for (int j = 0; j < LN_MAXV; ++j) {
-    int q = lane + 64 * j;
-    if (q < H4) {
-#pragma unroll
-      for (int e = 0; e < 4; ++e) {
-        float de = rs * (dg[j][e] - s1 - xh[j][e] * s2);
-        if (id != pad_idx) atomicAdd(&dword[(size_t)id * H + q * 4 + e], de);
-        atomicAdd(&dtype[(size_t)sg * H + q * 4 + e], de);
-        atomicAdd(&dpos[(size_t)t * H + q * 4 + e], de);
+    s1 = wave_sum(s1) / (float)H;
+    s2 = wave_sum(s2) / (float)H;
+#pragma unroll
+    for (int j = 0; j < LN_MAXV; ++j) {
+      int q = lane + 64 * j;
+      if (q < H4) {
+#pragma unroll
+        for (int e = 0; e < 4; ++e) {
+          float de = rs * (dg[j][e] - s1 - xh[j][e] * s2);
+          if (id != pad_idx) atomicAdd(&dword[(size_t)id * H + q * 4 + e], de);
+          if (sg == 0) at0[j][e] = de;
+          else if (sg == 1) at1[j][e] = de;
+          else {
+            atomicAdd(&dtype[(size_t)sg * H + q * 4 + e], de);
+            atomicAdd(&dpos[(size_t)t * H + q * 4 + e], de);
+          }
+        }
       }
+    }
+  }
+  float sg_[LN_CPT], sb_[LN_CPT], s0_[LN_CPT], s1_[LN_CPT];
+  wg_cols_sum(lds, ag, H, sg_);
+  wg_cols_sum(lds, ab, H, sb_);
+  wg_cols_sum(lds, at0, H, s0_);
+  wg_cols_sum(lds, at1, H, s1_);
+  const int any0 = __syncthreads_or(has0), any1 = __syncthreads_or(has1);
+#pragma unroll
+  for (int k = 0; k < LN_CPT; ++k) {
+    const int i = threadIdx.x + k * blockDim.x;
+    if (i < H) {
+      atomicAdd(&dgamma[i], sg_[k]);
+      atomicAdd(&dbeta[i], sb_[k]);
+      if (any0) atomicAdd(&dtype[i], s0_[k]);
+      if (any1) atomicAdd(&dtype[(size_t)H + i], s1_[k]);
+      if (any0 | any1) atomicAdd(&dpos[(size_t)t * H + i], s0_[k] + s1_[k]);
     }
   }
 }
@@ -767,13 +855,40 @@
   for (; i < n; i += stride) y[i] += a * x[i];
 }
 
-__global__ void colsum_kernel(const float* __restrict__ x, int ld, int rows, int cols, float* __restrict__ out) {
-  int c = blockIdx.x * blockDim.x + threadIdx.x;
-  if (c >= cols) return;
-  int r0 = blockIdx.y * 64, r1 = min(rows, r0 + 64);
-  float s = 0.f;
-  for (int r = r0; r < r1; ++r) s += x[(size_t)r * ld + c];
-  atomicAdd(&out[c], s);
+__global__ __launch_bounds__(256) void colsum_kernel(const float* __restrict__ x, int ld, int rows, int cols,
+                                                     float* __restrict__ out, int vec) {
+  __shared__ f32x4 part[3][64];
+  const int lane = threadIdx.x & 63, wave = threadIdx.x >> 6;
+  const int c0 = blockIdx.x * 256 + lane * 4;
+  const int r0 = blockIdx.y * 64, r1 = min(rows, r0 + 64);
+  f32x4 s = f32x4{0, 0, 0, 0};
+  if (c0 < cols) {
+    if (vec && c0 + 4 <= cols) {
+      f32x4 v[16];
+#pragma unroll
+      for (int k = 0; k < 16; ++k) v[k] = *reinterpret_cast<const f32x4*>(x + (size_t)min(r0 + wave + 4 * k, r1 - 1) * ld + c0);
+#pragma unroll
+      for (int k = 0; k < 16; ++k)
+        if (r0 + wave + 4 * k < r1) s += v[k];
+    } else {
+#pragma unroll
+      for (int k = 0; k < 16; ++k) {
+        const float* xr = x + (size_t)min(r0 + wave + 4 * k, r1 - 1) * ld + c0;
+        const bool in = r0 + wave + 4 * k < r1;
+#pragma unroll
+        for (int e = 0; e < 4; ++e)
+          if (c0 + e < cols) { const float v = xr[e]; s[e] += in ? v : 0.f; }
+      }
+    }
+  }
+  if (wave) part[wave - 1][lane] = s;
+  __syncthreads();
+  if (wave == 0 && c0 < cols) {
+    s += part[0][lane]; s += part[1][lane]; s += part[2][lane];
+#pragma unroll
+    for (int e = 0; e < 4; ++e)
+      if (c0 + e < cols) atomicAdd(&out[c0 + e], s[e]);
+  }
 }
 
 __global__ void dropout_kernel(float* __restrict__ x, long n, float p, uint32_t seed) {
@@ -940,15 +1055,27 @@
   return MMVQA_OK;
 }
 
+int k_layernorm_bwd_drop(hipStream_t st, const float* dy, const float* x, const float* gamma, const float* mean,
+                         const float* rstd, const float* dres, float* dx, float* dgamma, float* dbeta, int rows, int H,
+                         float* ddrop, float p, uint32_t seed) {
+  if (H % 4 != 0 || H > 256 * LN_MAXV) return mmvqa_set_error(MMVQA_ERR_ARG, "layernorm: H=%d unsupported", H);
+  if (ddrop && !(p >= 0.f && p < 1.f)) return mmvqa_set_error(MMVQA_ERR_ARG, "layernorm: dropout p=%g outside [0, 1)", (double)p);
+  if (rows <= 0) return MMVQA_OK;
+  if (rows <= 1024) {
+    hipLaunchKernelGGL(layernorm_bwd_kernel<false>, dim3(cdiv_i(rows, 4)), dim3(256), (size_t)4 * H * sizeof(float), st, dy,
+                       x, gamma, mean, rstd, dres, dx, dgamma, dbeta, ddrop, p, seed, rows, H, 1);
+  } else {
+    const int rpw = cdiv_i(rows, 1024) < 8 ? cdiv_i(rows, 1024) : 8;
+    hipLaunchKernelGGL(layernorm_bwd_kernel<true>, dim3(cdiv_i(rows, 8 * rpw)), dim3(512), (size_t)8 * H * sizeof(float), st,
+                       dy, x, gamma, mean, rstd, dres, dx, dgamma, dbeta, ddrop, p, seed, rows, H, rpw);
+  }
+  KERNEL_CHECK_RET();
+  return MMVQA_OK;
+}
+
 int k_layernorm_bwd(hipStream_t st, const float* dy, const float* x, const float* gamma, const float* mean,
                     const float* rstd, const float* dres, float* dx, float* dgamma, float* dbeta, int rows, int H) {
-  if (H % 4 != 0 || H > 256 * LN_MAXV) return mmvqa_set_error(MMVQA_ERR_ARG, "layernorm: H=%d unsupported", H);
-  int rpw = rows >= 2048 ? 4 : (rows >= 512 ? 2 : 1);
-  int grid = cdiv_i(rows, 4 * rpw);
-  hipLaunchKernelGGL(layernorm_bwd_kernel, dim3(grid), dim3(256), 2 * H * sizeof(float), st, dy, x, gamma, mean,
-                     rstd, dres, dx, dgamma, dbeta, rows, H, rpw);
-  KERNEL_CHECK_RET();
-  return MMVQA_OK;
+  return k_layernorm_bwd_drop(st, dy, x, gamma, mean, rstd, dres, dx, dgamma, dbeta, rows, H, nullptr, 0.f, 0);
 }
 
 int k_embed_fwd(hipStream_t st, const long long* ids, const long long* seg, const float* word, const float* pos,
@@ -967,8 +1094,10 @@
                 float* dbeta, float* dvis, int B, int T, int H, int num_vis, float drop_p, uint32_t seed,
                 int pad_idx) {
   if (H % 4 != 0 || H > 256 * LN_MAXV) return mmvqa_set_error(MMVQA_ERR_ARG, "embed: H=%d unsupported", H);
-  hipLaunchKernelGGL(embed_bwd_kernel, dim3(cdiv_i((long)B * T, 4)), dim3(256), 0, st, dout, ids, seg, xhat, rstd,
-                     gamma, dword, dpos, dtype, dgamma, dbeta, dvis, B, T, H, num_vis, drop_p, seed, pad_idx);
+  if (B <= 0 || T <= 0) return MMVQA_OK;
+  hipLaunchKernelGGL(embed_bwd_kernel, dim3(T, cdiv_i(B, 4)), dim3(256), (size_t)4 * H * sizeof(float), st, dout, ids,
+                     seg, xhat, rstd, gamma, dword, dpos, dtype, dgamma, dbeta, dvis, B, T, H, num_vis, drop_p, seed,
+                     pad_idx);
   KERNEL_CHECK_RET();
   return MMVQA_OK;
 }
@@ -1062,8 +1191,10 @@
 }
 
 int k_colsum(hipStream_t st, const float* x, int ld, int rows, int cols, float* out) {
+  if (rows <= 0 || cols <= 0) return MMVQA_OK;
+  const int vec = ((uintptr_t)x % 16 == 0 && ld % 4 == 0) ? 1 : 0;
   hipLaunchKernelGGL(colsum_kernel, dim3(cdiv_i(cols, 256), cdiv_i(rows, 64)), dim3(256), 0, st, x, ld, rows, cols,
-                     out);
+                     out, vec);
   KERNEL_CHECK_RET();
   return MMVQA_OK;
 }
diff --git a/mm-vqa_amd/csrc/engine.cpp b/mm-vqa_amd/csrc/engine.cpp
--- a/mm-vqa_amd/csrc/engine.cpp
+++ b/mm-vqa_amd/csrc/engine.cpp
@@ -599,10 +599,11 @@
   return MMVQA_OK;
 }
 static int ln_bwd(mmvqa_engine* e, hipStream_t st, const float* dy, const float* x, const LNRef& ln,
-                  const float* mean, const float* rstd, const float* dres, float* dx, long rows, bool data_only = false) {
-  RUNB(HB_LAYERNORM_BWD, (dres ? 16.0 : 12.0) * rows * e->d.hidden, k_layernorm_bwd(st, dy, x, PRM(ln.g), mean, rstd, dres, dx,
-                                     data_only ? nullptr : GRD(ln.g), data_only ? nullptr : GRD(ln.b), (int)rows,
-                                     e->d.hidden));
+                  const float* mean, const float* rstd, const float* dres, float* dx, long rows, bool data_only = false,
+                  float* ddrop = nullptr, float p = 0.f, uint32_t seed = 0) {
+  RUNB(HB_LAYERNORM_BWD, ((dres ? 16.0 : 12.0) + (ddrop ? 4.0 : 0.0)) * rows * e->d.hidden,
+       k_layernorm_bwd_drop(st, dy, x, PRM(ln.g), mean, rstd, dres, dx, data_only ? nullptr : GRD(ln.g),
+                            data_only ? nullptr : GRD(ln.b), (int)rows, e->d.hidden, ddrop, p, seed));
   return MMVQA_OK;
 }
 
@@ -1337,6 +1338,17 @@
   return MMVQA_OK;
 }
 
+static int ln_bwd_drop(mmvqa_engine* e, hipStream_t st, SideReads& sr, const float* dy, const float* x, const LNRef& ln,
+                       const float* mean, const float* rstd, const float* dres, float* dx, float p, uint32_t seed,
+                       const float** out) {
+  const long rows = (long)e->B * e->T;
+  *out = dx;
+  if (!(p > 0.f)) return ln_bwd(e, st, dy, x, ln, mean, rstd, dres, dx, rows, sr.data_only);
+  TRY(sr.write(WS(e->t_b)));
+  *out = WS(e->t_b);
+  return ln_bwd(e, st, dy, x, ln, mean, rstd, dres, dx, rows, sr.data_only, WS(e->t_b), p, seed);
+}
+
 static int bert_forward(mmvqa_engine* e, hipStream_t st, const float* x_in, const float** x_out) {
   REG(REG_ENC);
   const mmvqa_model_desc& d = e->d;
@@ -1375,11 +1387,11 @@
   const long M = (long)e->B * e->T;
   const float p = e->training ? d.p_drop : 0.f;
   float* dz = WS(e->t_a);
+  const float* dzd = dz;
   for (int i = d.n_layers - 1; i >= 0; --i) {
     BertLayerRef& L = e->bert[i];
     const float* x = i == 0 ? x_in : WS(e->bert[i - 1].z);
-    const float* dzd;
-    TRY(drop_grad(e, st, sr, dz, p, site_seed(e, i, 2), &dzd));
+    if (i == d.n_layers - 1) TRY(drop_grad(e, st, sr, dz, p, site_seed(e, i, 2), &dzd));
     TRY(lin_wgrad_side(e, sr, st, dzd, H, WS(L.h1), 4 * H, M, L.fc2, true));
     TRY(sr.write(WS(e->t_big)));
     TRY(lin_dgrad(e, st, dzd, H, M, L.fc2, WS(e->t_big), 4 * H, ACT_GELU, WS(L.pre1), 4 * H, sr.bias_grad(GRD(L.fc1.b)), nullptr, 0));
@@ -1387,10 +1399,9 @@
     TRY(sr.write(WS(e->t_c)));
     TRY(lin_dgrad(e, st, WS(e->t_big), 4 * H, M, L.fc1, WS(e->t_c), H, 0, nullptr, 0, nullptr, nullptr, 0));
     TRY(sr.write(WS(e->t_d)));
-    TRY(ln_bwd(e, st, WS(e->t_c), WS(L.y), e->norm1, WS(L.mean2), WS(L.rstd2), dz, WS(e->t_d), M, sr.data_only));
     float* dy = WS(e->t_d);
     const float* dyd;
-    TRY(drop_grad(e, st, sr, dy, p, site_seed(e, i, 1), &dyd));
+    TRY(ln_bwd_drop(e, st, sr, WS(e->t_c), WS(L.y), e->norm1, WS(L.mean2), WS(L.rstd2), dz, dy, p, site_seed(e, i, 1), &dyd));
     TRY(lin_wgrad_side(e, sr, st, dyd, H, WS(L.ctx), H, M, L.proj, true));
     TRY(sr.write(WS(e->t_c)));
     TRY(lin_dgrad(e, st, dyd, H, M, L.proj, WS(e->t_c), H, 0, nullptr, 0, nullptr, nullptr, 0));
@@ -1405,7 +1416,8 @@
       TRY(sr.write(WS(e->t_c)));
       TRY(lin_dgrad(e, st, dqkv, 3 * H, M, L.qkv, WS(e->t_c), H, 0, nullptr, 0, nullptr, nullptr, 0)); }
     TRY(sr.write(dz));
-    TRY(ln_bwd(e, st, WS(e->t_c), x, e->norm1, WS(L.mean1), WS(L.rstd1), dy, dz, M, sr.data_only));
+    if (i > 0) TRY(ln_bwd_drop(e, st, sr, WS(e->t_c), x, e->norm1, WS(L.mean1), WS(L.rstd1), dy, dz, p, site_seed(e, i - 1, 2), &dzd));
+    else TRY(ln_bwd(e, st, WS(e->t_c), x, e->norm1, WS(L.mean1), WS(L.rstd1), dy, dz, M, sr.data_only));
   }
   return MMVQA_OK;
 }
@@ -1444,10 +1456,9 @@
     RFLayerRef& L = e->rf[i];
     const float* x = i == 0 ? x_in : WS(e->rf[i - 1].x2);
     TRY(sr.write(WS(e->t_d)));
-    TRY(ln_bwd(e, st, dx2, WS(L.s2), L.ln2, WS(L.mean2), WS(L.rstd2), nullptr, WS(e->t_d), M, sr.data_only));
     float* ds2 = WS(e->t_d);
     const float* dff;
-    TRY(drop_grad(e, st, sr, ds2, p, site_seed(e, i, 2), &dff));
+    TRY(ln_bwd_drop(e, st, sr, dx2, WS(L.s2), L.ln2, WS(L.mean2), WS(L.rstd2), nullptr, ds2, p, site_seed(e, i, 2), &dff));
     TRY(lin_wgrad_side(e, sr, st, dff, H, WS(L.hact), 4 * H, M, L.ff2, true));
     TRY(sr.write(WS(e->t_big)));
     TRY(lin_dgrad(e, st, dff, H, M, L.ff2, WS(e->t_big), 4 * H, ACT_SERF, WS(L.pre), 4 * H, sr.bias_grad(GRD(L.ff0.b)), nullptr, 0));
@@ -1455,10 +1466,9 @@
     TRY(sr.write(WS(e->t_c)));
     TRY(lin_dgrad(e, st, WS(e->t_big), 4 * H, M, L.ff0, WS(e->t_c), H, 0, nullptr, 0, nullptr, ds2, H));
     TRY(sr.write(WS(e->t_d)));
-    TRY(ln_bwd(e, st, WS(e->t_c), WS(L.s1), L.ln1, WS(L.mean1), WS(L.rstd1), nullptr, WS(e->t_d), M, sr.data_only));
     float* ds1 = WS(e->t_d);
     const float* dr;
-    TRY(drop_grad(e, st, sr, ds1, p, site_seed(e, i, 1), &dr));
+    TRY(ln_bwd_drop(e, st, sr, WS(e->t_c), WS(L.s1), L.ln1, WS(L.mean1), WS(L.rstd1), nullptr, ds1, p, site_seed(e, i, 1), &dr));
     TRY(lin_wgrad_side(e, sr, st, dr, H, WS(L.res), H, M, L.proj, false));
     TRY(sr.write(WS(e->t_c)));
     TRY(lin_dgrad(e, st, dr, H, M, L.proj, WS(e->t_c), H, 0, nullptr, 0, nullptr, nullptr, 0));
diff --git a/mm-vqa_amd/csrc/kernels.h b/mm-vqa_amd/csrc/kernels.h
--- a/mm-vqa_amd/csrc/kernels.h
+++ b/mm-vqa_amd/csrc/kernels.h
@@ -41,6 +41,9 @@
                     float* y, float* sum_out, float* mean, float* rstd, int rows, int H, float eps);
 int k_layernorm_bwd(hipStream_t st, const float* dy, const float* x, const float* gamma, const float* mean,
                     const float* rstd, const float* dres, float* dx, float* dgamma, float* dbeta, int rows, int H);
+int k_layernorm_bwd_drop(hipStream_t st, const float* dy, const float* x, const float* gamma, const float* mean,
+                         const float* rstd, const float* dres, float* dx, float* dgamma, float* dbeta, int rows, int H,
+                         float* ddrop, float p, uint32_t seed);
 int k_embed_fwd(hipStream_t st, const long long* ids, const long long* seg, const float* word, const float* pos,
                 const float* type, const float* gamma, const float* beta, const float* vis, float* out,
                 float* xhat, float* rstd, int B, int T, int H, int num_vis, float eps, float drop_p, uint32_t seed);
```

Result: no change. 674.9 samples/s, median of 6 (+0.7%).
